# weidafeng/Efficient-SlowFast

Hardware: AMD Instinct MI355X
Metric: clips/sec (8x8 224^2 SlowFast-R50+CMDA, train step fwd+bwd+allreduce+SGD) (higher is better)
Workload: dtype f32

## Files before the change

### efficient-slowfast_amd/csrc/backward.hip

```cpp
#include "common.h"
#include <stdlib.h>

namespace {

constexpr int TPB = 256;


inline int pow2ceil_b(int v) {
  int p = 1;
  while (p < v) p <<= 1;
  return p;
}

template <int VEC>
__device__ __forceinline__ void bn_g(const float* __restrict__ dy, int dy_cs, int dy_coff,
                                     const float* __restrict__ y, int y_cs, int y_coff, long r, long THW, int HW,
                                     int rep, int relu, int c, float (&g)[VEC]) {
  long r0 = r;
  if (rep > 1) {
    const long n = r / THW, rem = r - n * THW;
    const long t = rem / HW, hw = rem - t * HW;
    r0 = (n * (THW / HW) * rep + t * rep) * HW + hw;
  }
#pragma unroll
// ... 387 lines not shown
  for (int a = 1; a < alpha; ++a) mx = fmaxf(mx, s[(long)a * HW * cs]);
  const float dm = dz[((long)b * rows + r) * dz_cs + dz_coff + c] * gate[(long)b * C + c] + dpool[(long)b * C + c];
  for (int a = 0; a < alpha; ++a)
    if (s[(long)a * HW * cs] == mx) {
      dx[(base + (long)a * HW) * dx_cs + dx_coff + c] += dm;
      break;
    }
}

__global__ void bcast_add_kernel(float* __restrict__ g, int cs, int coff, long rows_per_n, int C,
                                 const float* __restrict__ v, float scale, long total) {
  const long idx = (long)blockIdx.x * TPB + threadIdx.x;
  if (idx >= total) return;
  const int c = (int)(idx % C);
  const long r = idx / C;
  const long n = r / rows_per_n;
  g[r * cs + coff + c] += v[n * C + c] * scale;
}

__global__ void rowdot_kernel(const float* __restrict__ a, int a_cs, int a_coff, const float* __restrict__ b,
                              int b_cs, int b_coff, long rows, int C, float scale, float* __restrict__ out) {
  const long r = (long)blockIdx.x * TPB + threadIdx.x;
  if (r >= rows) return;
  const float* ap = a + r * a_cs + a_coff;
  const float* bp = b + r * b_cs + b_coff;
  float s = 0.f;
  for (int c = 0; c < C; ++c) s = fmaf(ap[c], bp[c], s);
  out[r] = s * scale;
}

__global__ __launch_bounds__(256) void rowdot_vec4_kernel(const float* __restrict__ a, int a_cs, int a_coff,
                                                          const float* __restrict__ b, int b_cs, int b_coff, long rows,
                                                          int cv_shift, float scale, float* __restrict__ out) {
  const long idx = (long)blockIdx.x * TPB + threadIdx.x;
  const long r = idx >> cv_shift;
  const int c = (int)(idx - (r << cv_shift)) * 4;
  float s = 0.f;
  if (r < rows) {
    const f32x4 x = *reinterpret_cast<const f32x4*>(a + r * a_cs + a_coff + c);
    const f32x4 y = *reinterpret_cast<const f32x4*>(b + r * b_cs + b_coff + c);
    s = x[0] * y[0] + x[1] * y[1] + x[2] * y[2] + x[3] * y[3];
  }
  for (int o = (1 << cv_shift) >> 1; o > 0; o >>= 1) s += __shfl_xor(s, o, 64);
  if (r < rows && c == 0) out[r] = s * scale;
}

__global__ void axpy_kernel(const float* __restrict__ a, int a_cs, int a_coff, float alpha, float* __restrict__ out,
                            int out_cs, int out_coff, int C, int accumulate, long total) {
  const long idx = (long)blockIdx.x * TPB + threadIdx.x;
  if (idx >= total) return;
  const int c = (int)(idx % C);
  const long r = idx / C;
  const float v = alpha * a[r * a_cs + a_coff + c];
  float* o = out + r * out_cs + out_coff + c;
  *o = accumulate ? *o + v : v;
}

__global__ void act_bwd_kernel(const float* __restrict__ dy, int dy_cs, int dy_coff, const float* __restrict__ y,
                               int y_cs, int y_coff, int act, float* __restrict__ dx, int dx_cs, int dx_coff, int C,
                               int accumulate, long total) {
  const long idx = (long)blockIdx.x * TPB + threadIdx.x;
  if (idx >= total) return;
  const int c = (int)(idx % C);
  const long r = idx / C;
  const float yv = y[r * y_cs + y_coff + c];
  const bool pass = (yv > 0.f) && (act != SF_ACT_RELU6 || yv < 6.f);
  const float v = pass ? dy[r * dy_cs + dy_coff + c] : 0.f;
  float* o = dx + r * dx_cs + dx_coff + c;
  *o = accumulate ? *o + v : v;
}

}

constexpr int MAX_P = 1024;
static inline void red_geometry(long rows, int C, int vec, int* CB, int* P) {
  const int cv = sf_cdiv(C, vec);
  *CB = pow2ceil_b(cv) < TPB ? pow2ceil_b(cv) : TPB;
  const int rpi = TPB / *CB;
  long p = rows / ((long)rpi * 8);
  if (p < 1) p = 1;
  if (p > MAX_P) p = MAX_P;
  *P = (int)p;
}
extern "C" long sf_bn_bwd_ws_floats(int C) { return (long)MAX_P * 2 * C; }

static int bn_bwd_reduce_launch(const float* dy, int dy_cs, int dy_coff, const float* y, int y_cs, int y_coff,
                                const float* z, int z_cs, int z_coff, int N, int T, int H, int W, int C, int S,
                                int rep, int relu, const float* mean, const float* invstd, float* dbeta,
                                float* dgamma, float* ws, void* stream, float* dbeta_acc = nullptr,
                                float* dgamma_acc = nullptr) {
  if ((dbeta_acc == nullptr) != (dgamma_acc == nullptr)) return SF_EINVAL;
  if (!dy || !z || !mean || !invstd || !dbeta || !dgamma || !ws || (relu && !y)) return SF_EINVAL;
  if (relu == 3 && (rep != 1 || (C % 4) != 0 || y_cs != C / 4 || y_coff != 0)) return SF_EINVAL;
  if (N <= 0 || T <= 0 || H <= 0 || W <= 0 || C <= 0 || rep <= 0 || S <= 0 || N % S != 0) return SF_EINVAL;
  if (S > 1 && N > MAX_P) return SF_EINVAL;
  const long rows = (long)N * T * H * W;
  const bool vec4 = (C % 4 == 0) && (dy_cs % 4 == 0) && (dy_coff % 4 == 0) && (z_cs % 4 == 0) && (z_coff % 4 == 0) &&
                    sf_aligned16(dy) && sf_aligned16(z) &&
                    (!relu || relu == 3 || ((y_cs % 4 == 0) && (y_coff % 4 == 0) && sf_aligned16(y)));
  if (relu == 3 && !vec4) return SF_EINVAL;
  const int groups = S > 1 ? N : 1;
  const long group_rows = rows / groups;
  int CB, P;
  const bool ring = sf_ticket_ring_ready((hipStream_t)stream);
  red_geometry(group_rows, C, vec4 ? 4 : 1, &CB, &P);
  const bool small = ring && S == 1 && P <= 16;
  const bool few = !small && ring && S == 1 && vec4 && C >= 256;
  const bool fused = few || small;
  const int max_p = few ? 64 : (small ? 512 : MAX_P);
  if (few && CB > 16) {
    CB = 16;
    long pp = group_rows / ((long)(TPB / CB) * 8);
    P = (int)(pp < 1 ? 1 : (pp > max_p ? max_p : pp));
  }
  if (P > max_p) P = max_p;
  if ((long)P * groups > max_p) P = max_p / groups;
  if (P < 1) return SF_EINVAL;
  const int chunks = P;
  P = chunks * groups;
  const int ncb = sf_cdiv(sf_cdiv(C, vec4 ? 4 : 1), CB);
  unsigned* tickets = fused ? sf_ticket_slots(ncb) : nullptr;
  if (fused && !tickets) return SF_ELAUNCH;
  if (vec4)
    hipLaunchKernelGGL(bn_bwd_partial_kernel<4>, dim3(P, ncb), dim3(TPB), 0, (hipStream_t)stream, dy, dy_cs, dy_coff,
                       y, y_cs, y_coff, z, z_cs, z_coff, group_rows, chunks, S, (long)T * H * W, H * W, C, rep, relu,
                       mean, invstd, CB, ws, tickets, dbeta, dgamma, dbeta_acc, dgamma_acc);
  else
    hipLaunchKernelGGL(bn_bwd_partial_kernel<1>, dim3(P, ncb), dim3(TPB), 0, (hipStream_t)stream, dy, dy_cs, dy_coff,
                       y, y_cs, y_coff, z, z_cs, z_coff, group_rows, chunks, S, (long)T * H * W, H * W, C, rep, relu,
                       mean, invstd, CB, ws, tickets, dbeta, dgamma, dbeta_acc, dgamma_acc);
  if (!fused)
    hipLaunchKernelGGL(pair_final_kernel, dim3(S * C), dim3(64), 0, (hipStream_t)stream, ws, C, P, chunks, S, dbeta,
                       dgamma, dbeta_acc, dgamma_acc);
  SF_CHECK_LAUNCH();
  return SF_OK;
}

extern "C" int sf_bn_bwd_reduce(const float* dy, int dy_cs, int dy_coff, const float* y, int y_cs, int y_coff,
                                const float* z, int z_cs, int z_coff, int N, int T, int H, int W, int C, int rep,
                                int relu, const float* mean, const float* invstd, float* dbeta, float* dgamma,
                                float* ws, void* stream) {
  return bn_bwd_reduce_launch(dy, dy_cs, dy_coff, y, y_cs, y_coff, z, z_cs, z_coff, N, T, H, W, C, 1, rep, relu, mean,
                              invstd, dbeta, dgamma, ws, stream);
}

extern "C" int sf_bn_bwd_reduce_acc(const float* dy, int dy_cs, int dy_coff, const float* y, int y_cs, int y_coff,
                                    const float* z, int z_cs, int z_coff, int N, int T, int H, int W, int C, int rep,
                                    int relu, const float* mean, const float* invstd, float* dbeta, float* dgamma,
                                    float* ws, float* dbeta_acc, float* dgamma_acc, void* stream) {
  return bn_bwd_reduce_launch(dy, dy_cs, dy_coff, y, y_cs, y_coff, z, z_cs, z_coff, N, T, H, W, C, 1, rep, relu, mean,
                              invstd, dbeta, dgamma, ws, stream, dbeta_acc, dgamma_acc);
}

extern "C" int sf_bn_bwd_reduce_split(const float* dy, int dy_cs, int dy_coff, const float* y, int y_cs, int y_coff,
                                      const float* z, int z_cs, int z_coff, int N, int T, int H, int W, int C,
                                      int nsplit, int rep, int relu, const float* mean, const float* invstd,
                                      float* dbeta, float* dgamma, float* ws, void* stream) {
  return bn_bwd_reduce_launch(dy, dy_cs, dy_coff, y, y_cs, y_coff, z, z_cs, z_coff, N, T, H, W, C, nsplit, rep, relu,
                              mean, invstd, dbeta, dgamma, ws, stream);
}

static int bn_bwd_apply_launch(const float* dy, int dy_cs, int dy_coff, const float* y, int y_cs, int y_coff,
                               const float* z, int z_cs, int z_coff, int N, int T, int H, int W, int C, int S, int rep,
                               int relu, const float* mean, const float* invstd, const float* gamma,
                               const float* dbeta, const float* dgamma, float* dz, int dz_cs, int dz_coff,
                               float* dres, int dres_cs, int dres_coff, int dres_acc, void* stream) {
  if (!dy || !z || !mean || !invstd || !gamma || !dbeta || !dgamma || !dz || (relu && !y)) return SF_EINVAL;
  if (relu == 3 && (rep != 1 || (C % 4) != 0 || y_cs != C / 4 || y_coff != 0)) return SF_EINVAL;
  if (N <= 0 || T <= 0 || H <= 0 || W <= 0 || C <= 0 || rep <= 0 || S <= 0 || N % S != 0) return SF_EINVAL;
  const long rows = (long)N * T * H * W;
  const bool vec4 = (C % 4 == 0) && (dy_cs % 4 == 0) && (dy_coff % 4 == 0) && (z_cs % 4 == 0) && (z_coff % 4 == 0) &&
                    (dz_cs % 4 == 0) && (dz_coff % 4 == 0) && sf_aligned16(dy) && sf_aligned16(z) && sf_aligned16(dz) &&
                    (!relu || relu == 3 || ((y_cs % 4 == 0) && (y_coff % 4 == 0) && sf_aligned16(y))) &&
                    (!dres || ((dres_cs % 4 == 0) && (dres_coff % 4 == 0) && sf_aligned16(dres)));
  if (relu == 3 && !vec4) return SF_EINVAL;
  const long total = rows * (vec4 ? C / 4 : C);
  const int unroll4 = (vec4 && rep == 1 && (relu == 0 || relu == 3) && total >= 262144L &&
                       total < 0x7fffffffL && rows < 0x7fffffffL && (rows % 4) == 0 &&
                       sf_aligned16(mean) && sf_aligned16(invstd) && sf_aligned16(gamma) && sf_aligned16(dbeta) &&
                       sf_aligned16(dgamma)) ? 1 : 0;
  if (vec4)
    hipLaunchKernelGGL(bn_bwd_apply_kernel<4>, dim3(sf_cdiv(unroll4 ? (total + 3) / 4 : total, TPB)), dim3(TPB), 0,
                       (hipStream_t)stream, dy, dy_cs, dy_coff, y, y_cs, y_coff, z, z_cs, z_coff, rows, (long)T * H * W,
                       H * W, C, S, rep, relu, mean, invstd, gamma, dbeta, dgamma, (float)S / (float)rows, dz, dz_cs,
                       dz_coff, dres, dres_cs, dres_coff, dres_acc, total, unroll4);
  else
    hipLaunchKernelGGL(bn_bwd_apply_kernel<1>, dim3(sf_cdiv(total, TPB)), dim3(TPB), 0, (hipStream_t)stream, dy, dy_cs,
                       dy_coff, y, y_cs, y_coff, z, z_cs, z_coff, rows, (long)T * H * W, H * W, C, S, rep, relu, mean,
                       invstd, gamma, dbeta, dgamma, (float)S / (float)rows, dz, dz_cs, dz_coff, dres, dres_cs,
                       dres_coff, dres_acc, total, 0);
  SF_CHECK_LAUNCH();
  return SF_OK;
}

extern "C" int sf_bn_bwd_apply(const float* dy, int dy_cs, int dy_coff, const float* y, int y_cs, int y_coff,
                               const float* z, int z_cs, int z_coff, int N, int T, int H, int W, int C, int rep,
                               int relu, const float* mean, const float* invstd, const float* gamma,
                               const float* dbeta, const float* dgamma, float* dz, int dz_cs, int dz_coff,
                               float* dres, int dres_cs, int dres_coff, void* stream) {
  return bn_bwd_apply_launch(dy, dy_cs, dy_coff, y, y_cs, y_coff, z, z_cs, z_coff, N, T, H, W, C, 1, rep, relu, mean,
                             invstd, gamma, dbeta, dgamma, dz, dz_cs, dz_coff, dres, dres_cs, dres_coff, 1, stream);
}

extern "C" int sf_bn_bwd_apply_first(const float* dy, int dy_cs, int dy_coff, const float* y, int y_cs, int y_coff,
                                     const float* z, int z_cs, int z_coff, int N, int T, int H, int W, int C, int rep,
                                     int relu, const float* mean, const float* invstd, const float* gamma,
                                     const float* dbeta, const float* dgamma, float* dz, int dz_cs, int dz_coff,
                                     float* dres, int dres_cs, int dres_coff, void* stream) {
  if (!dres) return SF_EINVAL;
  return bn_bwd_apply_launch(dy, dy_cs, dy_coff, y, y_cs, y_coff, z, z_cs, z_coff, N, T, H, W, C, 1, rep, relu, mean,
                             invstd, gamma, dbeta, dgamma, dz, dz_cs, dz_coff, dres, dres_cs, dres_coff, 0, stream);
}

extern "C" int sf_bn_bwd_apply_split(const float* dy, int dy_cs, int dy_coff, const float* y, int y_cs, int y_coff,
                                     const float* z, int z_cs, int z_coff, int N, int T, int H, int W, int C,
                                     int nsplit, int rep, int relu, const float* mean, const float* invstd,
                                     const float* gamma, const float* dbeta, const float* dgamma, float* dz,
                                     int dz_cs, int dz_coff, float* dres, int dres_cs, int dres_coff, void* stream) {
  return bn_bwd_apply_launch(dy, dy_cs, dy_coff, y, y_cs, y_coff, z, z_cs, z_coff, N, T, H, W, C, nsplit, rep, relu,
                             mean, invstd, gamma, dbeta, dgamma, dz, dz_cs, dz_coff, dres, dres_cs, dres_coff, 1,
                             stream);
}

__global__ __launch_bounds__(256) void maxpool_bwd_vec4_kernel(const sf_pool_desc d, const float* __restrict__ x,
                                                               const float* __restrict__ y,
                                                               const float* __restrict__ dy, int dy_cs, int dy_coff,
                                                               float* __restrict__ dx, int dx_cs, int dx_coff,
                                                               int acc, unsigned total) {
  const unsigned idx = blockIdx.x * TPB + threadIdx.x;
  if (idx >= total) return;
  const unsigned cv = d.C >> 2;
  const unsigned rin = idx / cv;
  const int c = (int)(idx - rin * cv) * 4;
  unsigned r = rin;
  const int wi = (int)(r % (unsigned)d.Wi);
  r /= (unsigned)d.Wi;
  const int hi = (int)(r % (unsigned)d.Hi);
  r /= (unsigned)d.Hi;
  const int ti = (int)(r % (unsigned)d.Ti);
  const int n = (int)(r / (unsigned)d.Ti);
  const f32x4 xv = *reinterpret_cast<const f32x4*>(x + (long)rin * d.in_cs + d.in_coff + c);
  auto lo = [](int i, int p, int k, int s) { const int a = i + p - k + 1; return a <= 0 ? 0 : (a + s - 1) / s; };
  const int t0 = lo(ti, d.pT, d.kT, d.sT), t1 = min((ti + d.pT) / d.sT, d.To - 1);
  const int h0 = lo(hi, d.pH, d.kH, d.sH), h1 = min((hi + d.pH) / d.sH, d.Ho - 1);
  const int w0 = lo(wi, d.pW, d.kW, d.sW), w1 = min((wi + d.pW) / d.sW, d.Wo - 1);
  f32x4 g = {0.f, 0.f, 0.f, 0.f};
  for (int to = t0; to <= t1; ++to)
    for (int ho = h0; ho <= h1; ++ho)
      for (int wo = w0; wo <= w1; ++wo) {
        const long ro = (((long)n * d.To + to) * d.Ho + ho) * d.Wo + wo;
        const f32x4 yv = *reinterpret_cast<const f32x4*>(y + ro * d.out_cs + d.out_coff + c);
        const f32x4 gv = *reinterpret_cast<const f32x4*>(dy + ro * dy_cs + dy_coff + c);
        unsigned m = (yv[0] == xv[0] ? 1u : 0u) | (yv[1] == xv[1] ? 2u : 0u) | (yv[2] == xv[2] ? 4u : 0u) |
                     (yv[3] == xv[3] ? 8u : 0u);
        if (m) {
          const int ts = to * d.sT - d.pT, hs = ho * d.sH - d.pH, ws = wo * d.sW - d.pW;
          for (int tt = max(ts, 0); tt <= ti && m; ++tt)
            for (int hh = max(hs, 0); hh < min(hs + d.kH, d.Hi) && m; ++hh) {
              if (tt == ti && hh > hi) break;
              for (int ww = max(ws, 0); ww < min(ws + d.kW, d.Wi) && m; ++ww) {
                if (tt == ti && hh == hi && ww >= wi) break;
                const f32x4 xe = *reinterpret_cast<const f32x4*>(
                    x + ((((long)n * d.Ti + tt) * d.Hi + hh) * d.Wi + ww) * d.in_cs + d.in_coff + c);
#pragma unroll
                for (int e = 0; e < 4; ++e)
                  if (xe[e] == yv[e]) m &= ~(1u << e);
              }
            }
#pragma unroll
          for (int e = 0; e < 4; ++e)
            if ((m >> e) & 1u) g[e] += gv[e];
        }
      }
  f32x4* o = reinterpret_cast<f32x4*>(dx + (long)rin * dx_cs + dx_coff + c);
  *o = acc ? *o + g : g;
}

static int maxpool_bwd_launch(const sf_pool_desc* d, const float* x, const float* y, const float* dy, int dy_cs,
                              int dy_coff, float* dx, int dx_cs, int dx_coff, int acc, void* stream) {
  if (!d || !x || !y || !dy || !dx || d->is_avg) return SF_EINVAL;
  const long total = (long)d->N * d->Ti * d->Hi * d->Wi * d->C;
  const bool vec4 = (d->C % 4 == 0) && (d->in_cs % 4 == 0) && (d->in_coff % 4 == 0) && (d->out_cs % 4 == 0) &&
                    (d->out_coff % 4 == 0) && (dy_cs % 4 == 0) && (dy_coff % 4 == 0) && (dx_cs % 4 == 0) &&
                    (dx_coff % 4 == 0) && sf_aligned16(x) && sf_aligned16(y) && sf_aligned16(dy) && sf_aligned16(dx) &&
                    total / 4 < 0x7fffffffL;
  if (vec4)
    hipLaunchKernelGGL(maxpool_bwd_vec4_kernel, dim3(sf_cdiv(total / 4, TPB)), dim3(TPB), 0, (hipStream_t)stream, *d, x,
                       y, dy, dy_cs, dy_coff, dx, dx_cs, dx_coff, acc, (unsigned)(total / 4));
  else
    hipLaunchKernelGGL(maxpool_bwd_kernel, dim3(sf_cdiv(total, TPB)), dim3(TPB), 0, (hipStream_t)stream, *d, x, y, dy,
                       dy_cs, dy_coff, dx, dx_cs, dx_coff, acc, total);
  SF_CHECK_LAUNCH();
  return SF_OK;
}

extern "C" int sf_maxpool_bwd(const sf_pool_desc* d, const float* x, const float* y, const float* dy, int dy_cs,
                              int dy_coff, float* dx, int dx_cs, int dx_coff, void* stream) {
  return maxpool_bwd_launch(d, x, y, dy, dy_cs, dy_coff, dx, dx_cs, dx_coff, 1, stream);
}

extern "C" int sf_maxpool_bwd_first(const sf_pool_desc* d, const float* x, const float* y, const float* dy, int dy_cs,
                                    int dy_coff, float* dx, int dx_cs, int dx_coff, void* stream) {
  return maxpool_bwd_launch(d, x, y, dy, dy_cs, dy_coff, dx, dx_cs, dx_coff, 0, stream);
}

extern "C" int sf_tmax_dot(const float* x, int cs, int coff, int N, int T, int H, int W, int C, int alpha,
// ... 449 lines not shown
```

### efficient-slowfast_amd/csrc/conv_bx.hip

```cpp
#include "bx.h"
#include <stdlib.h>

namespace {

constexpr int BXC_BM = 256;
constexpr int BXC_BK = 16;
constexpr int BXC_STAGES = 3;
constexpr int BXC_ROWB = BXC_BK * 2;
constexpr int BXC_A_STAGE = 3 * BXC_BM * BXC_ROWB;

struct BxArgs {
  sf_conv_desc d;
  const unsigned short* ap;
  const unsigned short* bp;
  float* ws;
  const float* scale;
  const float* bias;
  const float* res;
  float* out;
  int M, ntaps, cpk, nk, S, nk_per, nb_n, tiles;
  int tap_major;
  unsigned a_rows, a_bytes, b_bytes;
  unsigned a_plane, b_plane;
  unsigned wo_mul, wo_sh, ho_mul, ho_sh, to_mul, to_sh;
  const float* xf;
  unsigned xf_bytes;
  float* stats;
};

__device__ __forceinline__ unsigned mdiv(unsigned n, unsigned mul, unsigned sh) {
  return mul ? (__umulhi(n, mul) >> sh) : n;
}

typedef __attribute__((address_space(3))) void lds_void;

template <int BN, bool DIRECT, bool AF32>
__global__ __launch_bounds__(512, 2) void conv_bx_kernel(const BxArgs p) {
  constexpr int A_ST = AF32 ? BXC_BM * 64 : BXC_A_STAGE;
  constexpr int B_STAGE = 3 * BN * BXC_ROWB;
  constexpr int STAGE = A_ST + B_STAGE;
  constexpr int NT = BN / 64;
  extern __shared__ __attribute__((aligned(16))) char smem[];
  const sf_conv_desc& d = p.d;
  const int tid = threadIdx.x, lane = tid & 63;
  const int wave = __builtin_amdgcn_readfirstlane(tid >> 6);
  const int wm = wave & 3, wn = wave >> 2;
  const int bid = xcd_remap(blockIdx.x, p.tiles * p.S);
  const int split = bid / p.tiles, tile = bid - split * p.tiles;
  const int tile_m = tile / p.nb_n, tile_n = tile - tile_m * p.nb_n;
  const int m0 = tile_m * BXC_BM, n0 = tile_n * BN;
  const int ks0 = split * p.nk_per;
  const int ks1 = ks0 + p.nk_per < p.nk ? ks0 + p.nk_per : p.nk;
  const int nsteps = ks1 - ks0;

  const int lrow = lane >> 1;
  const unsigned lchunk = (unsigned)((lane & 1) ^ ((lrow >> 4) & 1)) * 16u;
  const int am = m0 + 32 * wave + lrow;
  const bool a_ok = am < p.M;
  int t0, h0, w0, nimg;
  {
    const unsigned mm = a_ok ? (unsigned)am : 0u;
    const unsigned q1 = mdiv(mm, p.wo_mul, p.wo_sh);
    const unsigned wo = mm - q1 * (unsigned)d.Wo;
    const unsigned q2 = mdiv(q1, p.ho_mul, p.ho_sh);
    const unsigned ho = q1 - q2 * (unsigned)d.Ho;
    const unsigned q3 = mdiv(q2, p.to_mul, p.to_sh);
    const unsigned to = q2 - q3 * (unsigned)d.To;
    nimg = (int)q3;
    t0 = d.transposed ? (int)to + d.pT : (int)to * d.sT - d.pT;
    h0 = d.transposed ? (int)ho + d.pH : (int)ho * d.sH - d.pH;
    w0 = d.transposed ? (int)wo + d.pW : (int)wo * d.sW - d.pW;
  }
  struct FRow { int t0, h0, w0, n; bool ok; unsigned chunk; };
  FRow fr0 = {0, 0, 0, 0, false, 0u}, fr1 = fr0;
  if constexpr (AF32) {
    auto frow = [&](int u) -> FRow {
      FRow f;
      const int r = 32 * wave + 16 * u + (lane >> 2);
      const int fm = m0 + r;
      f.ok = fm < p.M;
      f.chunk = (unsigned)((lane & 3) ^ ((r >> 2) & 3)) * 16u;
      const unsigned mm = f.ok ? (unsigned)fm : 0u;
      const unsigned q1 = mdiv(mm, p.wo_mul, p.wo_sh);
      const unsigned wo = mm - q1 * (unsigned)d.Wo;
      const unsigned q2 = mdiv(q1, p.ho_mul, p.ho_sh);
      const unsigned ho = q1 - q2 * (unsigned)d.Ho;
      const unsigned q3 = mdiv(q2, p.to_mul, p.to_sh);
      const unsigned to = q2 - q3 * (unsigned)d.To;
      f.n = (int)q3;
      f.t0 = d.transposed ? (int)to + d.pT : (int)to * d.sT - d.pT;
      f.h0 = d.transposed ? (int)ho + d.pH : (int)ho * d.sH - d.pH;
      f.w0 = d.transposed ? (int)wo + d.pW : (int)wo * d.sW - d.pW;
      return f;
    };
    fr0 = frow(0);
    fr1 = frow(1);
  }
  auto f_voff = [&](const FRow f, int kt, int kh, int kw) -> unsigned {
    const int ti = d.transposed ? f.t0 - kt * d.dT : f.t0 + kt * d.dT;
    const int hi = d.transposed ? f.h0 - kh * d.dH : f.h0 + kh * d.dH;
    const int wi = d.transposed ? f.w0 - kw * d.dW : f.w0 + kw * d.dW;
    const bool ok = f.ok && (unsigned)ti < (unsigned)d.Ti && (unsigned)hi < (unsigned)d.Hi && (unsigned)wi < (unsigned)d.Wi;
    if (!ok) return 0x80000000u;
    const unsigned r = (unsigned)(((f.n * d.Ti + ti) * d.Hi + hi) * d.Wi + wi);
    return (r * (unsigned)d.in_cs + (unsigned)d.in_coff) * 4u + f.chunk;
  };
  const unsigned row_bytes = (unsigned)d.Cin * 2u;
  auto a_voff = [&](int kt, int kh, int kw) -> unsigned {
    const int ti = d.transposed ? t0 - kt * d.dT : t0 + kt * d.dT;
    const int hi = d.transposed ? h0 - kh * d.dH : h0 + kh * d.dH;
    const int wi = d.transposed ? w0 - kw * d.dW : w0 + kw * d.dW;
    const bool ok = a_ok && (unsigned)ti < (unsigned)d.Ti && (unsigned)hi < (unsigned)d.Hi && (unsigned)wi < (unsigned)d.Wi;
    const unsigned r = ok ? (unsigned)(((nimg * d.Ti + ti) * d.Hi + hi) * d.Wi + wi) : p.a_rows;
    return r * row_bytes + lchunk;
  };
  const bool b_loader = BN == 256 || wave < BN / 32;
  const int bn = n0 + 32 * wave + lrow;
  const unsigned kbytes = (unsigned)p.nk * (unsigned)BXC_ROWB;
  const unsigned b_voff = (unsigned)((b_loader && bn < d.Cout) ? bn : d.Cout) * kbytes + lchunk;

  const __amdgpu_buffer_rsrc_t a_rs = __builtin_amdgcn_make_buffer_rsrc((void*)p.ap, 0, p.a_bytes, 0x00020000);
  const __amdgpu_buffer_rsrc_t b_rs = __builtin_amdgcn_make_buffer_rsrc((void*)p.bp, 0, p.b_bytes, 0x00020000);
  const __amdgpu_buffer_rsrc_t x_rs = __builtin_amdgcn_make_buffer_rsrc((void*)p.xf, 0, AF32 ? p.xf_bytes : 0u, 0x00020000);

  struct LS { int c, tap, kw, kh, kt; };
  LS ls;
  ls.c = __builtin_amdgcn_readfirstlane(p.tap_major ? ks0 % p.cpk : ks0 / p.ntaps);
  ls.tap = __builtin_amdgcn_readfirstlane(p.tap_major ? ks0 / p.cpk : ks0 - ls.c * p.ntaps);
  ls.kw = __builtin_amdgcn_readfirstlane(ls.tap % d.kW);
  ls.kh = __builtin_amdgcn_readfirstlane((ls.tap / d.kW) % d.kH);
  ls.kt = __builtin_amdgcn_readfirstlane(ls.tap / (d.kW * d.kH));
  const int tap_major = p.tap_major, cpk = p.cpk, kW = d.kW, kH = d.kH, kT = d.kT;
  auto next = [=](const LS o) -> LS {
    LS n;
    if (tap_major) {
      const int c1 = o.c + 1;
      const bool wc = c1 == cpk;
      n.c = wc ? 0 : c1;
      n.tap = o.tap + (wc ? 1 : 0);
      const int w1 = o.kw + (wc ? 1 : 0);
      const bool ww = w1 == kW;
      n.kw = ww ? 0 : w1;
      const int h1 = o.kh + (ww ? 1 : 0);
      const bool wh = h1 == kH;
      n.kh = wh ? 0 : h1;
      n.kt = o.kt + (wh ? 1 : 0);
      return n;
    }
    const int w1 = o.kw + 1;
    const bool ww = w1 == kW;
    n.kw = ww ? 0 : w1;
    const int h1 = o.kh + (ww ? 1 : 0);
    const bool wh = h1 == kH;
    n.kh = wh ? 0 : h1;
    const int t1 = o.kt + (wh ? 1 : 0);
    const bool wt = t1 == kT;
    n.kt = wt ? 0 : t1;
    n.tap = wt ? 0 : o.tap + 1;
    n.c = o.c + (wt ? 1 : 0);
    return n;
  };
  auto issue = [&](int stage) {
    const LS l = ls;
    unsigned cur_voff = 0, cur_aso, cur_f0 = 0, cur_f1 = 0;
    if constexpr (AF32) {
      cur_f0 = f_voff(fr0, l.kt, l.kh, l.kw);
      cur_f1 = f_voff(fr1, l.kt, l.kh, l.kw);
      cur_aso = (unsigned)l.c * 64u;
    } else {
      cur_voff = a_voff(l.kt, l.kh, l.kw);
      cur_aso = (unsigned)l.c * (unsigned)BXC_ROWB;
    }
    const unsigned cur_bso = (unsigned)(l.tap * p.cpk + l.c) * (unsigned)BXC_ROWB;
    if constexpr (AF32) {
      __builtin_amdgcn_raw_ptr_buffer_load_lds(x_rs, (lds_void*)(smem + stage * STAGE + wave * 2048), 16, cur_f0, cur_aso,
                                               0, 0);
      __builtin_amdgcn_raw_ptr_buffer_load_lds(x_rs, (lds_void*)(smem + stage * STAGE + wave * 2048 + 1024), 16, cur_f1,
                                               cur_aso, 0, 0);
    } else {
      char* const sa = smem + stage * STAGE + wave * 1024;
#pragma unroll
      for (int g = 0; g < 3; ++g)
        __builtin_amdgcn_raw_ptr_buffer_load_lds(a_rs, (lds_void*)(sa + g * (BXC_BM * BXC_ROWB)), 16, cur_voff,
                                                 cur_aso + (unsigned)g * p.a_plane, 0, 0);
    }
    if (b_loader) {
      char* const sb = smem + stage * STAGE + A_ST + wave * 1024;
#pragma unroll
      for (int g = 0; g < 3; ++g)
        __builtin_amdgcn_raw_ptr_buffer_load_lds(b_rs, (lds_void*)(sb + g * (BN * BXC_ROWB)), 16, b_voff,
                                                 cur_bso + (unsigned)g * p.b_plane, 0, 0);
    }
    ls = next(l);
  };

  const unsigned frag_lane = (unsigned)(lane & 31) * BXC_ROWB + (unsigned)(((lane >> 5) ^ ((lane >> 4) & 1)) * 16);
  const unsigned a_frag = (unsigned)(wm * 64) * BXC_ROWB + frag_lane;
  const unsigned b_frag = A_ST + (unsigned)(wn * (BN / 2)) * BXC_ROWB + frag_lane;
  unsigned f_frag[2][2] = {{0, 0}, {0, 0}};
  if constexpr (AF32) {
#pragma unroll
    for (int i = 0; i < 2; ++i) {
      const int r = wm * 64 + i * 32 + (lane & 31);
#pragma unroll
      for (int q = 0; q < 2; ++q) f_frag[i][q] = (unsigned)r * 64u + (unsigned)(((2 * (lane >> 5) + q) ^ ((r >> 2) & 3)) * 16);
    }
  }

  f32x16 acc[2][NT];
#pragma unroll
  for (int i = 0; i < 2; ++i)
#pragma unroll
    for (int j = 0; j < NT; ++j)
#pragma unroll
      for (int e = 0; e < 16; ++e) acc[i][j][e] = 0.f;

  if (nsteps > 0) issue(0);
  if (nsteps > 1) issue(1);
  for (int it = 0; it < nsteps; ++it) {
    if (it + 1 < nsteps) {
      if constexpr (AF32) {
        if (b_loader) asm volatile("s_waitcnt vmcnt(5)" ::: "memory");
        else asm volatile("s_waitcnt vmcnt(2)" ::: "memory");
      } else {
        if (b_loader) asm volatile("s_waitcnt vmcnt(6)" ::: "memory");
        else asm volatile("s_waitcnt vmcnt(3)" ::: "memory");
      }
    } else {
      asm volatile("s_waitcnt vmcnt(0)" ::: "memory");
    }
    __builtin_amdgcn_s_barrier();
    if (it + 2 < nsteps) issue((it + 2) % BXC_STAGES);
    const char* const st = smem + (it % BXC_STAGES) * STAGE;
    u32x4 af[2][3], bf[NT][3];
    if constexpr (AF32) {
#pragma unroll
      for (int i = 0; i < 2; ++i) {
        const f32x4 lo = *reinterpret_cast<const f32x4*>(st + f_frag[i][0]);
        const f32x4 hi = *reinterpret_cast<const f32x4*>(st + f_frag[i][1]);
        split_pair(lo[0], lo[1], af[i], 0);
        split_pair(lo[2], lo[3], af[i], 1);
        split_pair(hi[0], hi[1], af[i], 2);
        split_pair(hi[2], hi[3], af[i], 3);
      }
    }
#pragma unroll
    for (int pc = 0; pc < 3; ++pc) {
      if constexpr (!AF32) {
#pragma unroll
        for (int i = 0; i < 2; ++i)
          af[i][pc] = *reinterpret_cast<const u32x4*>(st + a_frag + pc * (BXC_BM * BXC_ROWB) + i * (32 * BXC_ROWB));
      }
#pragma unroll
      for (int j = 0; j < NT; ++j)
        bf[j][pc] = *reinterpret_cast<const u32x4*>(st + b_frag + pc * (BN * BXC_ROWB) + j * (32 * BXC_ROWB));
    }
#pragma unroll
    for (int i = 0; i < 2; ++i)
#pragma unroll
      for (int j = 0; j < NT; ++j) acc[i][j] = mfma_split(af[i], bf[j], acc[i][j]);
  }

  const int col = lane & 31, rsub = 4 * (lane >> 5);
  if (DIRECT) {
#pragma unroll
    for (int j = 0; j < NT; ++j) {
      const int n = n0 + wn * (BN / 2) + j * 32 + col;
      const bool n_ok = n < d.Cout;
      const float sc = (p.scale && n_ok) ? p.scale[n] : 1.f;
      const float bi = (p.bias && n_ok) ? p.bias[n] : 0.f;
#pragma unroll
      for (int i = 0; i < 2; ++i) {
        float r[16];
#pragma unroll
        for (int e = 0; e < 16; ++e) {
          const int m = m0 + wm * 64 + i * 32 + (e & 3) + 8 * (e >> 2) + rsub;
          r[e] = (p.res && m < p.M && n_ok) ? p.res[(long)m * d.res_cs + d.res_coff + n] : 0.f;
        }
#pragma unroll
        for (int e = 0; e < 16; ++e) {
          const int m = m0 + wm * 64 + i * 32 + (e & 3) + 8 * (e >> 2) + rsub;
          if (m < p.M && n_ok) p.out[(long)m * d.out_cs + d.out_coff + n] = sf_act(acc[i][j][e] * sc + bi + r[e], d.act);
        }
      }
    }
    return;
  }
  float* const wsp = p.ws + (long)split * p.M * d.Cout;
#pragma unroll
  for (int i = 0; i < 2; ++i)
#pragma unroll
    for (int j = 0; j < NT; ++j) {
      const int n = n0 + wn * (BN / 2) + j * 32 + col;
#pragma unroll
      for (int e = 0; e < 16; ++e) {
        const int m = m0 + wm * 64 + i * 32 + (e & 3) + 8 * (e >> 2) + rsub;
        if (m < p.M && n < d.Cout) wsp[(long)m * d.Cout + n] = acc[i][j][e];
      }
    }
}

template <int BN>
__global__ __launch_bounds__(512, 4) void conv_pw_bx_kernel(const BxArgs p) {
  constexpr int A_STAGE = BXC_BM * 64;
  constexpr int B_STAGE = 3 * BN * BXC_ROWB;
  constexpr int STAGE = A_STAGE + B_STAGE;
  constexpr int NT = BN / 64;
  extern __shared__ __attribute__((aligned(16))) char smem[];
  const sf_conv_desc& d = p.d;
  const int tid = threadIdx.x, lane = tid & 63;
  const int wave = __builtin_amdgcn_readfirstlane(tid >> 6);
  const int wm = wave & 3, wn = wave >> 2;
  const int bid = xcd_remap(blockIdx.x, p.tiles);
  const int tile_m = bid / p.nb_n, tile_n = bid - tile_m * p.nb_n;
  const int m0 = tile_m * BXC_BM, n0 = tile_n * BN;
  const int nsteps = p.nk;

  const int lrow = lane >> 1;
  const unsigned lchunk = (unsigned)((lane & 1) ^ ((lrow >> 4) & 1)) * 16u;
  const bool b_loader = BN == 256 || wave < BN / 32;
  const int bn = n0 + 32 * wave + lrow;
  const unsigned kbytes = (unsigned)p.nk * (unsigned)BXC_ROWB;
  const unsigned b_voff = (unsigned)((b_loader && bn < d.Cout) ? bn : d.Cout) * kbytes + lchunk;
  const __amdgpu_buffer_rsrc_t b_rs = __builtin_amdgcn_make_buffer_rsrc((void*)p.bp, 0, p.b_bytes, 0x00020000);
  const __amdgpu_buffer_rsrc_t x_rs = __builtin_amdgcn_make_buffer_rsrc((void*)p.xf, 0, p.xf_bytes, 0x00020000);
  unsigned a_lvoff[2];
#pragma unroll
  for (int u = 0; u < 2; ++u) {
    const int r = 32 * wave + 16 * u + (lane >> 2);
    const int m = m0 + r;
    const unsigned chunk = (unsigned)((lane & 3) ^ ((r >> 2) & 3));
    a_lvoff[u] = m < p.M ? ((unsigned)m * (unsigned)d.in_cs + (unsigned)d.in_coff) * 4u + chunk * 16u : 0x80000000u;
  }
  auto issue = [&](int step) {
    char* const st = smem + (step % 2) * STAGE;
#pragma unroll
    for (int u = 0; u < 2; ++u)
      __builtin_amdgcn_raw_ptr_buffer_load_lds(x_rs, (lds_void*)(st + wave * 2048 + u * 1024), 16, a_lvoff[u],
                                               (unsigned)step * 64u, 0, 0);
    if (b_loader) {
      char* const sb = st + A_STAGE + wave * 1024;
#pragma unroll
      for (int g = 0; g < 3; ++g)
        __builtin_amdgcn_raw_ptr_buffer_load_lds(b_rs, (lds_void*)(sb + g * (BN * BXC_ROWB)), 16, b_voff,
                                                 (unsigned)step * (unsigned)BXC_ROWB + (unsigned)g * p.b_plane, 0, 0);
    }
  };
  unsigned a_frag[2][2];
#pragma unroll
  for (int i = 0; i < 2; ++i) {
    const int r = wm * 64 + i * 32 + (lane & 31);
#pragma unroll
    for (int q = 0; q < 2; ++q)
      a_frag[i][q] = (unsigned)r * 64u + (unsigned)(((2 * (lane >> 5) + q) ^ ((r >> 2) & 3)) * 16);
  }
  const unsigned frag_lane = (unsigned)(lane & 31) * BXC_ROWB + (unsigned)(((lane >> 5) ^ ((lane >> 4) & 1)) * 16);
  const unsigned b_frag = A_STAGE + (unsigned)(wn * (BN / 2)) * BXC_ROWB + frag_lane;

  f32x16 acc[2][NT];
#pragma unroll
  for (int i = 0; i < 2; ++i)
#pragma unroll
    for (int j = 0; j < NT; ++j)
#pragma unroll
      for (int e = 0; e < 16; ++e) acc[i][j][e] = 0.f;

  if (nsteps > 0) issue(0);
  for (int it = 0; it < nsteps; ++it) {
    asm volatile("s_waitcnt vmcnt(0)" ::: "memory");
    __builtin_amdgcn_s_barrier();
    if (it + 1 < nsteps) issue(it + 1);
    const char* const st = smem + (it % 2) * STAGE;
    u32x4 af[2][3], bf[NT][3];
#pragma unroll
    for (int i = 0; i < 2; ++i) {
      const f32x4 lo = *reinterpret_cast<const f32x4*>(st + a_frag[i][0]);
      const f32x4 hi = *reinterpret_cast<const f32x4*>(st + a_frag[i][1]);
      split_pair(lo[0], lo[1], af[i], 0);
      split_pair(lo[2], lo[3], af[i], 1);
      split_pair(hi[0], hi[1], af[i], 2);
      split_pair(hi[2], hi[3], af[i], 3);
    }
#pragma unroll
    for (int pc = 0; pc < 3; ++pc)
#pragma unroll
      for (int j = 0; j < NT; ++j)
        bf[j][pc] = *reinterpret_cast<const u32x4*>(st + b_frag + pc * (BN * BXC_ROWB) + j * (32 * BXC_ROWB));
#pragma unroll
    for (int i = 0; i < 2; ++i)
#pragma unroll
      for (int j = 0; j < NT; ++j) acc[i][j] = mfma_split(af[i], bf[j], acc[i][j]);
  }

  const int col = lane & 31, rsub = 4 * (lane >> 5);
  const bool want_stats = p.stats != nullptr;
  float* const kred = reinterpret_cast<float*>(smem);
  if (want_stats) __syncthreads();
#pragma unroll
  for (int j = 0; j < NT; ++j) {
    const int cl = wn * (BN / 2) + j * 32 + col;
    const int n = n0 + cl;
    const bool n_ok = n < d.Cout;
    const float sc = (p.scale && n_ok) ? p.scale[n] : 1.f;
    const float bi = (p.bias && n_ok) ? p.bias[n] : 0.f;
#pragma unroll
    for (int i = 0; i < 2; ++i) {
      float r[16];
#pragma unroll
      for (int e = 0; e < 16; ++e) {
        const int m = m0 + wm * 64 + i * 32 + (e & 3) + 8 * (e >> 2) + rsub;
        r[e] = (p.res && m < p.M && n_ok) ? p.res[(long)m * d.res_cs + d.res_coff + n] : 0.f;
      }
#pragma unroll
      for (int e = 0; e < 16; ++e) {
        const int m = m0 + wm * 64 + i * 32 + (e & 3) + 8 * (e >> 2) + rsub;
        const float v = sf_act(acc[i][j][e] * sc + bi + r[e], d.act);
        acc[i][j][e] = v;
        if (m < p.M && n_ok) p.out[(long)m * d.out_cs + d.out_coff + n] = v;
      }
    }
    if (want_stats && wm == 0 && rsub == 0) kred[cl] = acc[0][j][0];
  }
  if (!want_stats) return;
  __syncthreads();
  float* const sred = kred + BN;
#pragma unroll
  for (int j = 0; j < NT; ++j) {
    const int cl = wn * (BN / 2) + j * 32 + col;
    const float k0 = kred[cl];
    float s1 = 0.f, s2 = 0.f;
#pragma unroll
    for (int i = 0; i < 2; ++i)
#pragma unroll
      for (int e = 0; e < 16; ++e) {
        const int m = m0 + wm * 64 + i * 32 + (e & 3) + 8 * (e >> 2) + rsub;
        if (m < p.M) {
          const float dv = acc[i][j][e] - k0;
          s1 += dv;
          s2 += dv * dv;
        }
      }
    s1 += __shfl_xor(s1, 32, 64);
    s2 += __shfl_xor(s2, 32, 64);
    if (rsub == 0) {
      sred[(wm * BN + cl) * 2] = s1;
      sred[(wm * BN + cl) * 2 + 1] = s2;
    }
  }
  __syncthreads();
  if (tid < BN) {
    const int n = n0 + tid;
    if (n < d.Cout) {
      float s1 = 0.f, s2 = 0.f;
#pragma unroll
      for (int w = 0; w < 4; ++w) {
        s1 += sred[(w * BN + tid) * 2];
        s2 += sred[(w * BN + tid) * 2 + 1];
      }
      const int left = p.M - m0;
      const float cnt = (float)(left < BXC_BM ? left : BXC_BM);
      float* const o = p.stats + ((long)tile_m * (d.Cout >> 2) + (n >> 2)) * 16 + (n & 3);
      o[0] = cnt;
      o[4] = kred[tid];
      o[8] = s1;
      o[12] = s2;
    }
  }
}

struct BxwArgs {
  sf_conv_desc d;
  const unsigned short* xp;
  const unsigned short* zp;
  float* part;
  int M, Kc, S, chunk, nb_col, tiles;
  unsigned x_rows, x_plane, x_bytes, z_plane, z_bytes;
  unsigned wo_mul, wo_sh, ho_mul, ho_sh, to_mul, to_sh, ci_mul, ci_sh;
};

__device__ __forceinline__ u32x2 lds_tr(const char* p) {
  return lds_read_tr(reinterpret_cast<const unsigned short*>(p));
}
__device__ __forceinline__ u32x2 lds_tr_raw(unsigned lds_byte_addr) {
  u32x2 r;
  asm volatile("ds_read_b64_tr_b16 %0, %1" : "=v"(r) : "v"(lds_byte_addr));
  return r;
}

template <int BCO>
__global__ __launch_bounds__(512, 2) void conv_bx_wgrad_kernel(const BxwArgs p) {
  constexpr int BCOL = 256;
  constexpr int NWC = BCO == 256 ? 2 : 4;
  constexpr int NT = BCOL / NWC / 32;
  constexpr int ROW_A = BCO * 2, ROW_B = BCOL * 2;
  constexpr int PL_A = 16 * ROW_A, PL_B = 16 * ROW_B;
  constexpr int A_STAGE = 3 * PL_A, STAGE = A_STAGE + 3 * PL_B;
  constexpr int NA = PL_A / 1024;
  constexpr int CPR_A = BCO / 8;
  extern __shared__ __attribute__((aligned(16))) char smem[];
  const sf_conv_desc& d = p.d;
  const int tid = threadIdx.x, lane = tid & 63;
  const int wave = __builtin_amdgcn_readfirstlane(tid >> 6);
  const int wr = wave / NWC, wc = wave - wr * NWC;
  const int bid = xcd_remap(blockIdx.x, p.tiles * p.S);
  const int split = bid / p.tiles, tile = bid - split * p.tiles;
  const int tile_co = tile / p.nb_col, tile_col = tile - tile_co * p.nb_col;
  const int co0 = tile_co * BCO, col0 = tile_col * BCOL;
  const int mb = split * p.chunk;
  const int me = mb + p.chunk < p.M ? mb + p.chunk : p.M;
  const int nsteps = me > mb ? (me - mb + 15) / 16 : 0;

  const int b_pos = 2 * wave + (lane >> 5);
  const int b_cs = (lane & 31) ^ ((b_pos & 3) << 2);
  const int b_col = col0 + b_cs * 8;
  const bool b_colok = b_col < p.Kc;
  const unsigned b_tap = b_colok ? mdiv((unsigned)b_col, p.ci_mul, p.ci_sh) : 0u;
  const unsigned b_ci = b_colok ? (unsigned)b_col - b_tap * (unsigned)d.Cin : 0u;
  const int b_kw = (int)(b_tap % (unsigned)d.kW), b_kh = (int)((b_tap / (unsigned)d.kW) % (unsigned)d.kH),
            b_kt = (int)(b_tap / (unsigned)(d.kW * d.kH));
  const int b_dt = b_kt * d.dT - d.pT, b_dh = b_kh * d.dH - d.pH, b_dw = b_kw * d.dW - d.pW;
  const unsigned x_rowb = (unsigned)d.Cin * 2u;
  auto b_voff = [&](int m) -> unsigned {
    unsigned r = p.x_rows;
    if (m < me && b_colok) {
      const unsigned q1 = mdiv((unsigned)m, p.wo_mul, p.wo_sh);
      const int wo = (int)((unsigned)m - q1 * (unsigned)d.Wo);
      const unsigned q2 = mdiv(q1, p.ho_mul, p.ho_sh);
      const int ho = (int)(q1 - q2 * (unsigned)d.Ho);
      const unsigned q3 = mdiv(q2, p.to_mul, p.to_sh);
      const int to = (int)(q2 - q3 * (unsigned)d.To);
      const int ti = to * d.sT + b_dt, hi = ho * d.sH + b_dh, wi = wo * d.sW + b_dw;
      if ((unsigned)ti < (unsigned)d.Ti && (unsigned)hi < (unsigned)d.Hi && (unsigned)wi < (unsigned)d.Wi)
        r = (unsigned)((((int)q3 * d.Ti + ti) * d.Hi + hi) * d.Wi + wi);
    }
    return r * x_rowb + b_ci * 2u;
  };
  const bool a_loader = wave < NA;
  const int a_pos = wave * (64 / CPR_A) + lane / CPR_A;
  const int a_cs = (lane % CPR_A) ^ ((a_pos & 3) << 2);
  const int a_co = co0 + a_cs * 8;
  const unsigned z_rowb = (unsigned)d.Cout * 2u;
  auto a_voff = [&](int m) -> unsigned {
    const unsigned r = (m < me && a_co < d.Cout) ? (unsigned)m : (unsigned)p.M;
    return r * z_rowb + (unsigned)(a_co < d.Cout ? a_co : 0) * 2u;
  };
  const __amdgpu_buffer_rsrc_t x_rs = __builtin_amdgcn_make_buffer_rsrc((void*)p.xp, 0, p.x_bytes, 0x00020000);
  const __amdgpu_buffer_rsrc_t z_rs = __builtin_amdgcn_make_buffer_rsrc((void*)p.zp, 0, p.z_bytes, 0x00020000);
// ... 18 lines not shown
  const int g = lane >> 4, q = (lane & 15) >> 2, pq = lane & 3, h = g >> 1;
  unsigned a_addr[2], b_addr[NT];
#pragma unroll
  for (int i = 0; i < 2; ++i) {
    const int ch = wr * 64 + i * 32 + 16 * (g & 1) + 4 * pq;
    a_addr[i] = (unsigned)((8 * h + q) * ROW_A + (((ch >> 3) ^ (q << 2)) << 4) + (ch & 7) * 2);
  }
#pragma unroll
  for (int j = 0; j < NT; ++j) {
    const int ch = wc * (BCOL / NWC) + j * 32 + 16 * (g & 1) + 4 * pq;
    b_addr[j] = (unsigned)(A_STAGE + (8 * h + q) * ROW_B + (((ch >> 3) ^ (q << 2)) << 4) + (ch & 7) * 2);
  }

  f32x16 acc[2][NT];
#pragma unroll
  for (int i = 0; i < 2; ++i)
#pragma unroll
    for (int j = 0; j < NT; ++j)
#pragma unroll
      for (int e = 0; e < 16; ++e) acc[i][j][e] = 0.f;
  const unsigned lds_base = (unsigned)(uintptr_t)(__attribute__((address_space(3))) char*)smem;

  if (nsteps > 0) issue(0);
  if (nsteps > 1) issue(1);
  for (int it = 0; it < nsteps; ++it) {
    if (it + 1 < nsteps) {
      if (a_loader) asm volatile("s_waitcnt vmcnt(6)" ::: "memory");
      else asm volatile("s_waitcnt vmcnt(3)" ::: "memory");
    } else {
      asm volatile("s_waitcnt vmcnt(0)" ::: "memory");
    }
    __builtin_amdgcn_s_barrier();
    const unsigned st = lds_base + (unsigned)((it % BXC_STAGES) * STAGE);
    u32x4 af[2][3], bf[NT][3];
#pragma unroll
    for (int pc = 0; pc < 3; ++pc) {
#pragma unroll
      for (int i = 0; i < 2; ++i) {
        const u32x2 lo = lds_tr_raw(st + a_addr[i] + pc * PL_A), hi = lds_tr_raw(st + a_addr[i] + pc * PL_A + 4 * ROW_A);
        af[i][pc] = (u32x4){lo[0], lo[1], hi[0], hi[1]};
      }
#pragma unroll
      for (int j = 0; j < NT; ++j) {
        const u32x2 lo = lds_tr_raw(st + b_addr[j] + pc * PL_B), hi = lds_tr_raw(st + b_addr[j] + pc * PL_B + 4 * ROW_B);
        bf[j][pc] = (u32x4){lo[0], lo[1], hi[0], hi[1]};
      }
    }
    __builtin_amdgcn_sched_barrier(0);
    if (it + 2 < nsteps) issue((it + 2) % BXC_STAGES);
    __builtin_amdgcn_sched_barrier(0);
#pragma unroll
    for (int pc = 0; pc < 3; ++pc) {
      if constexpr (NT == 4)
        asm volatile("s_waitcnt lgkmcnt(0)"
                     : "+v"(af[0][pc]), "+v"(af[1][pc]), "+v"(bf[0][pc]), "+v"(bf[1][pc]), "+v"(bf[2][pc]), "+v"(bf[3][pc]));
      else
        asm volatile("s_waitcnt lgkmcnt(0)" : "+v"(af[0][pc]), "+v"(af[1][pc]), "+v"(bf[0][pc]), "+v"(bf[1][pc]));
    }
#pragma unroll
    for (int i = 0; i < 2; ++i)
#pragma unroll
      for (int j = 0; j < NT; ++j) acc[i][j] = mfma_split(af[i], bf[j], acc[i][j]);
  }

  float* const out = p.part + (long)split * d.Cout * p.Kc;
  const int ccol = lane & 31, rsub = 4 * (lane >> 5);
#pragma unroll
  for (int i = 0; i < 2; ++i)
#pragma unroll
    for (int j = 0; j < NT; ++j) {
      const int col = col0 + wc * (BCOL / NWC) + j * 32 + ccol;
#pragma unroll
      for (int e = 0; e < 16; ++e) {
        const int co = co0 + wr * 64 + i * 32 + (e & 3) + 8 * (e >> 2) + rsub;
        if (co < d.Cout && col < p.Kc) out[(long)co * p.Kc + col] = acc[i][j][e];
      }
    }
}

__global__ __launch_bounds__(256) void bx_split_rows_kernel(const float* __restrict__ x, int cs, int coff, long rows,
                                                            int C, unsigned short* __restrict__ planes) {
  const int c8 = C >> 3;
  const long total = (rows + 1) * c8;
  const long plane = (rows + 1) * (long)C;
  for (long idx = (long)blockIdx.x * 256 + threadIdx.x; idx < total; idx += (long)gridDim.x * 256) {
    const long r = idx / c8;
    const int c = (int)(idx - r * c8) * 8;
    u32x4 w[3];
    if (r < rows) {
      const f32x4 v0 = *reinterpret_cast<const f32x4*>(x + r * cs + coff + c);
      const f32x4 v1 = *reinterpret_cast<const f32x4*>(x + r * cs + coff + c + 4);
      split_pair(v0[0], v0[1], w, 0);
      split_pair(v0[2], v0[3], w, 1);
      split_pair(v1[0], v1[1], w, 2);
      split_pair(v1[2], v1[3], w, 3);
    } else {
      w[0] = w[1] = w[2] = (u32x4){0u, 0u, 0u, 0u};
    }
#pragma unroll
    for (int pc = 0; pc < 3; ++pc) *reinterpret_cast<u32x4*>(planes + pc * plane + r * C + c) = w[pc];
  }
}

struct BxSplitItem {
  const float* x;
  unsigned short* planes;
  long rows;
  int C, pad_;
};
__global__ __launch_bounds__(256) void bx_split_batched_kernel(const BxSplitItem* __restrict__ items,
                                                               const int* __restrict__ blk0, int n) {
  int lo = 0, hi = n;
  while (hi - lo > 1) {
    const int mid = (lo + hi) >> 1;
    if (blk0[mid] <= (int)blockIdx.x) lo = mid; else hi = mid;
  }
  const BxSplitItem it = items[lo];
  const int c8 = it.C >> 3;
  const long idx = (long)((int)blockIdx.x - blk0[lo]) * 256 + threadIdx.x;
  if (idx >= (it.rows + 1) * c8) return;
  const long plane = (it.rows + 1) * (long)it.C;
  const long r = idx / c8;
  const int c = (int)(idx - r * c8) * 8;
  u32x4 w[3];
  if (r < it.rows) {
    const f32x4 v0 = *reinterpret_cast<const f32x4*>(it.x + r * it.C + c);
    const f32x4 v1 = *reinterpret_cast<const f32x4*>(it.x + r * it.C + c + 4);
    split_pair(v0[0], v0[1], w, 0);
    split_pair(v0[2], v0[3], w, 1);
    split_pair(v1[0], v1[1], w, 2);
    split_pair(v1[2], v1[3], w, 3);
  } else {
    w[0] = w[1] = w[2] = (u32x4){0u, 0u, 0u, 0u};
  }
#pragma unroll
  for (int pc = 0; pc < 3; ++pc) *reinterpret_cast<u32x4*>(it.planes + pc * plane + r * it.C + c) = w[pc];
}

void magic(unsigned dv, unsigned* mul, unsigned* sh) {
  if (dv <= 1) { *mul = 0; *sh = 0; return; }
  unsigned l = 0;
  while ((1u << l) < dv) ++l;
  const unsigned long long num = 1ull << (31 + l);
  *mul = (unsigned)((num + dv - 1) / dv);
  *sh = l - 1;
}

int g_bx_enable = 1;

struct BxPlan { int bn, S, nk, nk_per, nb_n, tiles, direct; long a_rows; };

bool bx_af32(const sf_conv_desc* d);

bool bx_plan(const sf_conv_desc* d, BxPlan* pl, bool gate = true) {
  if (!g_bx_enable) return false;
  const long M = (long)d->N * d->To * d->Ho * d->Wo;
  const int ntaps = d->kT * d->kH * d->kW;
  if ((d->Cin % 16) || d->cin_pad != d->Cin || (d->in_cs % 4) || (d->in_coff % 4)) return false;
  if (d->Cout < 128 || (d->Cout % 4) || d->out_cmul != 1) return false;
  const int nk = ntaps * (d->Cin / BXC_BK);
  if (nk < 32 || M < 2048 || M > 0x7fffffffL) return false;
  if (d->transposed && (d->sT != 1 || d->sH != 1 || d->sW != 1)) return false;
  const long a_rows = (long)d->N * d->Ti * d->Hi * d->Wi;
  if (3 * (a_rows + 1) * d->Cin * 2 > 0xfffffff0L) return false;
  if (3L * (d->Cout + 1) * nk * BXC_ROWB > 0xfffffff0L) return false;
  pl->bn = d->Cout >= 256 ? 256 : 128;
  pl->nb_n = sf_cdiv(d->Cout, pl->bn);
  pl->tiles = sf_cdiv(M, BXC_BM) * pl->nb_n;
  pl->nk = nk;
  pl->a_rows = a_rows;
  const bool scatter = d->os_T > 1 || d->os_H > 1 || d->os_W > 1;
  const double step_us = pl->bn == 256 ? 2.05 : 1.6;
  const double out_mb = (double)M * d->Cout * 4e-6;
  int best = 1;
  double best_t = 1e30;
  for (int S = 1; S <= 16 && nk / S >= 8; ++S) {
    const long wg = (long)pl->tiles * S;
    if (wg > 2048) break;
    const long rounds = sf_cdiv(wg, 256);
    double t = 6.0 + (double)rounds * sf_cdiv(nk, S) * step_us;
    if (S > 1 || scatter) t += 3.0 + out_mb * (2.0 * S + 1.0) / 4.0;
    else t += out_mb / 4.0;
    if (t < best_t - 1e-9) { best_t = t; best = S; }
  }
  pl->S = best;
  pl->nk_per = sf_cdiv(nk, best);
  pl->direct = (best == 1 && !scatter) ? 1 : 0;
  if (gate && g_bx_enable < 2) {
    const double flop = 2.0 * M * (double)nk * BXC_BK * d->Cout;
    const double wave_us = flop / (nk >= 64 ? 100e6 : 90e6);
    const double split_us = bx_af32(d) ? 0.0 : 4.0 + (double)a_rows * d->Cin * 10e-6 / 3.0;
    const double pad = (double)(pl->nb_n * pl->bn) / (double)d->Cout;
    if (best_t * pad + split_us > 0.93 * wave_us) return false;
  }
  return true;
}


int g_pw_enable = 1;

struct PwPlan { int bn, nb_n, tiles, nk; };

bool pw_plan(const sf_conv_desc* d, PwPlan* pl, bool gate = true) {
  if (!g_bx_enable || !g_pw_enable) return false;
  if (d->kT != 1 || d->kH != 1 || d->kW != 1 || d->sT != 1 || d->sH != 1 || d->sW != 1 || d->pT || d->pH || d->pW)
    return false;
  if (d->To != d->Ti || d->Ho != d->Hi || d->Wo != d->Wi) return false;
  if (d->os_T > 1 || d->os_H > 1 || d->os_W > 1 || d->out_cmul != 1) return false;
  if ((d->Cin % 16) || d->cin_pad != d->Cin || (d->in_cs % 4) || (d->in_coff % 4)) return false;
  if (d->Cin < 64 || d->Cout < 64 || (d->Cout % 4)) return false;
  const long M = (long)d->N * d->To * d->Ho * d->Wo;
  if (M < 2048 || M > 0x3fffffffL) return false;
  if (((M - 1) * d->in_cs + d->in_coff + d->Cin) * 4L >= 0x7fffffffL) return false;
  pl->nk = d->Cin / BXC_BK;
  if (3L * (d->Cout + 1) * pl->nk * BXC_ROWB > 0xfffffff0L) return false;
  pl->bn = d->Cout <= 64 ? 64 : 128;
  pl->nb_n = sf_cdiv(d->Cout, pl->bn);
  pl->tiles = sf_cdiv(M, BXC_BM) * pl->nb_n;
  if (gate && g_pw_enable < 2 && g_bx_enable < 2) {
    const double mb = (double)M * (d->Cin + d->Cout) * 4e-6;
    if (pl->bn == 64) {
      if (d->Cin < 128) return false;
      return true;
    }
    if (d->Cout < 128) return false;
    double t_pw = 6.0 + (double)sf_cdiv(pl->tiles, 256) * pl->nk * 1.5;
    if (t_pw < mb / 4.5) t_pw = mb / 4.5;
    const double t_f32 = 6.0 + 2.0 * M * (double)d->Cin * d->Cout / 95e6 + 0.5 * mb / 4.5;
    if (t_pw > 0.85 * t_f32) return false;
  }
  return true;
}

template <int BN>
int launch_pw(const BxArgs& a, int grid, hipStream_t stream) {
  constexpr int lds = 2 * (BXC_BM * 64 + 3 * BN * BXC_ROWB);
  static_assert(lds >= (BN + 4 * BN * 2) * 4, "the statistics scratch lives in the stages");
  static SfLdsAttr at;
  if (!sf_ensure_dyn_lds(at, reinterpret_cast<const void*>(conv_pw_bx_kernel<BN>), lds)) return SF_ELAUNCH;
  hipLaunchKernelGGL((conv_pw_bx_kernel<BN>), dim3(grid), dim3(512), lds, stream, a);
  SF_CHECK_LAUNCH();
  return SF_OK;
}

bool bx_af32(const sf_conv_desc* d) {
  const long rows = (long)d->N * d->Ti * d->Hi * d->Wi;
  return ((rows - 1) * d->in_cs + d->in_coff + d->Cin) * 4L < 0x7fffffffL;
}

long align4(long floats) { return (floats + 3) & ~3L; }
long a_plane_floats(const sf_conv_desc* d, long a_rows) { return align4((3 * (a_rows + 1) * d->Cin + 1) / 2); }
long b_plane_floats(const sf_conv_desc* d, int nk) { return align4((3L * (d->Cout + 1) * nk * BXC_BK + 1) / 2); }

template <int BN, bool DIRECT, bool AF32>
int launch_bx_v(const BxArgs& a, int grid, hipStream_t stream) {
  constexpr int lds = BXC_STAGES * ((AF32 ? BXC_BM * 64 : BXC_A_STAGE) + 3 * BN * BXC_ROWB);
  static SfLdsAttr at;
  if (!sf_ensure_dyn_lds(at, reinterpret_cast<const void*>(conv_bx_kernel<BN, DIRECT, AF32>), lds)) return SF_ELAUNCH;
  hipLaunchKernelGGL((conv_bx_kernel<BN, DIRECT, AF32>), dim3(grid), dim3(512), lds, stream, a);
  SF_CHECK_LAUNCH();
  return SF_OK;
}

template <int BN, bool DIRECT>
int launch_bx(const BxArgs& a, int grid, hipStream_t stream) {
  if (a.xf) return launch_bx_v<BN, DIRECT, true>(a, grid, stream);
  return launch_bx_v<BN, DIRECT, false>(a, grid, stream);
}

}

int sf_conv_bx_tune(int value) { g_bx_enable = value; return SF_OK; }

int sf_conv_bx_takes(const sf_conv_desc* d) {
  BxPlan pl;
  return bx_plan(d, &pl) ? 1 : 0;
}

extern "C" long sf_bx_planes_elems(long rows, int C) { return 3 * (rows + 1) * (long)C; }

int sf_bx_split_rows(const float* x, int cs, int coff, long rows, int C, unsigned short* planes, hipStream_t s) {
  if ((C & 7) || (cs & 3) || (coff & 3) || !sf_aligned16(x) || !sf_aligned16(planes)) return SF_EALIGN;
  const long total = (rows + 1) * (C >> 3);
  long blocks = (total + 255) / 256;
  if (blocks > 256 * 16) blocks = 256 * 16;
  hipLaunchKernelGGL(bx_split_rows_kernel, dim3((unsigned)blocks), dim3(256), 0, s, x, cs, coff, rows, C, planes);
  SF_CHECK_LAUNCH();
  return SF_OK;
}

extern "C" int sf_bx_split(const float* x, int cs, int coff, long rows, int C, unsigned short* planes, void* stream) {
  if (!x || !planes || rows <= 0 || C <= 0) return SF_EINVAL;
  return sf_bx_split_rows(x, cs, coff, rows, C, planes, (hipStream_t)stream);
}

extern "C" int sf_bx_split_batched(const void* items, const int* blk0, int n, int nblocks, void* stream) {
  if (!items || !blk0 || n <= 0 || nblocks <= 0) return SF_EINVAL;
  hipLaunchKernelGGL(bx_split_batched_kernel, dim3(nblocks), dim3(256), 0, (hipStream_t)stream,
                     reinterpret_cast<const BxSplitItem*>(items), blk0, n);
  SF_CHECK_LAUNCH();
  return SF_OK;
}

int sf_conv_pw_tune(int value) { g_pw_enable = value; return SF_OK; }

int sf_conv_pw_takes(const sf_conv_desc* d) {
  PwPlan pl;
  return pw_plan(d, &pl) ? 1 : 0;
}

extern "C" long sf_conv_pw_ws_floats(const sf_conv_desc* d, int have_w_planes) {
  PwPlan pl;
  if (!d || !pw_plan(d, &pl)) return 0;
  return 4 + (have_w_planes ? 0 : b_plane_floats(d, pl.nk));
}

extern "C" long sf_conv_pw_stats_floats(const sf_conv_desc* d) {
  PwPlan pl;
  if (!d || d->transposed || d->act != SF_ACT_NONE || !pw_plan(d, &pl)) return 0;
  const long M = (long)d->N * d->To * d->Ho * d->Wo;
  return (long)sf_cdiv(M, BXC_BM) * 4 * d->Cout;
}

int sf_conv_pw_try(const sf_conv_desc* d, const float* in, const float* w_packed, const unsigned short* w_planes,
                   const float* scale, const float* bias, const float* res, float* out, float* ws, float* stats,
                   int* parts, hipStream_t stream) {
  PwPlan pl;
  if (parts) *parts = 0;
  if (!ws || !pw_plan(d, &pl)) return 1;
  if (!sf_aligned16(in) || !sf_aligned16(w_packed) || !sf_aligned16(ws)) return 1;
  if (w_planes && !sf_aligned16(w_planes)) return SF_EALIGN;
  if (stats && (scale || res || d->act != SF_ACT_NONE || !parts || !sf_aligned16(stats))) return 1;
  const long M = (long)d->N * d->To * d->Ho * d->Wo;
  if (!w_planes) {
    unsigned short* const bp = reinterpret_cast<unsigned short*>(ws + 4);
    const int rc = sf_bx_split_rows(w_packed, pl.nk * BXC_BK, 0, d->Cout, pl.nk * BXC_BK, bp, stream);
    if (rc != SF_OK) return rc;
    w_planes = bp;
  }
  BxArgs a = {};
  a.d = *d;
  a.bp = w_planes;
  a.scale = scale; a.bias = bias; a.res = res; a.out = out;
  a.M = (int)M;
  a.ntaps = 1; a.cpk = pl.nk; a.nk = pl.nk; a.S = 1; a.nk_per = pl.nk; a.nb_n = pl.nb_n; a.tiles = pl.tiles;
  a.b_plane = (unsigned)((long)(d->Cout + 1) * pl.nk * BXC_ROWB);
  a.b_bytes = 3u * a.b_plane;
  a.xf = in;
  a.xf_bytes = (unsigned)(((M - 1) * d->in_cs + d->in_coff + d->Cin) * 4L);
  a.stats = stats;
  if (stats) *parts = (int)sf_cdiv(M, BXC_BM);
  if (pl.bn == 64) return launch_pw<64>(a, pl.tiles, stream);
  return launch_pw<128>(a, pl.tiles, stream);
}

extern "C" int sf_conv_fwd_pw(const sf_conv_desc* d, const float* in, const float* w_packed,
                              const unsigned short* w_planes, const float* scale, const float* bias, const float* res,
                              float* out, float* ws, float* stats, int* parts, void* stream) {
  if (!d || !in || !w_packed || !out || !ws) return SF_EINVAL;
  const int rc = sf_conv_pw_try(d, in, w_packed, w_planes, scale, bias, res, out, ws, stats, parts, (hipStream_t)stream);
  return rc == 1 ? SF_ENOTTAKEN : rc;
}

extern "C" long sf_conv_bx_ws_floats(const sf_conv_desc* d, int have_in_planes, int have_w_planes) {
  BxPlan pl;
  if (!d || !bx_plan(d, &pl)) return 0;
  const long M = (long)d->N * d->To * d->Ho * d->Wo;
  return 4 + ((have_in_planes || bx_af32(d)) ? 0 : a_plane_floats(d, pl.a_rows)) +
         (have_w_planes ? 0 : b_plane_floats(d, pl.nk)) + (pl.direct ? 0 : (long)pl.S * M * d->Cout);
}

int sf_conv_splitk_finish(const sf_conv_desc* d, const float* ws, int S, const float* scale, const float* bias,
                          const float* res, float* out, hipStream_t s);

int sf_conv_bx_try(const sf_conv_desc* d, const float* in, const unsigned short* in_planes, const float* w_packed,
                   const unsigned short* w_planes, const float* scale, const float* bias, const float* res, float* out,
                   float* ws, hipStream_t stream) {
  BxPlan pl;
  if (!ws || !bx_plan(d, &pl)) return 1;
  if (!sf_aligned16(in) || !sf_aligned16(w_packed) || !sf_aligned16(ws)) return 1;
  if ((in_planes && !sf_aligned16(in_planes)) || (w_planes && !sf_aligned16(w_planes))) return SF_EALIGN;
  const long M = (long)d->N * d->To * d->Ho * d->Wo;
  float* cur = ws;
  int rc = SF_OK;
  const bool af32 = bx_af32(d);
  if (!in_planes && !af32) {
    unsigned short* const ap = reinterpret_cast<unsigned short*>(cur);
    cur += a_plane_floats(d, pl.a_rows);
    rc = sf_bx_split_rows(in, d->in_cs, d->in_coff, pl.a_rows, d->Cin, ap, stream);
    if (rc != SF_OK) return rc;
    in_planes = ap;
  }
  if (!w_planes) {
    unsigned short* const bp = reinterpret_cast<unsigned short*>(cur);
    cur += b_plane_floats(d, pl.nk);
    rc = sf_bx_split_rows(w_packed, pl.nk * BXC_BK, 0, d->Cout, pl.nk * BXC_BK, bp, stream);
    if (rc != SF_OK) return rc;
    w_planes = bp;
  }
  BxArgs a = {};
  a.d = *d;
  a.ap = in_planes; a.bp = w_planes; a.ws = cur;
  if (af32) {
    a.xf = in;
    a.xf_bytes = (unsigned)(((pl.a_rows - 1) * d->in_cs + d->in_coff + d->Cin) * 4L);
  }
  a.scale = scale; a.bias = bias; a.res = res; a.out = out;
  a.M = (int)M;
  a.ntaps = d->kT * d->kH * d->kW;
  a.cpk = d->Cin / BXC_BK;
  a.nk = pl.nk; a.S = pl.S; a.nk_per = pl.nk_per; a.nb_n = pl.nb_n; a.tiles = pl.tiles;
  a.tap_major = (d->sT > 1 || d->sH > 1 || d->sW > 1) ? 1 : 0;
  a.a_rows = (unsigned)pl.a_rows;
  a.a_plane = (unsigned)((pl.a_rows + 1) * d->Cin * 2);
  a.a_bytes = 3u * a.a_plane;
  a.b_plane = (unsigned)((long)(d->Cout + 1) * pl.nk * BXC_ROWB);
  a.b_bytes = 3u * a.b_plane;
  magic((unsigned)d->Wo, &a.wo_mul, &a.wo_sh);
  magic((unsigned)d->Ho, &a.ho_mul, &a.ho_sh);
  magic((unsigned)d->To, &a.to_mul, &a.to_sh);
  const int grid = pl.tiles * pl.S;
  if (pl.bn == 256) rc = pl.direct ? launch_bx<256, true>(a, grid, stream) : launch_bx<256, false>(a, grid, stream);
  else rc = pl.direct ? launch_bx<128, true>(a, grid, stream) : launch_bx<128, false>(a, grid, stream);
  if (rc != SF_OK) return rc;
  if (pl.direct) return SF_OK;
  return sf_conv_splitk_finish(d, cur, pl.S, scale, bias, res, out, stream);
}

extern "C" int sf_conv_fwd_bx(const sf_conv_desc* d, const float* in, const unsigned short* in_planes,
                              const float* w_packed, const unsigned short* w_planes, const float* scale,
                              const float* bias, const float* res, float* out, float* ws, void* stream) {
  if (!d || !in || !w_packed || !out || !ws) return SF_EINVAL;
  const int rc = sf_conv_bx_try(d, in, in_planes, w_packed, w_planes, scale, bias, res, out, ws, (hipStream_t)stream);
  return rc == 1 ? SF_ENOTTAKEN : rc;
}

namespace {

struct BxwPlan { int bco, S, nb_col, tiles; long chunk, x_rows; };

int g_bxw_enable = 1;

bool bxw_plan(const sf_conv_desc* d, BxwPlan* pl) {
  if (!g_bxw_enable) return false;
  const long M = (long)d->N * d->To * d->Ho * d->Wo;
  const int ntaps = d->kT * d->kH * d->kW;
  if ((d->Cin % 8) || d->cin_pad != d->Cin || (d->in_cs % 4) || (d->in_coff % 4)) return false;
  if (d->Cout < 128 || (d->Cout % 8)) return false;
  const long Kc = (long)ntaps * d->Cin;
  if (Kc < 512 || M < 2048 || M > 0x7ffffff0L) return false;
  const long x_rows = (long)d->N * d->Ti * d->Hi * d->Wi;
  if (3 * (x_rows + 1) * d->Cin * 2 > 0xfffffff0L || 3 * (M + 1) * d->Cout * 2 > 0xfffffff0L) return false;
  pl->bco = d->Cout >= 256 ? 256 : 128;
  pl->nb_col = sf_cdiv(Kc, 256);
  pl->tiles = sf_cdiv(d->Cout, pl->bco) * pl->nb_col;
  pl->x_rows = x_rows;
  const double step_us = pl->bco == 256 ? 2.0 : 1.1;
  const double out_mb = (double)d->Cout * Kc * 4e-6;
  int best = 1;
  double best_t = 1e30;
  const int maxS = (int)(M / 256 > 512 ? 512 : M / 256);
  for (int S = 1; S <= maxS; ++S) {
    const long wg = (long)pl->tiles * S;
    if (wg > 1536) break;
    const long rounds = sf_cdiv(wg, 256);
    const long steps = sf_cdiv(sf_cdiv(M, S), 16);
    const double t = 6.0 + (double)rounds * steps * step_us + out_mb * (2.0 * S + 1.0) / 4.0;
    if (t < best_t - 1e-9) { best_t = t; best = S; }
  }
  pl->S = best;
  pl->chunk = (sf_cdiv(M, best) + 15) / 16 * 16;
  if (g_bxw_enable < 2) {
    const double flop = 2.0 * M * (double)Kc * d->Cout;
    const double wave_us = flop / 95e6;
    const double split_us = 8.0 + ((double)x_rows * d->Cin + (double)M * d->Cout) * 10e-6 / 3.0;
    if (best_t + split_us > 0.93 * wave_us) return false;
  }
  return true;
}

long x_plane_floats(const sf_conv_desc* d, long x_rows) { return align4((3 * (x_rows + 1) * d->Cin + 1) / 2); }
long z_plane_floats(const sf_conv_desc* d, long M) { return align4((3 * (M + 1) * d->Cout + 1) / 2); }

template <int BCO>
int launch_bxw(const BxwArgs& a, int grid, hipStream_t stream) {
  constexpr int lds = BXC_STAGES * (3 * 16 * BCO * 2 + 3 * 16 * 256 * 2);
  static SfLdsAttr at;
  if (!sf_ensure_dyn_lds(at, reinterpret_cast<const void*>(conv_bx_wgrad_kernel<BCO>), lds)) return SF_ELAUNCH;
  hipLaunchKernelGGL((conv_bx_wgrad_kernel<BCO>), dim3(grid), dim3(512), lds, stream, a);
  SF_CHECK_LAUNCH();
  return SF_OK;
}

}

int sf_conv_bxw_tune(int value) { g_bxw_enable = value; return SF_OK; }

extern "C" int sf_conv_wgrad_bx_splits(const sf_conv_desc* d) {
  BxwPlan pl;
  return (d && bxw_plan(d, &pl)) ? pl.S : 0;
}

extern "C" long sf_conv_wgrad_bx_ws_floats(const sf_conv_desc* d, int have_x_planes, int have_dz_planes) {
  BxwPlan pl;
  if (!d || !bxw_plan(d, &pl)) return 0;
  const long M = (long)d->N * d->To * d->Ho * d->Wo;
  return 4 + (have_x_planes ? 0 : x_plane_floats(d, pl.x_rows)) + (have_dz_planes ? 0 : z_plane_floats(d, M));
}

extern "C" int sf_conv_wgrad_bx(const sf_conv_desc* d, const float* x, const unsigned short* x_planes, const float* dz,
                                int dz_cs, int dz_coff, const unsigned short* dz_planes, float* partial, float* ws,
                                void* stream) {
  BxwPlan pl;
  if (!d || !x || !dz || !partial || !ws) return SF_EINVAL;
  if (!bxw_plan(d, &pl)) return SF_ENOTTAKEN;
  if (!sf_aligned16(x) || !sf_aligned16(dz) || !sf_aligned16(ws) || !sf_aligned16(partial) || (dz_cs % 4) || (dz_coff % 4))
    return SF_EALIGN;
  hipStream_t s = (hipStream_t)stream;
  const long M = (long)d->N * d->To * d->Ho * d->Wo;
  float* cur = ws;
  int rc = SF_OK;
  if (!x_planes) {
    unsigned short* const xp = reinterpret_cast<unsigned short*>(cur);
    cur += x_plane_floats(d, pl.x_rows);
    rc = sf_bx_split_rows(x, d->in_cs, d->in_coff, pl.x_rows, d->Cin, xp, s);
    if (rc != SF_OK) return rc;
    x_planes = xp;
  }
  if (!dz_planes) {
    unsigned short* const zp = reinterpret_cast<unsigned short*>(cur);
    cur += z_plane_floats(d, M);
    rc = sf_bx_split_rows(dz, dz_cs, dz_coff, M, d->Cout, zp, s);
    if (rc != SF_OK) return rc;
    dz_planes = zp;
  }
  BxwArgs a;
  a.d = *d;
  a.xp = x_planes; a.zp = dz_planes; a.part = partial;
  a.M = (int)M;
  a.Kc = d->kT * d->kH * d->kW * d->Cin;
  a.S = pl.S; a.chunk = (int)pl.chunk; a.nb_col = pl.nb_col; a.tiles = pl.tiles;
  a.x_rows = (unsigned)pl.x_rows;
  a.x_plane = (unsigned)((pl.x_rows + 1) * d->Cin * 2);
  a.x_bytes = 3u * a.x_plane;
  a.z_plane = (unsigned)((M + 1) * d->Cout * 2);
  a.z_bytes = 3u * a.z_plane;
  magic((unsigned)d->Wo, &a.wo_mul, &a.wo_sh);
  magic((unsigned)d->Ho, &a.ho_mul, &a.ho_sh);
  magic((unsigned)d->To, &a.to_mul, &a.to_sh);
  magic((unsigned)d->Cin, &a.ci_mul, &a.ci_sh);
  const int grid = pl.tiles * pl.S;
  return pl.bco == 256 ? launch_bxw<256>(a, grid, s) : launch_bxw<128>(a, grid, s);
}
```

### efficient-slowfast_amd/sfhip/__init__.py

```python
import ctypes
import os

import torch

_HERE = os.path.dirname(os.path.abspath(__file__))
_LIB_PATH = os.environ.get("SF_LIB") or os.path.join(_HERE, "libsfhip.so")
_lib = None

ACT_NONE, ACT_RELU, ACT_SIGMOID, ACT_SOFTMAX, ACT_HSIGMOID, ACT_RELU6 = 0, 1, 2, 3, 4, 5


def _act(relu):
    return ACT_RELU6 if relu == 6 else (ACT_RELU if relu else ACT_NONE)
SF_EINVAL, SF_EALIGN, SF_ELAUNCH, SF_ENOTTAKEN = -1, -2, -3, -4
_ERR = {-1: "SF_EINVAL (inconsistent descriptor)", -2: "SF_EALIGN", -3: "SF_ELAUNCH (hip launch failed)",
        -4: "SF_ENOTTAKEN (shape not served by this specialised entry point)"}
_REFUSED = (SF_EALIGN, SF_ENOTTAKEN)


class SfhipError(RuntimeError):
    pass


class ConvDesc(ctypes.Structure):
    _fields_ = [(n, ctypes.c_int) for n in (
        "N", "Ti", "Hi", "Wi", "Cin", "in_cs", "in_coff", "To", "Ho", "Wo", "Cout", "out_cs", "out_coff",
        "out_cmul", "kT", "kH", "kW", "sT", "sH", "sW", "pT", "pH", "pW", "dT", "dH", "dW", "cin_pad", "act",
        "res_cs", "res_coff", "transposed", "os_T", "os_H", "os_W", "oo_T", "oo_H", "oo_W", "ob_T", "ob_H", "ob_W")]


class PoolDesc(ctypes.Structure):
    _fields_ = [(n, ctypes.c_int) for n in (
        "N", "Ti", "Hi", "Wi", "C", "in_cs", "in_coff", "To", "Ho", "Wo", "out_cs", "out_coff",
        "kT", "kH", "kW", "sT", "sH", "sW", "pT", "pH", "pW", "is_avg")]


_vp, _ci, _cl, _cf = ctypes.c_void_p, ctypes.c_int, ctypes.c_long, ctypes.c_float
_CD, _PD, _pi, _pf = ctypes.POINTER(ConvDesc), ctypes.POINTER(PoolDesc), ctypes.POINTER(_ci), ctypes.POINTER(_cf)
_VIEW = [_vp, _ci, _ci]
_ATTN_FWD = [_vp, _ci, _vp, _ci, _vp, _ci, _vp, _ci, _vp, _vp, _vp, _ci, _vp, _ci, _ci] + [_ci] * 6 + [_vp, _vp]
_BN_BWD = _VIEW * 3 + [_ci] * 7 + [_vp] * 5
_BN_BWD_SPLIT = _VIEW * 3 + [_ci] * 8 + [_vp] * 5
_BN_APPLY_TAIL = _VIEW * 2 + [_vp]
_SIGNATURES = {
    "sf_abi_version": (_ci, []),
    "sf_build_arch": (ctypes.c_char_p, []),
    "sf_ncthw_to_ndhwc": (_ci, [_vp, _vp] + [_ci] * 9 + [_vp]),
    "sf_ndhwc_to_ncthw": (_ci, [_vp, _ci, _ci, _vp] + [_ci] * 5 + [_vp]),
    "sf_clip_prologue": (_ci, [_vp] + [_ci] * 10 + [_pf] * 2 + [_vp, _ci, _vp, _ci, _ci, _ci, _vp]),
    "sf_clip_prologue_gray": (_ci, [_vp] + [_ci] * 9 + [_cf, _cf, _vp, _ci, _vp, _ci, _ci, _ci, _vp]),
    "sf_clip_views": (_ci, [_vp, _ci, _ci, _ci, _vp, _vp] + [_ci] * 5 + [_vp] * 4 + [_ci, _ci, _ci, _vp]),
    "sf_clip_views_gray": (_ci, [_vp, _ci, _ci, _ci, _vp, _vp] + [_ci] * 4 + [_cf, _cf, _vp, _vp, _ci, _ci, _ci, _vp]),
    "sf_clip_batch": (_ci, [_vp, _vp] + [_ci] * 5 + [_vp] * 4 + [_ci, _ci, _ci, _vp]),
    "sf_clip_batch_gray": (_ci, [_vp, _vp] + [_ci] * 4 + [_cf, _cf, _vp, _vp, _ci, _ci, _ci, _vp]),
    "sf_ensemble_update": (_ci, [_vp] * 4 + [_pi] * 3 + [_ci] * 4 + [_vp]),
    "sf_ensemble_update_ml": (_ci, [_vp] * 3 + [_ci, _vp, _vp, _pi, _pi] + [_ci] * 4 + [_vp]),
    "sf_ncthw1_pack": (_ci, [_vp, _vp] + [_ci] * 7 + [_vp]),
    "sf_stem1_accepts": (_ci, [_ci] * 4),
    "sf_stem1_fwd": (_ci, [_vp, _ci, _ci, _ci, _ci, _vp, _ci, _ci, _ci, _vp, _vp, _ci, _vp, _ci, _ci, _vp]),
    "sf_stem1_wgrad_ws_floats": (_cl, [_ci] * 7),
    "sf_stem1_wgrad": (_ci, [_vp, _ci, _ci, _ci, _ci, _vp, _ci, _ci, _ci, _ci, _ci, _vp, _ci, _vp, _vp]),
    "sf_conv_fwd": (_ci, [_CD] + [_vp] * 7),
    "sf_conv_fwd_ws_floats": (_cl, [_CD]),
    "sf_conv_fwd_ws": (_ci, [_CD] + [_vp] * 8),
    "sf_conv_fwd_grouped": (_ci, [_CD, _ci, _ci] + [_vp] * 7),
    "sf_conv_stats_ws_floats": (_cl, [_CD]),
    "sf_conv_fwd_stats": (_ci, [_CD] + [_vp] * 7 + [_pi, _vp]),
    "sf_conv_tune": (_ci, [_ci, _ci]),
    "sf_bx_planes_elems": (_cl, [_cl, _ci]),
    "sf_bx_split": (_ci, [_vp, _ci, _ci, _cl, _ci, _vp, _vp]),
    "sf_bx_split_batched": (_ci, [_vp, _vp, _ci, _ci, _vp]),
    "sf_conv_rows_parts": (_ci, [_CD]),
    "sf_conv_pw_ws_floats": (_cl, [_CD, _ci]),
    "sf_conv_pw_stats_floats": (_cl, [_CD]),
    "sf_conv_fwd_pw": (_ci, [_CD] + [_vp] * 9 + [_pi, _vp]),
    "sf_conv_bx_ws_floats": (_cl, [_CD, _ci, _ci]),
    "sf_conv_fwd_bx": (_ci, [_CD] + [_vp] * 10),
    "sf_pack_conv_weight": (_ci, [_vp, _ci, _ci, _ci, _vp, _ci, _vp, _ci, _vp]),
    "sf_pack_conv_weights": (_ci, [_vp, _vp, _ci, _ci, _vp]),
    "sf_dwconv_fwd": (_ci, [_CD] + [_vp] * 7),
    "sf_conv_wgrad_splits": (_ci, [_CD]),
    "sf_conv_wgrad": (_ci, [_CD, _vp, _vp, _ci, _ci, _vp, _vp]),
    "sf_conv_wgrad_bx_splits": (_ci, [_CD]),
    "sf_conv_wgrad_bx_ws_floats": (_cl, [_CD, _ci, _ci]),
    "sf_conv_wgrad_bx": (_ci, [_CD, _vp, _vp, _vp, _ci, _ci, _vp, _vp, _vp, _vp]),
    "sf_conv_wgrad_grouped_splits": (_ci, [_CD, _ci]),
    "sf_conv_wgrad_grouped": (_ci, [_CD, _ci, _vp, _vp, _ci, _ci, _vp, _vp]),
    "sf_conv_wgrad_finish": (_ci, [_vp, _ci, _ci, _ci, _ci, _ci, _ci, _vp, _ci, _vp]),
    "sf_dwconv_dgrad": (_ci, [_CD, _vp, _ci, _ci, _vp, _vp, _ci, _ci, _ci, _vp]),
    "sf_dwconv_wgrad_ws_floats": (_cl, [_CD, _ci]),
    "sf_dwconv_wgrad": (_ci, [_CD, _vp, _vp, _ci, _ci, _ci, _vp, _vp, _vp]),
    "sf_dwconv_wgrad_param": (_ci, [_CD, _vp, _vp, _ci, _ci, _ci, _vp, _ci, _vp, _vp]),
    "sf_dwconv_dgrad_epi": (_ci, [_CD] + _VIEW * 2 + [_vp, _vp, _ci, _vp, _ci, _ci, _ci, _ci, _vp]),
    "sf_pool_fwd": (_ci, [_PD, _vp, _vp, _vp]),
    "sf_maxpool_fwd_arg": (_ci, [_PD, _vp, _vp, _vp, _vp]),
    "sf_maxpool_bwd_arg": (_ci, [_PD, _vp] + _VIEW * 2 + [_ci, _vp]),
    "sf_maxpool_bwd": (_ci, [_PD, _vp, _vp] + _VIEW * 2 + [_vp]),
    "sf_maxpool_bwd_first": (_ci, [_PD, _vp, _vp] + _VIEW * 2 + [_vp]),
    "sf_avgpool_win_fwd": (_ci, [_PD, _vp, _vp, _vp]),
    "sf_avgpool_win_bwd": (_ci, [_PD] + _VIEW * 2 + [_ci, _vp]),
    "sf_tmax_mean_ws_floats": (_cl, [_ci, _ci]),
    "sf_tmax_mean": (_ci, _VIEW + [_ci] * 6 + [_vp, _vp, _vp]),
    "sf_gate_apply": (_ci, _VIEW + [_ci] * 6 + [_vp, _vp, _vp, _vp, _ci] + _VIEW + [_vp]),
    "sf_tmax_dot": (_ci, _VIEW + [_ci] * 6 + _VIEW + [_vp, _vp, _vp]),
    "sf_eca_bwd_apply": (_ci, _VIEW + [_ci] * 6 + _VIEW + [_vp, _vp] + _VIEW + [_vp]),
    "sf_eca_gate_bwd": (_ci, [_vp, _vp, _vp, _ci, _ci, _cf, _vp, _vp, _vp, _vp]),
    "sf_attn_fwd": (_ci, _ATTN_FWD + [_vp]),
    "sf_attn_fwd_ws_floats": (_cl, [_ci] * 3),
    "sf_attn_products_per_fp32": (_ci, [_ci]),
    "sf_attn_fwd_ws": (_ci, _ATTN_FWD + [_vp, _vp]),
    "sf_attn_bwd": (_ci, [_vp, _ci] * 4 + [_vp, _vp, _vp] + [_vp, _ci] * 3 + [_ci] * 4 + [_vp]),
    "sf_attn_bwd_fused_ws_floats": (_cl, [_ci] * 3),
    "sf_attn_bwd_fused": (_ci, [_vp, _ci] * 4 + [_vp, _vp, _vp] + [_vp, _ci] * 3 + [_ci] * 3 + [_vp, _vp]),
    "sf_attn_bwd_variant": (_ci, [_ci] * 3),
    "sf_attn_tune": (_ci, [_ci, _ci]),
    "sf_xattn_accepts": (_ci, [_cl, _cl, _ci, _ci]),
    "sf_xattn_bwd_ws_floats": (_cl, [_ci, _cl, _cl, _ci, _ci]),
    "sf_xattn_fwd": (_ci, [_vp, _ci] * 4 + [_vp, _ci, _cl, _cl, _ci, _ci, _cf, _vp]),
    "sf_xattn_bwd": (_ci, [_vp, _ci] * 4 + [_vp, _vp] + [_vp, _ci] * 3 + [_ci, _ci, _cl, _cl, _ci, _ci, _cf, _vp, _vp]),
    "sf_assoc_accepts": (_ci, [_cl, _cl, _ci, _ci]),
    "sf_gram_splits": (_ci, [_ci, _cl, _ci, _ci]),
    "sf_gram_ws_floats": (_cl, [_ci, _cl, _ci, _ci]),
    "sf_gram": (_ci, [_vp, _ci, _vp, _ci, _vp, _vp, _ci, _cl, _ci, _ci, _cf, _vp, _vp]),
    "sf_rowmat": (_ci, [_vp, _ci, _vp, _vp, _ci, _ci, _cl, _ci, _ci, _cf, _ci, _vp]),
    "sf_channel_stats_ws_floats": (_cl, [_ci]),
    "sf_channel_stats": (_ci, _VIEW + [_cl, _ci, _vp, _vp, _vp, _vp]),
    "sf_bn_train_stats": (_ci, _VIEW + [_cl, _ci, _vp, _vp, _cf, _cf] + [_vp] * 9),
    "sf_bn_train_stats_split": (_ci, _VIEW + [_ci, _cl, _ci, _ci, _vp, _vp, _cf, _cf] + [_vp] * 9),
    "sf_bn_train_stats_merge": (_ci, [_vp, _ci, _ci, _vp, _vp, _cf, _cf] + [_vp] * 8),
    "sf_affine_fwd": (_ci, _VIEW + [_ci] * 5 + [_vp, _vp] + _VIEW + [_ci, _ci] + _VIEW + [_ci, _vp]),
    "sf_affine_fwd_split": (_ci, _VIEW + [_ci] * 6 + [_vp, _vp] + _VIEW + [_ci, _ci] + _VIEW + [_ci, _vp]),
    "sf_affine_fwd_mask": (_ci, _VIEW + [_ci] * 5 + [_vp, _vp] + _VIEW + [_ci] + _VIEW + [_vp, _vp]),
    "sf_bn_bwd_ws_floats": (_cl, [_ci]),
    "sf_bn_bwd_reduce": (_ci, _BN_BWD + [_vp]),
    "sf_bn_bwd_reduce_acc": (_ci, _BN_BWD + [_vp, _vp, _vp]),
    "sf_bn_bwd_reduce_split": (_ci, _BN_BWD_SPLIT + [_vp]),
    "sf_bn_bwd_apply": (_ci, _BN_BWD + _BN_APPLY_TAIL),
    "sf_bn_bwd_apply_first": (_ci, _BN_BWD + _BN_APPLY_TAIL),
    "sf_bn_bwd_apply_split": (_ci, _BN_BWD_SPLIT + _BN_APPLY_TAIL),
    "sf_bn_frozen_bwd": (_ci, _VIEW * 3 + [_ci] * 7 + [_vp] * 3 + _VIEW * 2 + [_ci] + [_vp] * 4),
    "sf_head_act_mean": (_ci, [_vp, _ci, _ci, _ci, _ci, _vp, _vp]),
    "sf_head_act_mean_bwd": (_ci, [_vp, _vp, _ci, _ci, _ci, _ci, _vp, _ci, _vp]),
    "sf_copy_channels": (_ci, _VIEW * 2 + [_ci, _cl, _ci, _vp]),
    "sf_channel_shuffle": (_ci, _VIEW * 2 + [_ci, _cl, _ci, _ci, _vp]),
    "sf_gather_add": (_ci, _VIEW + [_ci] + _VIEW + [_cl, _ci, _ci, _vp]),
    "sf_bcast_add": (_ci, _VIEW + [_ci, _cl, _ci, _vp, _cf, _vp]),
    "sf_rowdot": (_ci, _VIEW * 2 + [_cl, _ci, _cf, _vp, _vp]),
    "sf_axpy": (_ci, _VIEW + [_cf] + _VIEW + [_cl, _ci, _ci, _vp]),
    "sf_act_bwd": (_ci, _VIEW * 2 + [_ci] + _VIEW + [_cl, _ci, _ci, _vp]),
    "sf_sigmoid_bwd": (_ci, [_vp, _vp, _vp, _cl, _ci, _vp]),
    "sf_row_softmax_fwd": (_ci, _VIEW + [_cl, _ci, _cf, _vp]),
    "sf_row_softmax_bwd": (_ci, _VIEW * 2 + [_cl, _ci, _cf, _vp]),
    "sf_roi_tpool_fwd": (_ci, _VIEW + [_ci] * 5 + [_vp, _vp]),
    "sf_roi_align_max_fwd": (_ci, [_vp] + [_ci] * 4 + [_vp, _ci, _ci, _cf, _ci] + _VIEW + [_vp, _vp]),
    "sf_roi_align_max_bwd": (_ci, _VIEW + [_vp, _vp] + [_ci] * 7 + [_cf, _ci] + _VIEW + [_ci, _vp]),
    "sf_epilogue_bwd": (_ci, _VIEW * 2 + [_ci] * 6 + [_vp, _ci] + _VIEW + [_ci] + _VIEW + [_ci, _vp]),
    "sf_epilogue_bwd_act": (_ci, _VIEW * 2 + [_ci] * 6 + [_vp, _ci, _ci] + _VIEW + [_ci] + _VIEW + [_ci, _vp]),
    "sf_cam_weights": (_ci, _VIEW + [_ci] * 5 + [_vp, _vp]),
    "sf_cam_map_ws_floats": (_cl, [_ci] * 4),
    "sf_cam_map": (_ci, _VIEW + [_vp] + [_ci] * 5 + [_vp, _vp, _vp, _vp]),
    "sf_ctx_pool_parts": (_ci, [_cl]),
    "sf_ctx_pool_ws_floats": (_cl, [_ci, _cl, _ci]),
    "sf_ctx_pool_fwd": (_ci, _VIEW + [_ci, _cl, _ci] + [_vp] * 6),
    "sf_ctx_pool_bwd": (_ci, _VIEW + [_ci, _cl, _ci] + [_vp] * 5 + _VIEW + [_ci, _vp, _vp, _ci, _vp, _vp]),
    "sf_sample_affine_ws_floats": (_cl, [_ci, _cl, _ci]),
    "sf_sample_affine_fwd": (_ci, _VIEW + [_ci, _cl, _ci, _vp, _vp] + _VIEW + [_vp]),
    "sf_sample_affine_bwd": (_ci, _VIEW * 2 + [_ci, _cl, _ci, _vp] + _VIEW + [_ci, _vp, _vp, _vp, _vp]),
    "sf_stripe_pool_fwd": (_ci, _VIEW + [_ci] * 7 + _VIEW + [_vp, _vp]),
    "sf_stripe_add_fwd": (_ci, _VIEW * 2 + [_ci] * 6 + _VIEW + [_vp]),
    "sf_stripe_pool_bwd": (_ci, _VIEW * 3 + [_vp] + [_ci] * 6 + _VIEW + [_ci, _vp]),
    "sf_ce_topk": (_ci, [_vp, _ci, _vp, _ci, _ci, _ci, _vp, _vp, _pi, _ci, _vp, _vp]),
    "sf_sgd_chunk_elems": (_ci, []),
    "sf_sgd_step": (_ci, [_vp, _vp, _ci, _vp, _vp, _ci, _vp, _vp, _ci, _vp, _ci, _vp]),
    "sf_bce": (_ci, [_vp, _ci, _vp, _ci, _ci, _ci, _ci, _vp, _vp, _pi, _ci, _vp, _vp]),
    "sf_adam_step": (_ci, [_vp, _vp, _ci, _vp, _vp, _ci, _vp, _vp, _ci, _vp, _ci, _vp]),
    "sf_topk_errors": (_ci, [_vp, _ci, _vp, _ci, _ci, _ci, _vp, _pi, _ci, _vp]),
    "sf_rows_append": (_ci, [_vp, _ci, _vp, _ci, _ci, _ci, _vp, _vp, _pi, _ci, _vp]),
    "sf_map_ws_bytes": (_cl, [_ci, _ci]),
    "sf_map": (_ci, [_vp, _ci, _vp, _ci, _ci, _ci, _vp, _vp, _vp, _vp]),
    "sf_confusion_small_kmax": (_ci, []),
    "sf_confusion_update": (_ci, [_vp, _ci, _vp, _ci, _ci, _ci, _vp, _vp, _vp, _vp]),
    "sf_class_report": (_ci, [_vp, _vp, _ci, _vp, _vp, _vp]),
}
EXPORTS = list(_SIGNATURES)


def lib_path():
    return _LIB_PATH


def lib():
    global _lib
    if _lib is None:
        if not os.path.exists(_LIB_PATH):
            raise SfhipError(
                "libsfhip.so not found at %s — build it with `make -C efficient-slowfast_amd/csrc` "
                "(there is no CPU fallback for the SlowFast hot path)" % _LIB_PATH)
        L = ctypes.CDLL(_LIB_PATH)
        for name, (restype, argtypes) in _SIGNATURES.items():
            try:
                fn = getattr(L, name)
            except AttributeError:
                raise SfhipError("%s does not export %s — rebuild it with `make -C efficient-slowfast_amd/csrc`" % (
                    _LIB_PATH, name))
            fn.restype, fn.argtypes = restype, argtypes
        _lib = L
    return _lib


def _check(rc, what):
    if rc != 0:
        raise SfhipError("%s failed: %s" % (what, _ERR.get(rc, rc)))


CALLS = 0


def _stream():
    global CALLS
    CALLS += 1
    return ctypes.c_void_p(torch.cuda.current_stream().cuda_stream)


def _ptr(t):
    return ctypes.c_void_p(t.data_ptr()) if t is not None else None


def _slice_base(a):
    return ctypes.c_void_p(a.buf.data_ptr() + 4 * a.coff)


EVENT_TRACE = None


def _traced(tag, fn):
    if EVENT_TRACE is None:
        return fn()
    e0 = torch.cuda.Event(enable_timing=True)
    e1 = torch.cuda.Event(enable_timing=True)
    e0.record()
    rc = fn()
    e1.record()
    EVENT_TRACE.append((tag, e0, e1))
    return rc


def _call(name, *args, tag=None, what=None, allow=()):
    fn = getattr(lib(), name)
    if tag is None:
        rc = fn(*args, _stream())
    else:
        rc = _traced(tag, lambda: fn(*args, _stream()))
    if rc not in allow:
        _check(rc, what or name)
    return rc


def _require_gpu(t, what):
    if not t.is_cuda:
        raise SfhipError("%s: tensor is on %s — the SlowFast hot path only runs on an MI355X GPU "
                         "(no CPU fallback)" % (what, t.device))
    if t.dtype != torch.float32:
        raise SfhipError("%s: expected float32, got %s" % (what, t.dtype))
    if t.device.index != torch.cuda.current_device():
        raise SfhipError("%s: tensor is on %s but the current device is cuda:%d — call torch.cuda.set_device(%d) (one "
                         "process per GPU)" % (what, t.device, torch.cuda.current_device(), t.device.index))


class Act(object):
    __slots__ = ("buf", "coff", "C")

    def __init__(self, buf, coff=0, C=None):
        assert buf.dim() == 5 and buf.is_contiguous()
        self.buf = buf
        self.coff = coff
        self.C = buf.shape[4] - coff if C is None else C

    N = property(lambda s: s.buf.shape[0])
    T = property(lambda s: s.buf.shape[1])
    H = property(lambda s: s.buf.shape[2])
    W = property(lambda s: s.buf.shape[3])
    cs = property(lambda s: s.buf.shape[4])
    rows = property(lambda s: s.buf.shape[0] * s.buf.shape[1] * s.buf.shape[2] * s.buf.shape[3])

    def slice(self, off, C):
        assert 0 <= off and off + C <= self.C
        return Act(self.buf, self.coff + off, C)

    def ptr(self):
# ... 546 lines not shown
    if out is None:
        out = new_act(x, x.N, To, Ho, Wo, cout)
    else:
        assert (out.N, out.T, out.H, out.W) == (x.N, To, Ho, Wo)
    d = _conv_desc(x, (To, Ho, Wo), out.cs, out.coff, cout, kernel, stride, padding, cin_pad=wpitch, act=_act(relu),
                   res=res, out_cmul=out_cmul)
    nbytes = 4 * (x.rows * c + out.rows * cout * (2 if res is not None else 1))
    _call("sf_dwconv_fwd", ctypes.byref(d), x.ptr(), _ptr(wp), _ptr(scale), _ptr(bias),
          res.ptr() if res is not None else None, out.ptr(), tag=("dwconv", nbytes, taps, c))
    return out


def _pool_desc(x, out_thw, out_cs, out_coff, kernel, stride, padding, avg):
    return PoolDesc(x.N, x.T, x.H, x.W, x.C, x.cs, x.coff, out_thw[0], out_thw[1], out_thw[2], out_cs, out_coff,
                    kernel[0], kernel[1], kernel[2], stride[0], stride[1], stride[2],
                    padding[0], padding[1], padding[2], 1 if avg else 0)


def pool(x, kernel, stride, padding=(0, 0, 0), avg=False, out=None, out_reserve=(0, 0), want_arg=False):
    _require_gpu(x.buf, "pool")
    To, Ho, Wo = _out_thw(x, kernel, stride, padding)
    if out is None:
        out = new_act(x, x.N, To, Ho, Wo, x.C, out_reserve[0], out_reserve[1])
    else:
        assert (out.N, out.T, out.H, out.W, out.C) == (x.N, To, Ho, Wo, x.C)
    d = _pool_desc(x, (To, Ho, Wo), out.cs, out.coff, kernel, stride, padding, avg)
    if want_arg and not avg:
        ok = (x.C % 4 == 0 and x.cs % 4 == 0 and x.coff % 4 == 0 and out.cs % 4 == 0 and out.coff % 4 == 0 and
              kernel[0] * kernel[1] * kernel[2] <= 255 and x.buf.data_ptr() % 16 == 0 and out.buf.data_ptr() % 16 == 0)
        if ok:
            arg = torch.empty((out.rows, x.C), dtype=torch.uint8, device=x.buf.device)
            _call("sf_maxpool_fwd_arg", ctypes.byref(d), x.ptr(), out.ptr(), _ptr(arg))
            return out, arg
    _call("sf_pool_fwd", ctypes.byref(d), x.ptr(), out.ptr())
    return (out, None) if want_arg else out


def tmax_mean(x, alpha):
    _require_gpu(x.buf, "tmax_mean")
    pooled = torch.empty((x.N, x.C), dtype=torch.float32, device=x.buf.device)
    ws = torch.empty((lib().sf_tmax_mean_ws_floats(x.N, x.C),), dtype=torch.float32, device=x.buf.device)
    _call("sf_tmax_mean", x.ptr(), x.cs, x.coff, x.N, x.T, x.H, x.W, x.C, alpha, _ptr(pooled), _ptr(ws))
    return pooled


def gate_apply(x, alpha, pooled, w3=None, scale=None, bias=None, relu=False, out=None):
    _require_gpu(x.buf, "gate_apply")
    if out is None:
        out = new_act(x, x.N, x.T // alpha, x.H, x.W, x.C)
    else:
        assert (out.N, out.T, out.H, out.W, out.C) == (x.N, x.T // alpha, x.H, x.W, x.C), (out, x)
    _call("sf_gate_apply", x.ptr(), x.cs, x.coff, x.N, x.T, x.H, x.W, x.C, alpha, _ptr(pooled), _ptr(w3),
          _ptr(scale), _ptr(bias), ACT_RELU if relu else ACT_NONE, out.ptr(), out.cs, out.coff)
    return out


def attention(q, k, v, x, gamma, scale=None, bias=None, relu=False, alpha=1, out=None, save=None):
    _require_gpu(x.buf, "attention")
    if out is None:
        out = new_act(x, x.N, x.T * alpha, x.H, x.W, x.C)
    else:
        assert (out.N, out.T, out.H, out.W, out.C) == (x.N, x.T * alpha, x.H, x.W, x.C), (out, x)
    o_save = lse_save = None
    if save is not None:
        n = x.T * x.H * x.W
        o_save = save["o"] = torch.empty((x.N, n, x.C), dtype=torch.float32, device=x.buf.device)
        lse_save = save["lse"] = torch.empty((x.N, n), dtype=torch.float32, device=x.buf.device)
    ws = torch.empty((lib().sf_attn_fwd_ws_floats(x.N, x.T * x.H * x.W, x.C),), dtype=torch.float32,
                     device=x.buf.device)
    _call("sf_attn_fwd_ws", _slice_base(q), q.cs, _slice_base(k), k.cs, _slice_base(v), v.cs, _slice_base(x), x.cs,
          _ptr(gamma), _ptr(scale), _ptr(bias), ACT_RELU if relu else ACT_NONE, out.ptr(), out.cs, out.coff,
          x.N, x.T, x.H, x.W, x.C, alpha, _ptr(o_save), _ptr(lse_save), _ptr(ws),
          tag=("attn", x.N, x.T * x.H * x.W, x.C))
    return out


def head_act_mean(logits, act):
    assert logits.coff == 0 and logits.C == logits.cs
    out = torch.empty((logits.N, logits.C), dtype=torch.float32, device=logits.buf.device)
    _call("sf_head_act_mean", logits.ptr(), logits.N, logits.T * logits.H * logits.W, logits.C, act, _ptr(out))
    return out


def copy_channels(x, out, out_cmul=1):
    assert x.rows == out.rows
    _call("sf_copy_channels", x.ptr(), x.cs, x.coff, out.ptr(), out.cs, out.coff, out_cmul, x.rows, x.C)
    return out


def channel_shuffle(x, out, groups, accumulate=False):
    assert x.rows == out.rows and x.C == out.C and x.C % groups == 0
    _call("sf_channel_shuffle", x.ptr(), x.cs, x.coff, out.ptr(), out.cs, out.coff, groups, x.rows, x.C,
          1 if accumulate else 0)
    return out


def channel_stats(x):
    _require_gpu(x.buf, "channel_stats")
    dev = x.buf.device
    mean = torch.empty((x.C,), dtype=torch.float32, device=dev)
    var = torch.empty((x.C,), dtype=torch.float32, device=dev)
    ws = torch.empty((lib().sf_channel_stats_ws_floats(x.C),), dtype=torch.float32, device=dev)
    _call("sf_channel_stats", x.ptr(), x.cs, x.coff, x.rows, x.C, _ptr(mean), _ptr(var), _ptr(ws))
    return mean, var


def affine(x, scale=None, bias=None, res=None, relu=False, rep=1, out=None, out_reserve=(0, 0), out_cmul=1,
           nsplit=1, mask=None):
    _require_gpu(x.buf, "affine")
    if out is None:
        out = new_act(x, x.N, x.T * rep, x.H, x.W, x.C, out_reserve[0], out_reserve[1])
    else:
        assert (out.N, out.T, out.H, out.W) == (x.N, x.T * rep, x.H, x.W), (out, x, rep)
        assert out.coff + (x.C - 1) * out_cmul < out.cs and (out_cmul > 1 or out.C == x.C), (out, x)
    if res is not None:
        assert res.rows == x.rows and res.C == x.C
    head = (x.ptr(), x.cs, x.coff, x.N, x.T, x.H, x.W, x.C)
    mid = (_ptr(scale), _ptr(bias), res.ptr() if res is not None else None, res.cs if res is not None else 0,
           res.coff if res is not None else 0, _act(relu))
    if (mask is not None and relu and rep == 1 and nsplit == 1 and out_cmul == 1 and x.C % 4 == 0 and
            x.cs % 4 == 0 and x.coff % 4 == 0 and out.cs % 4 == 0 and out.coff % 4 == 0 and
            x.rows * (x.C // 4) < 2 ** 31 - 1 and scale is not None and
            (res is None or (res.cs % 4 == 0 and res.coff % 4 == 0))):
        mk = torch.empty((x.rows * (x.C // 4),), dtype=torch.uint8, device=x.buf.device)
        _call("sf_affine_fwd_mask", *head, *mid, out.ptr(), out.cs, out.coff, _ptr(mk))
        mask["bytes"] = mk
        return out
    tail = mid + (rep, out.ptr(), out.cs, out.coff, out_cmul)
    if nsplit == 1:
        _call("sf_affine_fwd", *head, *tail)
    else:
        _call("sf_affine_fwd_split", *head, nsplit, *tail)
    return out


def conv_dgrad(dz, wt_packed, x_like, kernel, stride=(1, 1, 1), padding=(0, 0, 0), dilation=(1, 1, 1),
               out=None, accumulate=False, dz_planes=None):
    _require_gpu(dz.buf, "conv_dgrad")
    cin, taps, cout_pad = wt_packed.shape
    if out is None:
        out = new_act(dz, x_like.N, x_like.T, x_like.H, x_like.W, cin)
        accumulate = False
    assert (out.N, out.T, out.H, out.W, out.C) == (x_like.N, x_like.T, x_like.H, x_like.W, cin), (out, x_like)
    if max(stride) > 1 and tuple(dilation) == (1, 1, 1) and (accumulate or (out.coff == 0 and out.cs == out.C)):
        return _conv_dgrad_strided(dz, wt_packed, out, kernel, stride, padding, accumulate, dz_planes)
    d = _conv_desc(dz, (out.T, out.H, out.W), out.cs, out.coff, cin, kernel, stride, padding, dilation,
                   cin_pad=cout_pad, res=out if accumulate else None, transposed=1)
    _conv_launch(d, dz.ptr(), _ptr(wt_packed), None, None, out.ptr() if accumulate else None, out.ptr(),
                 dz.buf.device, "sf_conv_fwd(transposed)", w_tensor=wt_packed, in_planes=dz_planes)
    return out



def _residue_taps(k, s, p, a):
    pairs = sorted(((a + p - kk) // s, kk) for kk in range(k) if (a + p - kk) % s == 0)
    return [o for o, _ in pairs], [kk for _, kk in pairs]


_TAP_INDEX = {}


def _class_weights(wt_packed, store, kernel, stride, padding):
    cin, taps, cout_pad = wt_packed.shape
    kT, kH, kW = kernel
    fam = (tuple(kernel), tuple(stride), tuple(padding))
    classes = []
    for at in range(stride[0]):
        tt = _residue_taps(kT, stride[0], padding[0], at)[1]
        for ah in range(stride[1]):
            th = _residue_taps(kH, stride[1], padding[1], ah)[1]
            for aw in range(stride[2]):
                tw = _residue_taps(kW, stride[2], padding[2], aw)[1]
                if tt and th and tw:
                    classes.append(((at, ah, aw) + fam, [(a * kH + b) * kW + c for a in tt for b in th for c in tw]))
    ikey = (cin, taps, fam, str(wt_packed.device))
    idx = _TAP_INDEX.get(ikey)
    if idx is None:
        rows = [ci * taps + t for _, sel in classes for ci in range(cin) for t in sel]
        idx = _TAP_INDEX[ikey] = torch.tensor(rows, dtype=torch.long, device=wt_packed.device)
    allrows = wt_packed.view(cin * taps, cout_pad).index_select(0, idx)
    off = 0
    for key, sel in classes:
        n = cin * len(sel)
        store[key] = allrows[off:off + n].view(cin, len(sel), cout_pad)
        off += n
    return store


def _conv_dgrad_strided(dz, wt_packed, out, kernel, stride, padding, accumulate, dz_planes=None):
    cin, _, cout_pad = wt_packed.shape
    kT, kH, kW = kernel
    every = all(_residue_taps(k, s, p, a)[1] and (full - a + s - 1) // s > 0
                for k, s, p, full in zip(kernel, stride, padding, (out.T, out.H, out.W)) for a in range(s))
    add = accumulate or not every
    if not accumulate and not every:
        out.buf.zero_()
    for at in range(stride[0]):
        ot, tt = _residue_taps(kT, stride[0], padding[0], at)
        for ah in range(stride[1]):
            oh, th = _residue_taps(kH, stride[1], padding[1], ah)
            for aw in range(stride[2]):
                ow, tw = _residue_taps(kW, stride[2], padding[2], aw)
                dims = [(full - a + s - 1) // s for full, a, s in zip((out.T, out.H, out.W), (at, ah, aw), stride)]
                if not (tt and th and tw) or min(dims) <= 0:
                    continue
                store = wt_packed.__dict__.setdefault("_sf_classes", {})
                key = (at, ah, aw, tuple(kernel), tuple(stride), tuple(padding))
                wsub = store.get(key)
                if wsub is None:
                    wsub = _class_weights(wt_packed, store, kernel, stride, padding)[key]
                d = _conv_desc(dz, dims, out.cs, out.coff, cin, (len(tt), len(th), len(tw)), (1, 1, 1),
                               (-ot[0], -oh[0], -ow[0]), cin_pad=cout_pad, res=out,
                               scatter=(stride[0], stride[1], stride[2], at, ah, aw, out.T, out.H, out.W))
                _conv_launch(d, dz.ptr(), _ptr(wsub), None, None, out.ptr() if add else None, out.ptr(),
                             dz.buf.device, "sf_conv_fwd(strided dgrad class)", w_tensor=wsub, in_planes=dz_planes)
    return out




def conv_wgrad(x, dz, cout, kernel, stride=(1, 1, 1), padding=(0, 0, 0), dilation=(1, 1, 1), cin=None,
               cin_pad=None, finish_into=None, x_planes=None, dz_planes=None):
    _require_gpu(x.buf, "conv_wgrad")
    cin = x.C if cin is None else cin
    cin_pad = _pad16(cin) if cin_pad is None else cin_pad
    kT, kH, kW = kernel
    d = _conv_desc(x, (dz.T, dz.H, dz.W), 0, 0, cout, kernel, stride, padding, dilation, cin=cin, cin_pad=cin_pad)
    tag = ("conv", dz.rows, kT * kH * kW * cin, cout)
    nws = lib().sf_conv_wgrad_bx_ws_floats(ctypes.byref(d), 1 if x_planes is not None else 0,
                                           1 if dz_planes is not None else 0) if cin_pad == cin else 0
    if nws > 0:
        S = lib().sf_conv_wgrad_bx_splits(ctypes.byref(d))
        part = torch.empty((S, cout, kT * kH * kW, cin_pad), dtype=torch.float32, device=x.buf.device)
        ws = torch.empty((nws,), dtype=torch.float32, device=x.buf.device)
        if _call("sf_conv_wgrad_bx", ctypes.byref(d), x.ptr(), _ptr(x_planes), dz.ptr(), dz.cs, dz.coff,
                 _ptr(dz_planes), _ptr(part), _ptr(ws), tag=tag, allow=_REFUSED) != 0:
            nws = 0
    if nws <= 0:
        S = lib().sf_conv_wgrad_splits(ctypes.byref(d))
        part = torch.empty((S, cout, kT * kH * kW, cin_pad), dtype=torch.float32, device=x.buf.device)
        _call("sf_conv_wgrad", ctypes.byref(d), x.ptr(), dz.ptr(), dz.cs, dz.coff, _ptr(part), tag=tag)
    if finish_into is not None:
        dst, real_cin, fold_kw = finish_into
        assert dst.is_contiguous() and dst.dtype == torch.float32
        if S > 128 and cout * kT * kH * kW * cin_pad > 65536:
            part, S = part.sum(0, keepdim=True), 1
        assert dst.numel() == cout * real_cin * kT * kH * kW * max(fold_kw, 1), (dst.shape, cout, real_cin, kernel)
        _call("sf_conv_wgrad_finish", _ptr(part), S, cout, kT * kH * kW, cin_pad, real_cin, fold_kw, _ptr(dst), 1)
        return None
    return part.sum(0) if S > 1 else part[0]


def conv_grouped(x, wp, groups, kernel, stride=(1, 1, 1), padding=(0, 0, 0), dilation=(1, 1, 1), scale=None,
                 bias=None, relu=False, res=None, out=None, shuffle=False, out_reserve=(0, 0)):
    _require_gpu(x.buf, "conv_grouped")
    cout, taps, cin_pad = wp.shape
    To, Ho, Wo = _out_thw(x, kernel, stride, padding, dilation)
    if out is None:
        out = new_act(x, x.N, To, Ho, Wo, cout, out_reserve[0], out_reserve[1])
    assert (out.N, out.T, out.H, out.W, out.C) == (x.N, To, Ho, Wo, cout), (out, (x.N, To, Ho, Wo, cout))
    assert x.C % groups == 0 and cout % groups == 0 and cin_pad >= x.C // groups, (x, wp.shape, groups)
    d = _conv_desc(x, (To, Ho, Wo), out.cs, out.coff, cout, kernel, stride, padding, dilation, cin_pad=cin_pad,
                   act=_act(relu), res=res)
    if res is not None:
        assert res.rows == out.rows and res.C == cout
    _call("sf_conv_fwd_grouped", ctypes.byref(d), groups, 1 if shuffle else 0, x.ptr(), _ptr(wp), _ptr(scale),
          _ptr(bias), res.ptr() if res is not None else None, out.ptr(),
          tag=("conv", d.N * d.To * d.Ho * d.Wo, taps * (x.C // groups), cout))
    return out


def conv_dgrad_grouped(dz, wtp, groups, x_like, kernel, stride=(1, 1, 1), padding=(0, 0, 0), dilation=(1, 1, 1),
                       out=None, accumulate=False):
    _require_gpu(dz.buf, "conv_dgrad_grouped")
    cin, taps, cout_pad = wtp.shape
    if out is None:
        out = new_act(dz, x_like.N, x_like.T, x_like.H, x_like.W, cin)
        accumulate = False
    assert (out.N, out.T, out.H, out.W, out.C) == (x_like.N, x_like.T, x_like.H, x_like.W, cin), (out, x_like)
    assert dz.C % groups == 0 and cin % groups == 0 and cout_pad >= dz.C // groups
    d = _conv_desc(dz, (out.T, out.H, out.W), out.cs, out.coff, cin, kernel, stride, padding, dilation,
                   cin_pad=cout_pad, res=out if accumulate else None, transposed=1)
    _call("sf_conv_fwd_grouped", ctypes.byref(d), groups, 0, dz.ptr(), _ptr(wtp), None, None,
          out.ptr() if accumulate else None, out.ptr(), tag=("conv", dz.rows, taps * (dz.C // groups), cin),
          what="sf_conv_fwd_grouped(transposed)")
    return out


def conv_wgrad_grouped(x, dz, groups, kernel, stride=(1, 1, 1), padding=(0, 0, 0), dilation=(1, 1, 1),
                       cin_pad=None, finish_into=None):
    _require_gpu(x.buf, "conv_wgrad_grouped")
    cin_g, cout = x.C // groups, dz.C
    assert x.C % groups == 0 and cout % groups == 0
    cin_pad = _pad16(cin_g) if cin_pad is None else cin_pad
    kT, kH, kW = kernel
    d = _conv_desc(x, (dz.T, dz.H, dz.W), 0, 0, cout, kernel, stride, padding, dilation, cin_pad=cin_pad)
    S = lib().sf_conv_wgrad_grouped_splits(ctypes.byref(d), groups)
    if S <= 0:
        raise SfhipError("sf_conv_wgrad_grouped_splits: %d -> %d channels in %d groups" % (x.C, cout, groups))
    part = torch.empty((S, cout, kT * kH * kW, cin_pad), dtype=torch.float32, device=x.buf.device)
    _call("sf_conv_wgrad_grouped", ctypes.byref(d), groups, x.ptr(), dz.ptr(), dz.cs, dz.coff, _ptr(part),
          tag=("conv", dz.rows, kT * kH * kW * cin_g, cout))
    if finish_into is not None:
        dst = finish_into
        assert dst.is_contiguous() and dst.dtype == torch.float32 and dst.numel() == cout * cin_g * kT * kH * kW
        _call("sf_conv_wgrad_finish", _ptr(part), S, cout, kT * kH * kW, cin_pad, cin_g, 0, _ptr(dst), 1)
        return None
    return part.sum(0) if S > 1 else part[0]


def unpack_conv_weight_grad(dwp, shape):
    cout, cin, kT, kH, kW = shape
    return dwp[:, :, :cin].permute(0, 2, 1).reshape(cout, cin, kT, kH, kW).contiguous()


def _bn_bwd_y(who, y, z, relu, mask, plain):
    if mask is not None and relu:
        if not plain or mask.numel() != z.rows * (z.C // 4) or not mask.is_cuda:
            raise SfhipError("%s: the byte mask holds rows * C/4 bytes of an un-repeated, un-split layer" % who)
        return _ptr(mask), z.C // 4, 0, 3
    code = 2 if relu == 6 else (1 if relu else 0)
    return (y.ptr(), y.cs, y.coff, code) if y is not None else (None, 0, 0, code)


def bn_bwd(dy, y, z, mean, invstd, gamma, relu, rep=1, dres=None, dz_out=None, dgamma_out=None, nsplit=1,
           sync=None, grad_sink=None, mask=None, dres_overwrite=False):
    C = z.C
    dev = z.buf.device
    mean, invstd, gamma = mean.contiguous(), invstd.contiguous(), gamma.detach().contiguous()
    dbeta = torch.empty((nsplit * C,), dtype=torch.float32, device=dev)
    dgamma = torch.empty((nsplit * C,), dtype=torch.float32, device=dev)
    ws = torch.empty((lib().sf_bn_bwd_ws_floats(C),), dtype=torch.float32, device=dev)
    yp, ycs, yco, code = _bn_bwd_y("bn_bwd", y, z, relu, mask, rep == 1 and nsplit == 1)
    head = (dy.ptr(), dy.cs, dy.coff, yp, ycs, yco, z.ptr(), z.cs, z.coff, z.N, z.T, z.H, z.W, C)
    tail = (rep, code, _ptr(mean), _ptr(invstd))
    split = (nsplit,) if nsplit > 1 else ()
    reduce_fn = "sf_bn_bwd_reduce_split" if nsplit > 1 else "sf_bn_bwd_reduce"
    apply_fn = "sf_bn_bwd_apply_split" if nsplit > 1 else "sf_bn_bwd_apply"
    if dres_overwrite:
        assert dres is not None and nsplit == 1
        apply_fn = "sf_bn_bwd_apply_first"
    if grad_sink is not None:
        assert nsplit == 1 and dgamma_out is None
        _call("sf_bn_bwd_reduce_acc", *head, *tail, _ptr(dbeta), _ptr(dgamma), _ptr(ws), _ptr(grad_sink[1]),
              _ptr(grad_sink[0]))
    else:
        _call(reduce_fn, *head, *split, *tail, _ptr(dbeta), _ptr(dgamma), _ptr(ws))
    db_apply, dg_apply = (dbeta, dgamma) if sync is None else sync(dbeta, dgamma)
    out = z if dz_out is None else dz_out
    _call(apply_fn, *head, *split, *tail, _ptr(gamma), _ptr(db_apply), _ptr(dg_apply), out.ptr(), out.cs, out.coff,
          dres.ptr() if dres is not None else None, dres.cs if dres is not None else 0,
          dres.coff if dres is not None else 0)
    if dgamma_out is not None:
        if nsplit > 1:
            dgamma_out[0][:C] = dgamma.view(nsplit, C).sum(0)
            dgamma_out[1][:C] = dbeta.view(nsplit, C).sum(0)
        else:
            dgamma_out[0][:C] = dgamma
            dgamma_out[1][:C] = dbeta
    return out, dgamma, dbeta


def bn_frozen_bwd(dy, y, z, mean, invstd, gamma, relu, rep=1, dres=None, dres_overwrite=False, dz_out=None,
                  grads=None, mask=None):
    if dy is None or z is None or (relu and mask is None and y is None):
        raise SfhipError("bn_frozen_bwd: dy, z and (with an activation) y or its mask are required")
    for name, a in (("dy", dy), ("z", z), ("dz", dz_out), ("dres", dres), ("y", y if (relu and mask is None) else None)):
        if a is not None:
            _require_gpu(a.buf, "bn_frozen_bwd(%s)" % name)
    C, dev = z.C, z.buf.device
    if dres is not None and rep != 1:
        raise SfhipError("bn_frozen_bwd: the residual's gradient is only defined without a T repeat (rep = %d)" % rep)
    if (dy.N, dy.T, dy.H, dy.W, dy.C) != (z.N, z.T * rep, z.H, z.W, C):
        raise SfhipError("bn_frozen_bwd: dy %r does not match z %r repeated %d times" % (dy, z, rep))
    vecs = [("mean", mean), ("invstd", invstd)] + ([("gamma", gamma)] if gamma is not None else [])
    for name, v in vecs:
        _require_gpu(v, "bn_frozen_bwd(%s)" % name)
        if v.numel() < C or not v.is_contiguous():
            raise SfhipError("bn_frozen_bwd: %s must be a contiguous tensor of at least %d floats" % (name, C))
    dgp = dbp = ws = None
    if grads is not None:
        for name, v in (("dgamma", grads[0]), ("dbeta", grads[1])):
            _require_gpu(v, "bn_frozen_bwd(%s)" % name)
            if v.numel() < C or not v.is_contiguous():
                raise SfhipError("bn_frozen_bwd: %s must be a contiguous tensor of at least %d floats" % (name, C))
        dgp, dbp = _ptr(grads[0]), _ptr(grads[1])
        ws = torch.empty((lib().sf_bn_bwd_ws_floats(C),), dtype=torch.float32, device=dev)
    yp, ycs, yco, code = _bn_bwd_y("bn_frozen_bwd", y if relu else None, z, relu, mask, rep == 1)
    out = z if dz_out is None else dz_out
    _call("sf_bn_frozen_bwd", dy.ptr(), dy.cs, dy.coff, yp, ycs, yco, z.ptr(), z.cs, z.coff, z.N, z.T, z.H, z.W, C,
          rep, code, _ptr(mean.detach()), _ptr(invstd.detach()), _ptr(gamma.detach()) if gamma is not None else None,
          out.ptr(), out.cs, out.coff, dres.ptr() if dres is not None else None,
          dres.cs if dres is not None else 0, dres.coff if dres is not None else 0, 0 if dres_overwrite else 1,
          dbp, dgp, _ptr(ws))
    return out


def maxpool_bwd(x, y, dy, dx, kernel, stride, padding=(0, 0, 0), overwrite=False):
    d = _pool_desc(x, (y.T, y.H, y.W), y.cs, y.coff, kernel, stride, padding, False)
    _call("sf_maxpool_bwd_first" if overwrite else "sf_maxpool_bwd", ctypes.byref(d), x.ptr(), y.ptr(), dy.ptr(),
          dy.cs, dy.coff, dx.ptr(), dx.cs, dx.coff)
    return dx


def maxpool_bwd_arg(x_like, arg, dy, dx, kernel, stride, padding=(0, 0, 0), overwrite=False):
    if not (dy.cs % 4 == 0 and dy.coff % 4 == 0 and dx.cs % 4 == 0 and dx.coff % 4 == 0 and
            dy.buf.data_ptr() % 16 == 0 and dx.buf.data_ptr() % 16 == 0):
        return False
    d = _pool_desc(x_like, (dy.T, dy.H, dy.W), dy.cs, dy.coff, kernel, stride, padding, False)
    _call("sf_maxpool_bwd_arg", ctypes.byref(d), _ptr(arg), dy.ptr(), dy.cs, dy.coff, dx.ptr(), dx.cs, dx.coff,
          1 if overwrite else 0)
    return True


def tmax_dot(x, alpha, dz):
    out = torch.empty((x.N, x.C), dtype=torch.float32, device=x.buf.device)
    ws = torch.empty((lib().sf_tmax_mean_ws_floats(x.N, x.C),), dtype=torch.float32, device=x.buf.device)
    _call("sf_tmax_dot", x.ptr(), x.cs, x.coff, x.N, x.T, x.H, x.W, x.C, alpha, dz.ptr(), dz.cs, dz.coff,
          _ptr(out), _ptr(ws))
    return out


def eca_bwd_apply(x, alpha, dz, gate, dpool, dx):
    _call("sf_eca_bwd_apply", x.ptr(), x.cs, x.coff, x.N, x.T, x.H, x.W, x.C, alpha, dz.ptr(), dz.cs, dz.coff,
          _ptr(gate), _ptr(dpool), dx.ptr(), dx.cs, dx.coff)
    return dx


def eca_gate_bwd(dg, pooled, w3, dpool_scale, dw3):
    n, c = pooled.shape
    gate = torch.empty_like(pooled)
    dpool = torch.empty_like(pooled)
    _call("sf_eca_gate_bwd", _ptr(dg), _ptr(pooled), _ptr(w3), n, c, float(dpool_scale), _ptr(gate), _ptr(dpool),
          _ptr(dw3))
    return gate, dpool


def bcast_add(g, v, scale):
    _call("sf_bcast_add", g.ptr(), g.cs, g.coff, g.N, g.T * g.H * g.W, g.C, _ptr(v), float(scale))
    return g


def rowdot(a, b, scale=1.0):
    out = torch.empty((a.rows,), dtype=torch.float32, device=a.buf.device)
    _call("sf_rowdot", a.ptr(), a.cs, a.coff, b.ptr(), b.cs, b.coff, a.rows, a.C, float(scale), _ptr(out))
    return out


def axpy(a, out, alpha=1.0, accumulate=True):
    assert a.rows == out.rows and a.C == out.C
    _call("sf_axpy", a.ptr(), a.cs, a.coff, float(alpha), out.ptr(), out.cs, out.coff, a.rows, a.C,
          1 if accumulate else 0)
    return out


def row_softmax(x, scale=1.0):
    _require_gpu(x.buf, "row_softmax")
    _call("sf_row_softmax_fwd", x.ptr(), x.cs, x.coff, x.rows, x.C, float(scale))
    return x


def row_softmax_bwd(p, dp, scale=1.0):
    assert p.rows == dp.rows and p.C == dp.C
    _call("sf_row_softmax_bwd", p.ptr(), p.cs, p.coff, dp.ptr(), dp.cs, dp.coff, p.rows, p.C, float(scale))
    return dp


def act_bwd(dy, y, relu, dx, accumulate=True):
    assert dy.rows == y.rows == dx.rows and dy.C == y.C == dx.C
    _call("sf_act_bwd", dy.ptr(), dy.cs, dy.coff, y.ptr(), y.cs, y.coff, _act(relu), dx.ptr(), dx.cs, dx.coff,
          dy.rows, dy.C, 1 if accumulate else 0)
    return dx


def attention_bwd(q, k, v, dz, o, lse, gamma, dq, dk, dv, workspace=True):
    B, n, C = o.shape
    o_act = Act(o.view(B, 1, 1, n, C))
    dvec = rowdot(Act(dz.buf.view(B, 1, 1, n, dz.cs), dz.coff, C), o_act)
    args = (_slice_base(q), q.cs, _slice_base(k), k.cs, _slice_base(v), v.cs, _slice_base(dz), dz.cs, _ptr(lse),
            _ptr(dvec), _ptr(gamma), _slice_base(dq), dq.cs, _slice_base(dk), dk.cs, _slice_base(dv), dv.cs, B, n, C)
    nws = lib().sf_attn_bwd_fused_ws_floats(B, n, C) if workspace else 0
    if nws > 0:
        ws = torch.empty((nws,), dtype=torch.float32, device=o.device)
        _call("sf_attn_bwd_fused", *args, _ptr(ws), tag=("attn_bwd_fused", B, n, C))
        return dvec
    for which, tag in ((1, "attn_bwd_dq"), (2, "attn_bwd_dkv")):
        _call("sf_attn_bwd", *args, which, tag=(tag, B, n, C))
    return dvec


def xattn_accepts(q, k, v):
    nq, nk = q.T * q.H * q.W, k.T * k.H * k.W
    if not lib().sf_xattn_accepts(nq, nk, q.C, v.C):
        return False
    return all(a.cs % 4 == 0 and a.coff % 4 == 0 and a.buf.data_ptr() % 16 == 0 for a in (q, k, v))
# ... 441 lines not shown
```

### efficient-slowfast_amd/slowfast/models/engine.py

```python
import os
import threading
import weakref

import torch
import torch.nn as nn

import sfhip
from sfhip import Act

_tls = threading.local()


class internal(object):

    def __enter__(self):
        self.prev = getattr(_tls, "depth", 0)
        _tls.depth = self.prev + 1

    def __exit__(self, *a):
        _tls.depth = self.prev


def is_internal():
    return getattr(_tls, "depth", 0) > 0


def enter(xs):
    return [x if isinstance(x, Act) else sfhip.from_ncthw(x) for x in xs]


def leave(acts):
    if is_internal():
        return acts
    return [sfhip.to_ncthw(a) for a in acts]


class Tape(object):

    def __init__(self):
        self.ops = []
        self.gbuf = {}
        self.pgrads = {}
        self.out_act = None
        self.sink = None
        self.side = None
        self.serial = getattr(_tls, "serial", False)
        self.input_ids = {}
        self.input_grads = {}
        self.joins = set()
        self.model = None
        self.capturing = False
        self.arena = None
        self.arena_off = 0
        self.zero_floats = -1
        self.armed = True
        self.param_grads = True

    def pgrad_target(self, param):
        if self.sink is None:
            return None
        g = self.sink.get(param)
        return g if g is not None and g.is_contiguous() else None

    def grad_of(self, act):
        key = act.buf.data_ptr()
        g = self.gbuf.get(key)
        if g is None:
            n = act.buf.numel()
            nal = (n + 63) // 64 * 64
            if self.zero_floats >= 0:
                self.zero_floats += nal
            if self.arena is not None and self.arena_off + nal <= self.arena.numel() and \
                    self.arena.device == act.buf.device:
                g = self.arena[self.arena_off:self.arena_off + n]
                self.arena_off += nal
            else:
                g = torch.zeros(n, dtype=torch.float32, device=act.buf.device)
            self.gbuf[key] = g
        return Act(g.view(act.buf.shape), act.coff, act.C)

    def has_grad(self, act):
        return act.buf.data_ptr() in self.gbuf

    def grad_dst(self, act, whole=True):
        key = act.buf.data_ptr()
        if not whole or key in self.gbuf or act.coff != 0 or act.cs != act.C:
            return self.grad_of(act), True
        g = torch.empty(act.buf.numel(), dtype=torch.float32, device=act.buf.device)
        self.gbuf[key] = g
        return Act(g.view(act.buf.shape), 0, act.C), False

    def record(self, fn):
        self.ops.append((fn, self.side))

    def add_pgrad(self, param, g):
        g = g.reshape(param.shape)
        tgt = self.sink.get(param) if self.sink is not None else None
        if tgt is not None:
            tgt.add_(g)
            return
        cur = self.pgrads.get(param)
        self.pgrads[param] = g if cur is None else cur + g

    def add_pgrads(self, params, grads):
        tgts = [self.sink.get(p) if self.sink is not None else None for p in params]
        if all(t is not None for t in tgts) and len(tgts) > 1:
            torch._foreach_add_(tgts, [g.reshape(p.shape) for p, g in zip(params, grads)])
            return
        for p, g in zip(params, grads):
            self.add_pgrad(p, g)

    def _replay(self):
        for fn, side in reversed(self.ops):
            if side is None:
                fn()
            else:
                with torch.cuda.stream(side):
                    fn()

    def backward(self):
        self._open_arena()
        self.capturing = bool(torch.cuda.is_available() and torch.cuda.is_current_stream_capturing())
        asked = -1
        try:
            self._replay()
            for wg in self.joins:
                _sync_streams(wg, torch.cuda.current_stream(wg.device))
            asked = self.zero_floats
        finally:
            self.joins = set()
            self.ops = []
            self.zero_floats = -1
            self.gbuf = {}
            self.arena = None
            self.arena_off = 0
            self.capturing = False
        if self.model is not None and asked >= 0:
            self.model.__dict__["_sf_arena_floats"] = asked

    def _open_arena(self):
        self.zero_floats = 0
        if self.model is None or self.out_act is None:
            return
        want = self.model.__dict__.get("_sf_arena_floats", 0)
        if 0 < want <= ARENA_MAX_FLOATS:
            self.arena = torch.zeros(want, dtype=torch.float32, device=self.out_act.buf.device)
            self.arena_off = 0


def tape():
    t = getattr(_tls, "tape", None)
    return t if t is None or t.armed else None


class EvalTape(Tape):

    def __init__(self, target):
        super(EvalTape, self).__init__()
        self.armed = False
        self.param_grads = False
        self.target = target
        self.target_acts = None
        self.out = None
        self.dout = None

    def pgrad_target(self, param):
        return None

    def add_pgrad(self, param, g):
        pass

    def add_pgrads(self, params, grads):
        pass

    def backward(self, dout):
        if self.target_acts is None or self.out is None:
            raise RuntimeError("the eval tape saw no boundary named %r, or no head output" % (self.target,))
        self.dout = dout.contiguous()
        try:
            self._replay()
            return [self.grad_of(a) for a in self.target_acts]
        finally:
            self.ops = []
            self.gbuf = {}
            self.dout = None


class eval_taping(object):

    def __init__(self, target):
        self.t = EvalTape(target)

    def __enter__(self):
        self.prev = getattr(_tls, "tape", None)
        _tls.tape = self.t
        return self.t

    def __exit__(self, *a):
        _tls.tape = self.prev


def boundary(name, x):
    t = getattr(_tls, "tape", None)
    if isinstance(t, EvalTape) and not t.armed and name == t.target:
        join_pending(x[0].buf.device)
        t.target_acts = list(x)
        t.armed = True
    return x


_MILESTONE_HOOKS = weakref.WeakKeyDictionary()


def set_milestone_hook(fn, model):
    if fn is None:
        _MILESTONE_HOOKS.pop(model, None)
    else:
        _MILESTONE_HOOKS[model] = fn


def milestone(name):
    t = tape()
    if t is None or t.model is None:
        return
    hook = _MILESTONE_HOOKS.get(t.model)
    if hook is not None:
        t.record(lambda: hook(name, t))


OVERLAP_PATHS = os.environ.get("SF_OVERLAP_PATHS", "1") != "0"
_SIDE = {}


def _side_stream(device):
    s = _SIDE.get(device)
    if s is None:
        s = _SIDE[device] = torch.cuda.Stream(device=device)
    return s


_COMPANION = {}


def _companion_stream(parent):
    key = (parent.device, parent.cuda_stream)
    s = _COMPANION.get(key)
    if s is None:
        s = _COMPANION[key] = torch.cuda.Stream(device=parent.device)
    return s


def _sync_streams(first, then):
    ev = torch.cuda.Event()
    ev.record(first)
    then.wait_event(ev)


def run_paths(fns, device, defer_join=False):
    if not OVERLAP_PATHS or getattr(_tls, "serial", False) or len(fns) != 2 or device.type != "cuda":
        return [f() for f in fns]
    t = tape()
    if t is not None and t.side is not None:
        return [f() for f in fns]
    main, side = torch.cuda.current_stream(device), _side_stream(device)

    def bwd_join():
        _sync_streams(side, torch.cuda.current_stream(device))

    def bwd_fork():
        _sync_streams(torch.cuda.current_stream(device), side)

    if t is not None:
        t.record(bwd_join)
    _sync_streams(main, side)
    out0 = fns[0]()
    with torch.cuda.stream(side):
        if t is not None:
            t.side = side
        try:
            out1 = fns[1]()
        finally:
            if t is not None:
                t.side = None
    if not defer_join:
        _sync_streams(side, main)
        _tls.pending_side = None
    else:
        _tls.pending_side = side
    if t is not None:
        t.record(bwd_fork)
    return [out0, out1]


def join_pending(device):
    pend = getattr(_tls, "pending_side", None)
    if pend is not None:
        _sync_streams(pend, torch.cuda.current_stream(device))
        _tls.pending_side = None


class taping(object):
    def __init__(self, t):
        self.t = t

    def __enter__(self):
        self.prev = getattr(_tls, "tape", None)
        _tls.tape = self.t

    def __exit__(self, *a):
        _tls.tape = self.prev


def _colsum(act):
    mean, _ = sfhip.channel_stats(act)
    return mean * float(act.rows)


def _record_conv(x, conv_weight, conv_bias, wp_shape, gsrc, kernel, stride, padding, dilation, x_needs_grad=True,
                 cin=None, unpack=None, fold_kw=0):
    t = tape()
    if t is None:
        return
    cout = conv_weight.shape[0]

    def wgrad(g):
        tgt = t.pgrad_target(conv_weight)
        if tgt is not None:
            real_cin = conv_weight.shape[1]
            sfhip.conv_wgrad(x, g, cout, kernel, stride, padding, dilation, cin=cin, cin_pad=wp_shape[2],
                             finish_into=(tgt, real_cin, fold_kw))
        else:
            dwp = sfhip.conv_wgrad(x, g, cout, kernel, stride, padding, dilation, cin=cin, cin_pad=wp_shape[2])
            t.add_pgrad(conv_weight, unpack(dwp) if unpack else sfhip.unpack_conv_weight_grad(dwp, conv_weight.shape))
        if conv_bias is not None:
            t.add_pgrad(conv_bias, _colsum(g))

    def bwd():
        g = gsrc() if callable(gsrc) else gsrc
        dev = x.buf.device
        if not t.param_grads:
            pass
        elif OVERLAP_PATHS and not t.capturing and not t.serial and x_needs_grad and dev.type == "cuda":
            cur = torch.cuda.current_stream(dev)
            wg = _companion_stream(cur)
            _sync_streams(cur, wg)
            with torch.cuda.stream(wg):
                wgrad(g)
            g.buf.record_stream(wg)
            x.buf.record_stream(wg)
            t.joins.add(wg)
        else:
            wgrad(g)
        if x_needs_grad:
            if conv_weight.dim() == 5 and tuple(conv_weight.shape[2:]) == tuple(kernel):
                wtp = _packed_pair(conv_weight)[1]
            else:
                wtp = _cached_t(conv_weight, "_sf_wtp", _key(conv_weight),
                                lambda: sfhip.pack_conv_weight(conv_weight.detach().reshape(
                                    conv_weight.shape[0], conv_weight.shape[1], *kernel).transpose(0, 1).contiguous()))
            dx, acc = t.grad_dst(x)
            sfhip.conv_dgrad(g, wtp, x, kernel, stride, padding, dilation, out=dx, accumulate=acc)

    t.record(bwd)


_PCACHE = {}


_CAPTURE_KEEP = {}


def _keep_if_capturing(obj):
    if getattr(_tls, "capturing", False):
        _CAPTURE_KEEP[id(obj)] = obj
    return obj


def _cached_t(tensor, slot, key, make):
    store = tensor.__dict__.setdefault("_sf_cache", {})
    c = store.get(slot)
    if c is None or c[0] != key:
        with torch.no_grad():
            c = (key, make())
        store[slot] = c
    return _keep_if_capturing(c[1])


_PARAM_EPOCH = 0


def parameters_changed(*_unused):
    global _PARAM_EPOCH
    _PARAM_EPOCH += 1


def replay(graph):
    graph.replay()
    parameters_changed()


try:
    from torch.optim.optimizer import register_optimizer_step_post_hook as _register_step_hook
    _STEP_HOOK = _register_step_hook(lambda optimizer, args, kwargs: parameters_changed())
except ImportError:
    _STEP_HOOK = None


def _key(*tensors):
    return (_PARAM_EPOCH,) + tuple((t.data_ptr(), t._version) for t in tensors if t is not None)


def _cached(mod, slot, key, make):
    c = mod.__dict__.get(slot)
    if c is None or c[0] != key:
        with torch.no_grad():
            c = (key, make())
        mod.__dict__[slot] = c
    return _keep_if_capturing(c[1])


def check_bn(bn):
    from .batchnorm_helper import SubBatchNorm3d
    if not isinstance(bn, (nn.BatchNorm3d, SubBatchNorm3d)):
        raise NotImplementedError("unsupported normalisation layer on the HIP path: %s" % type(bn))


def _sub_bn(bn):
    from .batchnorm_helper import SubBatchNorm3d
    return isinstance(bn, SubBatchNorm3d)


def _sync_bn(bn):
    from .batchnorm_helper import NaiveSyncBatchNorm3d
    from slowfast.utils import distributed as du
    return isinstance(bn, NaiveSyncBatchNorm3d) and du.get_local_size() > 1


_NBT = None


def _bump(counter):
    if _NBT is not None:
        _NBT.append(counter)
    else:
        counter.add_(1)


def _plain_bn(bn):
    return not _sub_bn(bn) and not _sync_bn(bn)


def _bn_train_stats(bn, z, conv_stats=None):
    if _sub_bn(bn):
        S, sb = bn.num_splits, bn.split_bn
        if z.N % S != 0:
            raise ValueError("SubBatchNorm3d: batch %d is not divisible by num_splits %d" % (z.N, S))
        dev = z.buf.device
        w = bn.weight.detach().repeat(S) if bn.affine else torch.ones(S * z.C, device=dev)
        b = bn.bias.detach().repeat(S) if bn.affine else torch.zeros(S * z.C, device=dev)
        track = sb.track_running_stats and sb.running_mean is not None
        m = sb.momentum if sb.momentum is not None else 1.0 / float(int(sb.num_batches_tracked) + 1)
        mean, invstd, scale, shift = sfhip.bn_train_stats(
            z, w, b, sb.eps, m, sb.running_mean if track else None, sb.running_var if track else None, nsplit=S)
        if track:
            _bump(sb.num_batches_tracked)
        return mean, invstd, scale, shift, S, w, None
    track = bn.track_running_stats and bn.running_mean is not None
    m = bn.momentum if bn.momentum is not None else 1.0 / float(int(bn.num_batches_tracked) + 1)
    if _sync_bn(bn):
        from .batchnorm_helper import group_gather_sum
        nd, ng = bn.num_sync_devices, bn.num_groups
        lmean, lvar = sfhip.channel_stats(z)
        lm = lmean.double()
        vec = group_gather_sum(torch.cat([lm, lvar.double() + lm * lm]), nd, ng) / nd
        mean64, meansqr = vec[:z.C], vec[z.C:]
        var64 = (meansqr - mean64 * mean64).clamp_min(0.0)
        mean, var = mean64.float(), var64.float()
        invstd = torch.rsqrt(var64 + bn.eps).float()
        scale = (bn.weight.detach() * invstd).contiguous()
        shift = (bn.bias.detach() - mean * scale).contiguous()
        if track:
            bn.running_mean += m * (mean - bn.running_mean)
            bn.running_var += m * (var - bn.running_var)
            bn.__dict__.pop("_sf_affine", None)

        def sync(dbeta, dgamma):
            tot = group_gather_sum(torch.cat([dbeta, dgamma]).double(), nd, ng) / nd
            return tot[:dbeta.numel()].float().contiguous(), tot[dbeta.numel():].float().contiguous()

        return mean, invstd, scale, shift, 1, bn.weight, sync
    if conv_stats is not None:
        mean, invstd, scale, shift = sfhip.bn_train_stats_merge(
            conv_stats, z.C, bn.weight, bn.bias, bn.eps, m, bn.running_mean if track else None,
            bn.running_var if track else None)
    else:
        mean, invstd, scale, shift = sfhip.bn_train_stats(
            z, bn.weight, bn.bias, bn.eps, m, bn.running_mean if track else None, bn.running_var if track else None)
    if track:
        bn.__dict__.pop("_sf_affine", None)
        _bump(bn.num_batches_tracked)
    return mean, invstd, scale, shift, 1, bn.weight, None


def _bn_epilogue(bn, z, scale, shift, make_backward, res, relu, rep, out, out_reserve, keep, out_cmul, nsplit=1,
                 eager_sums=False, always_sums=False):
    zz = z if keep is None else z.slice(0, keep)
    if keep is not None:
        assert nsplit == 1, "channel-sliced BN (GhostModule) is only defined for plain BatchNorm3d"
        scale, shift = scale[:keep], shift[:keep]
    t = tape()
    shuffled = t is not None and out_cmul != 1
    mk = {} if (t is not None and relu) else None
    dst = {} if shuffled else dict(out=out, out_reserve=out_reserve, out_cmul=out_cmul)
    y = sfhip.affine(zz, scale.contiguous(), shift.contiguous(), res=res, relu=relu, rep=rep, nsplit=nsplit, mask=mk,
                     **dst)
    if t is not None:
        mask = mk.get("bytes") if mk else None
        weight, bias = getattr(bn, "weight", None), getattr(bn, "bias", None)
        affine = weight is not None and bias is not None
        backward = make_backward()

        def zeros():
            return torch.zeros(z.C, dtype=torch.float32, device=z.buf.device)

        made = (zeros(), zeros()) if eager_sums else None

        def bwd():
            dres, acc = None, True
            if res is not None:
                dres, acc = t.grad_dst(res, whole=nsplit == 1 and res.C == zz.C and rep == 1)
            sink = sums = None
            if always_sums or (affine and t.param_grads):
                wt, bt = (t.pgrad_target(weight), t.pgrad_target(bias)) if (affine and nsplit == 1) else (None, None)
                if wt is not None and bt is not None:
                    sink = (wt, bt)
                else:
                    sums = made or (zeros(), zeros())
            backward(t.grad_of(y), y, zz, dres, acc, sink, sums, mask)
            if keep is not None and keep < z.C:
                rest = z.slice(keep, z.C - keep)
                sfhip.axpy(rest, rest, alpha=0.0, accumulate=False)
            if sums is not None and affine:
                t.add_pgrad(weight, sums[0])
                t.add_pgrad(bias, sums[1])

        t.record(bwd)
    if shuffled:
        return copy_channels(y, out, out_cmul=out_cmul)
    return y


def bn_train_apply(bn, z, res=None, relu=False, rep=1, out=None, out_reserve=(0, 0), keep=None, out_cmul=1,
                   conv_stats=None):
    check_bn(bn)
    with torch.no_grad():
        mean, invstd, scale, shift, nsplit, gamma_b, sync = _bn_train_stats(bn, z, conv_stats)
    sel = slice(None) if nsplit > 1 else slice(0, z.C if keep is None else keep)

    def backward(dy, y, zz, dres, dres_accumulate, sink, sums, mask):
        sfhip.bn_bwd(dy, y, zz, mean[sel], invstd[sel], gamma_b[sel], relu, rep=rep, dres=dres, dz_out=zz,
                     dgamma_out=sums, nsplit=nsplit, sync=sync, grad_sink=sink, mask=mask,
                     dres_overwrite=not dres_accumulate)

    return _bn_epilogue(bn, z, scale, shift, lambda: backward, res, relu, rep, out, out_reserve, keep, out_cmul,
                        nsplit=nsplit, eager_sums=not _GRAD_SINK, always_sums=True)


def bn_affine(bn, conv_bias=None):
    check_bn(bn)
    stat = bn.bn if _sub_bn(bn) else bn
    w = getattr(bn, "weight", None)
    b = getattr(bn, "bias", None)

    def make():
        inv = 1.0 / torch.sqrt(stat.running_var + stat.eps)
        scale = w * inv if w is not None else inv
        bias = -stat.running_mean * scale
        if b is not None:
            bias = bias + b
        if conv_bias is not None:
            bias = bias + scale * conv_bias
        return scale.detach().contiguous(), bias.detach().contiguous()

    return _cached(bn, "_sf_affine", _key(w, b, stat.running_mean, stat.running_var, conv_bias), make)


def _taped_training():
    t = tape()
    return t is not None and not isinstance(t, EvalTape)


def bn_unfused(bn):
    return bn.training or _taped_training()


def bn_apply(bn, z, conv_stats=None, **kw):
    if bn.training:
        return bn_train_apply(bn, z, conv_stats=conv_stats, **kw)
    return bn_frozen_apply(bn, z, **kw)


def _bn_frozen_stats(bn):
    stat = bn.bn if _sub_bn(bn) else bn
    return _cached(bn, "_sf_frozen", _key(stat.running_mean, stat.running_var),
                   lambda: (stat.running_mean.detach().float().contiguous(),
                            (1.0 / torch.sqrt(stat.running_var + stat.eps)).detach().contiguous()))


def bn_frozen_apply(bn, z, res=None, relu=False, rep=1, out=None, out_reserve=(0, 0), keep=None, out_cmul=1):
    check_bn(bn)
    scale, shift = bn_affine(bn)

    def make_backward():
        mean, invstd = _bn_frozen_stats(bn)
        weight = getattr(bn, "weight", None)

        def backward(dy, y, zz, dres, dres_accumulate, sink, sums, mask):
            sfhip.bn_frozen_bwd(dy, y, zz, mean, invstd, weight, relu, rep=rep, dres=dres,
                                dres_overwrite=not dres_accumulate, dz_out=zz,
                                grads=sink if sink is not None else sums, mask=mask)

        return backward

    return _bn_epilogue(bn, z, scale, shift, make_backward, res, relu, rep, out, out_reserve, keep, out_cmul)


def norm_forward(bn, x):
    (a,) = enter([x])
    if bn.training:
        y = bn_train_apply(bn, a)
    elif _taped_training():
        y = bn_frozen_apply(bn, a)
    else:
        y = sfhip.affine(a, *bn_affine(bn))
    return leave([y])[0]


ARENA_MAX_FLOATS = 64 << 18
_GROUPS_OF = {}
_PAIR_WEIGHTS = {}


def _packed_pair(weight):
    if not weight.is_cuda:
        return sfhip.pack_conv_weight(weight), None
    if id(weight) not in _PAIR_WEIGHTS:
        wid = id(weight)
        _PAIR_WEIGHTS[wid] = weakref.ref(weight, lambda _r, wid=wid: _PAIR_WEIGHTS.pop(wid, None))
    return _cached_t(weight, "_sf_wpair", _key(weight), lambda: sfhip.pack_conv_weight_pair(weight))


def repack_all(model):
    cand = model.__dict__.get("_sf_pair_params")
    if cand is None or cand[0] != len(_PAIR_WEIGHTS):
        cand = (len(_PAIR_WEIGHTS), [p for p in model.parameters()
                                     if id(p) in _PAIR_WEIGHTS and _PAIR_WEIGHTS[id(p)]() is p])
        model.__dict__["_sf_pair_params"] = cand
    stale, old, slots = [], [], []
    for w in cand[1]:
        store = w.__dict__.get("_sf_cache", {})
        c = store.get("_sf_wpair")
        if c is not None and c[0] != _key(w) and w.is_cuda and w.is_contiguous():
            stale.append(w.detach())
            old.append(c[1])
            slots.append((w, "_sf_wpair", None))
        c = store.get("_sf_wgroups")
        G = _GROUPS_OF.get(id(w))
        if c is not None and G and c[0] != _key(w) and w.is_cuda and w.is_contiguous():
            wd, (wp, wtp) = w.detach(), c[1]
            cout_g, cin_g = wd.shape[0] // G, wd.shape[1]
            for g in range(G):
                stale.append(wd[g * cout_g:(g + 1) * cout_g])
                old.append((wp[g * cout_g:(g + 1) * cout_g], wtp[g * cin_g:(g + 1) * cin_g]))
                slots.append((w, "_sf_wgroups", (wp, wtp)) if g == 0 else None)
    if len(stale) < 2:
        return
    with torch.no_grad():
        new = sfhip.pack_conv_weight_pairs(stale, old)
    for sl, o, prev in zip(slots, new, old):
        if sl is None:
            continue
        w, name, whole = sl
        if whole is not None and (o[0].data_ptr() != prev[0].data_ptr() or o[1].data_ptr() != prev[1].data_ptr()):
            continue
        w.__dict__["_sf_cache"][name] = (_key(w), _keep_if_capturing(o if whole is None else whole))


def packed_weight(conv):
    if conv.groups == 1:
        return _packed_pair(conv.weight)[0]
    if conv.groups == conv.in_channels and conv.out_channels == conv.in_channels:
        if conv.weight.is_cuda:
            return _packed_pair(conv.weight)[1][0]
        return _cached(conv, "_sf_wp", _key(conv.weight), lambda: sfhip.pack_dw_weight(conv.weight))
    return _group_pairs(conv)


def _group_pairs(conv):
    w, G = conv.weight, conv.groups
    if conv.in_channels % G or conv.out_channels % G:
        raise ValueError("grouped conv: %d -> %d channels are not divisible by %d groups" % (
            conv.in_channels, conv.out_channels, G))
    if w.is_cuda and id(w) not in _PAIR_WEIGHTS:
        wid = id(w)
        _PAIR_WEIGHTS[wid] = weakref.ref(w, lambda _r, wid=wid: (_PAIR_WEIGHTS.pop(wid, None), _GROUPS_OF.pop(wid, None)))
        _GROUPS_OF[wid] = G
    return _cached_t(w, "_sf_wgroups", _key(w), lambda: sfhip.pack_grouped_weight_pair(w, G))


def grouped_conv(x, conv, scale=None, bias=None, relu=False, res=None, out=None, out_reserve=(0, 0), shuffle=False):
    k, s, p, d = conv.kernel_size, conv.stride, conv.padding, conv.dilation
    assert x.C == conv.in_channels, (x, conv)
    return sfhip.conv_grouped(x, _group_pairs(conv)[0], conv.groups, k, s, p, d,
                              scale=None if scale is None else scale.contiguous(),
                              bias=None if bias is None else bias.contiguous(), relu=relu, res=res, out=out,
                              shuffle=shuffle, out_reserve=out_reserve)


# ... 484 lines not shown
```

### include/sfhip.h

```cpp
#ifndef SFHIP_H
#define SFHIP_H
#ifdef __cplusplus
extern "C" {
#endif

#define SF_OK 0
#define SF_EINVAL (-1)
#define SF_EALIGN (-2)
#define SF_ELAUNCH (-3)
#define SF_ENOTTAKEN (-4)

#define SF_ACT_NONE 0
#define SF_ACT_RELU 1
#define SF_ACT_SIGMOID 2
#define SF_ACT_SOFTMAX 3
#define SF_ACT_HSIGMOID 4
#define SF_ACT_RELU6 5

int sf_abi_version(void);
const char* sf_build_arch(void);

int sf_ncthw_to_ndhwc(const float* src, float* dst, int N, int C, int T, int H, int W,
                      int cpad, int ph, int pw, int Wp, void* stream);
int sf_ndhwc_to_ncthw(const float* src, int cs, int coff, float* dst, int N, int C, int T, int H,
                      int W, void* stream);

typedef struct sf_conv_desc {
  int N, Ti, Hi, Wi, Cin;
  int in_cs, in_coff;
  int To, Ho, Wo, Cout;
  int out_cs, out_coff;
  int out_cmul;
  int kT, kH, kW, sT, sH, sW, pT, pH, pW, dT, dH, dW;
  int cin_pad;
  int act;
  int res_cs, res_coff;
  int transposed;
  int os_T, os_H, os_W;
  int oo_T, oo_H, oo_W;
  int ob_T, ob_H, ob_W;
} sf_conv_desc;
int sf_conv_fwd(const sf_conv_desc* d, const float* in, const float* w_packed, const float* scale,
                const float* bias, const float* res, float* out, void* stream);
long sf_conv_fwd_ws_floats(const sf_conv_desc* d);
int sf_conv_fwd_ws(const sf_conv_desc* d, const float* in, const float* w_packed, const float* scale,
                   const float* bias, const float* res, float* out, float* ws, void* stream);
int sf_conv_fwd_grouped(const sf_conv_desc* d, int groups, int shuffle, const float* in, const float* w_packed,
                        const float* scale, const float* bias, const float* res, float* out, void* stream);
long sf_conv_stats_ws_floats(const sf_conv_desc* d);
int sf_conv_fwd_stats(const sf_conv_desc* d, const float* in, const float* w_packed, const float* scale,
                      const float* bias, const float* res, float* out, float* stats_ws, int* parts, void* stream);
int sf_conv_tune(int knob, int value);
long sf_bx_planes_elems(long rows, int C);
int sf_bx_split(const float* x, int cs, int coff, long rows, int C, unsigned short* planes, void* stream);
int sf_bx_split_batched(const void* items, const int* blk0, int n, int nblocks, void* stream);
int sf_conv_rows_parts(const sf_conv_desc* d);
long sf_conv_pw_ws_floats(const sf_conv_desc* d, int have_w_planes);
long sf_conv_pw_stats_floats(const sf_conv_desc* d);
int sf_conv_fwd_pw(const sf_conv_desc* d, const float* in, const float* w_packed, const unsigned short* w_planes,
                   const float* scale, const float* bias, const float* res, float* out, float* ws, float* stats,
                   int* parts, void* stream);
long sf_conv_bx_ws_floats(const sf_conv_desc* d, int have_in_planes, int have_w_planes);
int sf_conv_fwd_bx(const sf_conv_desc* d, const float* in, const unsigned short* in_planes, const float* w_packed,
                   const unsigned short* w_planes, const float* scale, const float* bias, const float* res, float* out,
                   float* ws, void* stream);
int sf_pack_conv_weight(const float* w, int Cout, int Cin, int taps, float* wp, int cin_pad, float* wtp,
                        int cout_pad, void* stream);
int sf_pack_conv_weights(const void* items, const int* blk0, int n, int nblocks, void* stream);

int sf_dwconv_fwd(const sf_conv_desc* d, const float* in, const float* w_packed, const float* scale,
                  const float* bias, const float* res, float* out, void* stream);

typedef struct sf_pool_desc {
  int N, Ti, Hi, Wi, C, in_cs, in_coff;
  int To, Ho, Wo, out_cs, out_coff;
  int kT, kH, kW, sT, sH, sW, pT, pH, pW;
  int is_avg;
} sf_pool_desc;
int sf_pool_fwd(const sf_pool_desc* d, const float* in, float* out, void* stream);
int sf_maxpool_fwd_arg(const sf_pool_desc* d, const float* in, float* out, unsigned char* arg, void* stream);
int sf_maxpool_bwd_arg(const sf_pool_desc* d, const unsigned char* arg, const float* dy, int dy_cs, int dy_coff,
                       float* dx, int dx_cs, int dx_coff, int overwrite, void* stream);

long sf_tmax_mean_ws_floats(int N, int C);
int sf_tmax_mean(const float* x, int cs, int coff, int N, int T, int H, int W, int C, int alpha,
                 float* pooled, float* ws, void* stream);
int sf_gate_apply(const float* x, int cs, int coff, int N, int T, int H, int W, int C, int alpha,
                  const float* pooled, const float* w3, const float* scale, const float* bias, int act,
                  float* out, int out_cs, int out_coff, void* stream);

int sf_attn_fwd(const float* q, int q_cs, const float* k, int k_cs, const float* v, int v_cs,
                const float* x, int x_cs, const float* gamma, const float* scale, const float* bias,
                int act, float* out, int out_cs, int out_coff, int B, int T, int H, int W, int C,
                int alpha, float* o_save, float* lse_save, void* stream);

long sf_attn_fwd_ws_floats(int B, int N, int C);
int sf_attn_products_per_fp32(int C);
int sf_attn_fwd_ws(const float* q, int q_cs, const float* k, int k_cs, const float* v, int v_cs,
                   const float* x, int x_cs, const float* gamma, const float* scale, const float* bias,
                   int act, float* out, int out_cs, int out_coff, int B, int T, int H, int W, int C,
                   int alpha, float* o_save, float* lse_save, float* ws, void* stream);

int sf_attn_bwd(const float* q, int q_cs, const float* k, int k_cs, const float* v, int v_cs,
                const float* dz, int dz_cs, const float* lse, const float* dvec, const float* gamma,
                float* dq, int dq_cs, float* dk, int dk_cs, float* dv, int dv_cs, int B, int N, int C,
                int which , void* stream);

long sf_attn_bwd_fused_ws_floats(int B, int N, int C);
int sf_attn_bwd_fused(const float* q, int q_cs, const float* k, int k_cs, const float* v, int v_cs, const float* dz,
                      int dz_cs, const float* lse, const float* dvec, const float* gamma, float* dq, int dq_cs,
                      float* dk, int dk_cs, float* dv, int dv_cs, int B, int N, int C, float* ws, void* stream);

int sf_attn_bwd_variant(int B, int N, int C);
int sf_attn_tune(int knob, int value);

int sf_xattn_accepts(long Nq, long Nk, int d, int dv);
long sf_xattn_bwd_ws_floats(int B, long Nq, long Nk, int d, int dv);
int sf_xattn_fwd(const float* q, int q_cs, const float* k, int k_cs, const float* v, int v_cs, float* y, int y_cs,
                 float* lse, int B, long Nq, long Nk, int d, int dv, float sm_scale, void* stream);
int sf_xattn_bwd(const float* q, int q_cs, const float* k, int k_cs, const float* v, int v_cs, const float* dy,
                 int dy_cs, const float* lse, const float* dvec, float* dq, int dq_cs, float* dk, int dk_cs,
                 float* dv_, int dv_cs, int accumulate_mask, int B, long Nq, long Nk, int d, int dv, float sm_scale,
                 float* ws, void* stream);

int sf_assoc_accepts(long Nq, long Nk, int d, int dv);
int sf_gram_splits(int B, long R, int da, int db);
long sf_gram_ws_floats(int B, long R, int da, int db);
int sf_gram(const float* a, int a_cs, const float* b, int b_cs, float* g, float* gt, int B, long R, int da, int db,
            float alpha, float* ws, void* stream);
int sf_rowmat(const float* x, int x_cs, const float* w, float* y, int y_cs, int B, long R, int k, int n, float alpha,
              int accumulate, void* stream);

long sf_channel_stats_ws_floats(int C);
int sf_channel_stats(const float* x, int cs, int coff, long rows, int C, float* mean, float* var, float* ws,
                     void* stream);
int sf_bn_train_stats(const float* x, int cs, int coff, long rows, int C, const float* gamma, const float* beta,
                      float eps, float momentum, float* run_mean, float* run_var, float* mean, float* var,
                      float* invstd, float* scale, float* shift, float* ws, void* stream);
int sf_bn_train_stats_merge(const float* parts_ws, int parts, int C, const float* gamma, const float* beta, float eps,
                            float momentum, float* run_mean, float* run_var, float* mean, float* var, float* invstd,
                            float* scale, float* shift, void* stream);
int sf_affine_fwd(const float* x, int cs, int coff, int N, int T, int H, int W, int C, const float* scale,
                  const float* bias, const float* res, int res_cs, int res_coff, int act, int rep, float* out,
                  int out_cs, int out_coff, int out_cmul, void* stream);

int sf_head_act_mean(const float* logits, int B, int P, int K, int act, float* out, void* stream);

int sf_copy_channels(const float* in, int in_cs, int in_coff, float* out, int out_cs, int out_coff,
                     int out_cmul, long rows, int C, void* stream);
int sf_channel_shuffle(const float* in, int in_cs, int in_coff, float* out, int out_cs, int out_coff, int groups,
                       long rows, int C, int accumulate, void* stream);

int sf_conv_wgrad_splits(const sf_conv_desc* d);
int sf_conv_wgrad_bx_splits(const sf_conv_desc* d);
long sf_conv_wgrad_bx_ws_floats(const sf_conv_desc* d, int have_x_planes, int have_dz_planes);
int sf_conv_wgrad_bx(const sf_conv_desc* d, const float* x, const unsigned short* x_planes, const float* dz, int dz_cs,
                     int dz_coff, const unsigned short* dz_planes, float* partial, float* ws, void* stream);
int sf_conv_wgrad(const sf_conv_desc* d, const float* x, const float* dz, int dz_cs, int dz_coff,
                  float* partial, void* stream);
int sf_conv_wgrad_grouped_splits(const sf_conv_desc* d, int groups);
int sf_conv_wgrad_grouped(const sf_conv_desc* d, int groups, const float* x, const float* dz, int dz_cs, int dz_coff,
                          float* partial, void* stream);
int sf_conv_wgrad_finish(const float* partial, int S, int Cout, int packed_taps, int cin_pad, int Cin, int fold_kw,
                         float* dst, int accumulate, void* stream);

#define SF_BN_MASK_BYTES 3
long sf_bn_bwd_ws_floats(int C);
int sf_affine_fwd_mask(const float* x, int cs, int coff, int N, int T, int H, int W, int C, const float* scale,
                       const float* bias, const float* res, int res_cs, int res_coff, int act, float* out,
                       int out_cs, int out_coff, unsigned char* mask, void* stream);
int sf_bn_bwd_reduce(const float* dy, int dy_cs, int dy_coff, const float* y, int y_cs, int y_coff,
                     const float* z, int z_cs, int z_coff, int N, int T, int H, int W, int C, int rep, int relu,
                     const float* mean, const float* invstd, float* dbeta, float* dgamma, float* ws, void* stream);
int sf_bn_bwd_reduce_acc(const float* dy, int dy_cs, int dy_coff, const float* y, int y_cs, int y_coff,
                         const float* z, int z_cs, int z_coff, int N, int T, int H, int W, int C, int rep, int relu,
                         const float* mean, const float* invstd, float* dbeta, float* dgamma, float* ws,
                         float* dbeta_acc, float* dgamma_acc, void* stream);
int sf_bn_bwd_apply(const float* dy, int dy_cs, int dy_coff, const float* y, int y_cs, int y_coff,
                    const float* z, int z_cs, int z_coff, int N, int T, int H, int W, int C, int rep, int relu,
                    const float* mean, const float* invstd, const float* gamma, const float* dbeta,
                    const float* dgamma, float* dz, int dz_cs, int dz_coff, float* dres, int dres_cs,
                    int dres_coff, void* stream);
int sf_bn_bwd_apply_first(const float* dy, int dy_cs, int dy_coff, const float* y, int y_cs, int y_coff,
                          const float* z, int z_cs, int z_coff, int N, int T, int H, int W, int C, int rep, int relu,
                          const float* mean, const float* invstd, const float* gamma, const float* dbeta,
                          const float* dgamma, float* dz, int dz_cs, int dz_coff, float* dres, int dres_cs,
                          int dres_coff, void* stream);
int sf_bn_frozen_bwd(const float* dy, int dy_cs, int dy_coff, const float* y, int y_cs, int y_coff,
                     const float* z, int z_cs, int z_coff, int N, int T, int H, int W, int C, int rep, int relu,
                     const float* mean, const float* invstd, const float* gamma, float* dz, int dz_cs, int dz_coff,
                     float* dres, int dres_cs, int dres_coff, int dres_accumulate, float* dbeta, float* dgamma,
                     float* ws, void* stream);

int sf_maxpool_bwd(const sf_pool_desc* d, const float* x, const float* y, const float* dy, int dy_cs,
                   int dy_coff, float* dx, int dx_cs, int dx_coff, void* stream);
int sf_maxpool_bwd_first(const sf_pool_desc* d, const float* x, const float* y, const float* dy, int dy_cs,
                         int dy_coff, float* dx, int dx_cs, int dx_coff, void* stream);

int sf_tmax_dot(const float* x, int cs, int coff, int N, int T, int H, int W, int C, int alpha, const float* dz,
                int dz_cs, int dz_coff, float* out, float* ws, void* stream);
int sf_eca_bwd_apply(const float* x, int cs, int coff, int N, int T, int H, int W, int C, int alpha,
                     const float* dz, int dz_cs, int dz_coff, const float* gate, const float* dpool, float* dx,
                     int dx_cs, int dx_coff, void* stream);

int sf_eca_gate_bwd(const float* dg, const float* pooled, const float* w3, int N, int C, float dpool_scale,
                    float* gate, float* dpool, float* dw3, void* stream);

int sf_dwconv_dgrad(const sf_conv_desc* d, const float* dz, int dz_cs, int dz_coff, const float* w_packed,
                    float* dx, int dx_cs, int dx_coff, int C, void* stream);
long sf_dwconv_wgrad_ws_floats(const sf_conv_desc* d, int C);
int sf_dwconv_wgrad(const sf_conv_desc* d, const float* x, const float* dz, int dz_cs, int dz_coff, int C,
                    float* dw, float* ws, void* stream);
int sf_dwconv_wgrad_param(const sf_conv_desc* d, const float* x, const float* dz, int dz_cs, int dz_coff, int C,
                          float* dw_param, int accumulate, float* ws, void* stream);
int sf_gather_add(const float* in, int in_cs, int in_coff, int in_cmul, float* out, int out_cs, int out_coff,
                  long rows, int C, int accumulate, void* stream);

int sf_bcast_add(float* g, int cs, int coff, int N, long rows_per_n, int C, const float* v, float scale,
                 void* stream);
int sf_rowdot(const float* a, int a_cs, int a_coff, const float* b, int b_cs, int b_coff, long rows, int C,
              float scale, float* out, void* stream);
int sf_axpy(const float* a, int a_cs, int a_coff, float alpha, float* out, int out_cs, int out_coff, long rows,
            int C, int accumulate, void* stream);
int sf_bn_train_stats_split(const float* x, int cs, int coff, int N, long rows_per_sample, int C, int nsplit,
                            const float* gamma, const float* beta, float eps, float momentum, float* run_mean,
                            float* run_var, float* mean, float* var, float* invstd, float* scale, float* shift,
                            float* ws, void* stream);
int sf_affine_fwd_split(const float* x, int cs, int coff, int N, int T, int H, int W, int C, int nsplit,
                        const float* scale, const float* bias, const float* res, int res_cs, int res_coff, int act,
                        int rep, float* out, int out_cs, int out_coff, int out_cmul, void* stream);
int sf_bn_bwd_reduce_split(const float* dy, int dy_cs, int dy_coff, const float* y, int y_cs, int y_coff,
                           const float* z, int z_cs, int z_coff, int N, int T, int H, int W, int C, int nsplit,
                           int rep, int relu, const float* mean, const float* invstd, float* dbeta, float* dgamma,
                           float* ws, void* stream);
int sf_bn_bwd_apply_split(const float* dy, int dy_cs, int dy_coff, const float* y, int y_cs, int y_coff,
                          const float* z, int z_cs, int z_coff, int N, int T, int H, int W, int C, int nsplit,
                          int rep, int relu, const float* mean, const float* invstd, const float* gamma,
                          const float* dbeta, const float* dgamma, float* dz, int dz_cs, int dz_coff, float* dres,
                          int dres_cs, int dres_coff, void* stream);
int sf_act_bwd(const float* dy, int dy_cs, int dy_coff, const float* y, int y_cs, int y_coff, int act, float* dx,
               int dx_cs, int dx_coff, long rows, int C, int accumulate, void* stream);

int sf_row_softmax_fwd(float* x, int cs, int coff, long rows, int C, float scale, void* stream);
int sf_row_softmax_bwd(const float* p, int p_cs, int p_coff, float* dp, int dp_cs, int dp_coff, long rows, int C,
                       float scale, void* stream);

int sf_roi_tpool_fwd(const float* x, int cs, int coff, int N, int T, int H, int W, int C, float* out, void* stream);
int sf_roi_align_max_fwd(const float* x, int N, int H, int W, int C, const float* boxes, int K, int R,
                         float spatial_scale, int aligned, float* out, int out_cs, int out_coff, unsigned char* arg,
                         void* stream);
int sf_roi_align_max_bwd(const float* dy, int dy_cs, int dy_coff, const unsigned char* arg, const float* boxes, int K,
                         int N, int T, int H, int W, int C, int R, float spatial_scale, int aligned, float* dx,
                         int dx_cs, int dx_coff, int accumulate, void* stream);
int sf_sigmoid_bwd(const float* y, const float* dy, float* dx, long n, int accumulate, void* stream);

int sf_avgpool_win_fwd(const sf_pool_desc* d, const float* x, float* out, void* stream);
int sf_avgpool_win_bwd(const sf_pool_desc* d, const float* dy, int dy_cs, int dy_coff, float* dx, int dx_cs,
                       int dx_coff, int overwrite, void* stream);

int sf_clip_prologue(const unsigned char* clip, int T, int H, int W, int new_h, int new_w, int y0, int x0, int crop,
                     int flip, int reverse, const float* mean3, const float* std3, const int* frame_idx,
                     int n_frames, float* dst, int ph, int pw, int Wp, void* stream);

int sf_clip_prologue_gray(const unsigned char* clip, int T, int H, int W, int new_h, int new_w, int y0, int x0,
                          int crop, int flip, float mean, float stdv, const int* frame_idx, int n_frames, float* dst,
                          int ph, int pw, int Wp, void* stream);

int sf_clip_views(const unsigned char* video, int T, int H, int W, const int* table_host, const int* table, int V,
                  int n_fast, int n_slow, int crop, int reverse, const float* mean3, const float* std3, float* fast,
                  float* slow, int ph, int pw, int Wp, void* stream);
int sf_clip_views_gray(const unsigned char* video, int T, int H, int W, const int* table_host, const int* table, int V,
                       int n_fast, int n_slow, int crop, float mean, float stdv, float* fast, float* slow, int ph,
                       int pw, int Wp, void* stream);

int sf_clip_batch(const long* table_host, const long* table, int B, int n_fast, int n_slow, int crop, int reverse,
                  const float* mean3, const float* std3, float* fast, float* slow, int ph, int pw, int Wp,
                  void* stream);
int sf_clip_batch_gray(const long* table_host, const long* table, int B, int n_fast, int n_slow, int crop, float mean,
                       float stdv, float* fast, float* slow, int ph, int pw, int Wp, void* stream);

int sf_ensemble_update(const float* preds, const int* video_idx, const int* labels, float* video_preds,
                       int* video_labels, int* clip_count, int* bad_count, int B, int K, int Nv, int mode,
                       void* stream);
int sf_ensemble_update_ml(const float* preds, const int* video_idx, const float* labels, int ldl, float* video_preds,
                          float* video_labels, int* clip_count, int* bad_count, int B, int K, int Nv, int mode,
                          void* stream);

int sf_stem1_accepts(int Hp, int Wp, int Cout, int kT);
int sf_stem1_fwd(const float* x, int N, int T, int Hp, int Wp, const float* w, int Cout, int kT, int pT,
                 const float* scale, const float* bias, int act, float* out, int out_cs, int out_coff, void* stream);
long sf_stem1_wgrad_ws_floats(int N, int T, int Hp, int Wp, int Cout, int kT, int pT);
int sf_stem1_wgrad(const float* x, int N, int T, int Hp, int Wp, const float* dz, int dz_cs, int dz_coff, int Cout,
                   int kT, int pT, float* dw, int accumulate, float* ws, void* stream);
int sf_ncthw1_pack(const float* src, float* dst, int N, int T, int H, int W, int ph, int pw, int Wp, void* stream);

int sf_epilogue_bwd(const float* dy, int dy_cs, int dy_coff, const float* y, int y_cs, int y_coff, int N, int T, int H,
                    int W, int C, int rep, const float* scale, int relu, float* dz, int dz_cs, int dz_coff,
                    int dz_accumulate, float* dres, int dres_cs, int dres_coff, int dres_accumulate, void* stream);
int sf_epilogue_bwd_act(const float* dy, int dy_cs, int dy_coff, const float* y, int y_cs, int y_coff, int N, int T,
                        int H, int W, int C, int rep, const float* scale, int act, int groups, float* dz, int dz_cs,
                        int dz_coff, int dz_accumulate, float* dres, int dres_cs, int dres_coff, int dres_accumulate,
                        void* stream);
int sf_dwconv_dgrad_epi(const sf_conv_desc* d, const float* dy, int dy_cs, int dy_coff, const float* y, int y_cs,
                        int y_coff, const float* w_packed, const float* scale, int act, float* dx, int dx_cs,
                        int dx_coff, int C, int accumulate, void* stream);
int sf_head_act_mean_bwd(const float* logits, const float* dout, int B, int P, int K, int act, float* dl,
                         int accumulate, void* stream);
int sf_cam_weights(const float* g, int g_cs, int g_coff, int N, int T, int H, int W, int C, float* w, void* stream);
long sf_cam_map_ws_floats(int N, int H, int W, int C);
int sf_cam_map(const float* a, int a_cs, int a_coff, const float* w, int N, int T, int H, int W, int C, float* ws,
               float* raw, float* cam, void* stream);

int sf_ctx_pool_parts(long rows_per_sample);
long sf_ctx_pool_ws_floats(int N, long rows_per_sample, int C);
int sf_ctx_pool_fwd(const float* x, int cs, int coff, int N, long rows_per_sample, int C, const float* w,
                    const float* b, float* ctx, float* lse, float* ws, void* stream);
int sf_ctx_pool_bwd(const float* x, int cs, int coff, int N, long rows_per_sample, int C, const float* w,
                    const float* b, const float* lse, const float* ctx, const float* dctx, float* dx, int dx_cs,
                    int dx_coff, int accumulate, float* dw, float* db, int dw_accumulate, float* ws, void* stream);
long sf_sample_affine_ws_floats(int N, long rows_per_sample, int C);
int sf_sample_affine_fwd(const float* x, int cs, int coff, int N, long rows_per_sample, int C, const float* mul,
                         const float* add, float* out, int out_cs, int out_coff, void* stream);
int sf_sample_affine_bwd(const float* dy, int dy_cs, int dy_coff, const float* x, int x_cs, int x_coff, int N,
                         long rows_per_sample, int C, const float* mul, float* dx, int dx_cs, int dx_coff,
                         int accumulate, float* dmul, float* dadd, float* ws, void* stream);

#define SF_STRIPE_MEAN 0
#define SF_STRIPE_MAX 1
#define SF_STRIPE_MEANMAX 2
#define SF_STRIPE_SUM 3
// ... 38 lines not shown
```

Measured before the change: 152.8.

## Fuse BN-backward channel reductions into the conv dgrad epilogue

When a conv's data-gradient output feeds straight into a BatchNorm backward, the dgrad GEMM epilogue now also computes per-tile partial sums of masked dy and dy*xhat from the accumulator registers. It writes those partials to a small buffer. The BN backward then runs a light final reduction instead of a full reduce pass over dy and z, saving one read of large activations. The cost is extra z and mask loads plus an LDS reduction in the GEMM epilogue, and bookkeeping in the tape to check that the gradient is touched only once.

```diff
diff --git a/efficient-slowfast_amd/csrc/backward.hip b/efficient-slowfast_amd/csrc/backward.hip
--- a/efficient-slowfast_amd/csrc/backward.hip
+++ b/efficient-slowfast_amd/csrc/backward.hip
@@ -563,6 +563,16 @@
                               invstd, dbeta, dgamma, ws, stream, dbeta_acc, dgamma_acc);
 }
 
+extern "C" int sf_bn_bwd_sums_final(const float* sums, int parts, int C, float* dbeta, float* dgamma, float* dbeta_acc,
+                                    float* dgamma_acc, void* stream) {
+  if (!sums || parts <= 0 || C <= 0 || !dbeta || !dgamma) return SF_EINVAL;
+  if ((dbeta_acc == nullptr) != (dgamma_acc == nullptr)) return SF_EINVAL;
+  hipLaunchKernelGGL(pair_final_kernel, dim3(C), dim3(64), 0, (hipStream_t)stream, sums, C, parts, parts, 1, dbeta,
+                     dgamma, dbeta_acc, dgamma_acc);
+  SF_CHECK_LAUNCH();
+  return SF_OK;
+}
+
 extern "C" int sf_bn_bwd_reduce_split(const float* dy, int dy_cs, int dy_coff, const float* y, int y_cs, int y_coff,
                                       const float* z, int z_cs, int z_coff, int N, int T, int H, int W, int C,
                                       int nsplit, int rep, int relu, const float* mean, const float* invstd,
diff --git a/efficient-slowfast_amd/csrc/conv_bx.hip b/efficient-slowfast_amd/csrc/conv_bx.hip
--- a/efficient-slowfast_amd/csrc/conv_bx.hip
+++ b/efficient-slowfast_amd/csrc/conv_bx.hip
@@ -26,6 +26,13 @@
   const float* xf;
   unsigned xf_bytes;
   float* stats;
+  const float* bn_z;
+  const unsigned char* bn_mask;
+  const float* bn_mean;
+  const float* bn_invstd;
+  float* sums;
+  int bn_z_cs, bn_z_coff;
+  unsigned bn_z_bytes, bn_mask_bytes;
 };
 
 __device__ __forceinline__ unsigned mdiv(unsigned n, unsigned mul, unsigned sh) {
@@ -34,8 +41,71 @@
 
 typedef __attribute__((address_space(3))) void lds_void;
 
-template <int BN, bool DIRECT, bool AF32>
+template <int BN, int NT, int EB, class Args>
+__device__ __forceinline__ void bn_sums_tile(const Args& p, const f32x16 (&acc)[2][NT], float* sred, int m0, int n0,
+                                             int tile_m, int wm, int wn, int lane, int tid) {
+  const int col = lane & 31, rsub = 4 * (lane >> 5);
+  const int C = p.d.Cout;
+  const __amdgpu_buffer_rsrc_t z_rs = __builtin_amdgcn_make_buffer_rsrc((void*)p.bn_z, 0, p.bn_z_bytes, 0x00020000);
+  const __amdgpu_buffer_rsrc_t k_rs = __builtin_amdgcn_make_buffer_rsrc((void*)p.bn_mask, 0, p.bn_mask_bytes, 0x00020000);
+#pragma unroll
+  for (int j = 0; j < NT; ++j) {
+    const int cl = wn * (BN / 2) + j * 32 + col;
+    const int n = n0 + cl;
+    const bool n_ok = n < C;
+    const float mu = n_ok ? p.bn_mean[n] : 0.f;
+    const float is = n_ok ? p.bn_invstd[n] : 0.f;
+    const unsigned bit = 1u << (n & 3);
+    float s1 = 0.f, s2 = 0.f;
+#pragma unroll
+    for (int ih = 0; ih < 2 * (16 / EB); ++ih) {
+      const int i = ih / (16 / EB), e0 = (ih % (16 / EB)) * EB;
+      float zv[EB];
+      unsigned mk[EB];
+#pragma unroll
+      for (int u = 0; u < EB; ++u) {
+        const int e = e0 + u;
+        const int m = m0 + wm * 64 + i * 32 + (e & 3) + 8 * (e >> 2) + rsub;
+        const bool ok = n_ok && m < p.M;
+        const unsigned zo = ((unsigned)m * (unsigned)p.bn_z_cs + (unsigned)(p.bn_z_coff + n)) * 4u;
+        const unsigned ko = (unsigned)m * (unsigned)(C >> 2) + (unsigned)(n >> 2);
+        zv[u] = __builtin_bit_cast(float, __builtin_amdgcn_raw_buffer_load_b32(z_rs, ok ? zo : 0x80000000u, 0, 0));
+        mk[u] = (unsigned)__builtin_amdgcn_raw_buffer_load_b8(k_rs, ok ? ko : 0x80000000u, 0, 0);
+      }
+#pragma unroll
+      for (int u = 0; u < EB; ++u) {
+        const float g = (mk[u] & bit) ? acc[i][j][e0 + u] : 0.f;
+        s1 += g;
+        s2 = fmaf(g, (zv[u] - mu) * is, s2);
+      }
+      __builtin_amdgcn_sched_barrier(0);
+    }
+    s1 += __shfl_xor(s1, 32, 64);
+    s2 += __shfl_xor(s2, 32, 64);
+    if (rsub == 0) {
+      sred[(wm * BN + cl) * 2] = s1;
+      sred[(wm * BN + cl) * 2 + 1] = s2;
+    }
+  }
+  __syncthreads();
+  if (tid < BN) {
+    const int n = n0 + tid;
+    if (n < C) {
+      float s1 = 0.f, s2 = 0.f;
+#pragma unroll
+      for (int w = 0; w < 4; ++w) {
+        s1 += sred[(w * BN + tid) * 2];
+        s2 += sred[(w * BN + tid) * 2 + 1];
+      }
+      p.sums[((long)tile_m * 2 + 0) * C + n] = s1;
+      p.sums[((long)tile_m * 2 + 1) * C + n] = s2;
+    }
+  }
+}
+
+template <int BN, bool DIRECT, bool AF32, bool SUMS = false>
 __global__ __launch_bounds__(512, 2) void conv_bx_kernel(const BxArgs p) {
+  static_assert(!SUMS || DIRECT, "only a workgroup that holds the finished tile takes the BN-backward sums");
   constexpr int A_ST = AF32 ? BXC_BM * 64 : BXC_A_STAGE;
   constexpr int B_STAGE = 3 * BN * BXC_ROWB;
   constexpr int STAGE = A_ST + B_STAGE;
@@ -284,6 +354,10 @@
         }
       }
     }
+    if constexpr (SUMS) {
+      __syncthreads();
+      bn_sums_tile<BN, NT, 16>(p, acc, reinterpret_cast<float*>(smem), m0, n0, tile_m, wm, wn, lane, tid);
+    }
     return;
   }
   float* const wsp = p.ws + (long)split * p.M * d.Cout;
@@ -300,7 +374,7 @@
     }
 }
 
-template <int BN>
+template <int BN, bool SUMS = false>
 __global__ __launch_bounds__(512, 4) void conv_pw_bx_kernel(const BxArgs p) {
   constexpr int A_STAGE = BXC_BM * 64;
   constexpr int B_STAGE = 3 * BN * BXC_ROWB;
@@ -393,6 +467,23 @@
   }
 
   const int col = lane & 31, rsub = 4 * (lane >> 5);
+  if constexpr (SUMS) {
+#pragma unroll
+    for (int j = 0; j < NT; ++j) {
+      const int n = n0 + wn * (BN / 2) + j * 32 + col;
+#pragma unroll
+      for (int i = 0; i < 2; ++i)
+#pragma unroll
+        for (int e = 0; e < 16; ++e) {
+          const int m = m0 + wm * 64 + i * 32 + (e & 3) + 8 * (e >> 2) + rsub;
+          if (m < p.M && n < d.Cout) p.out[(long)m * d.out_cs + d.out_coff + n] = acc[i][j][e];
+        }
+    }
+    __syncthreads();
+    constexpr int EB = BN > 64 ? 4 : 16;
+    bn_sums_tile<BN, NT, EB>(p, acc, reinterpret_cast<float*>(smem), m0, n0, tile_m, wm, wn, lane, tid);
+    return;
+  }
   const bool want_stats = p.stats != nullptr;
   float* const kred = reinterpret_cast<float*>(smem);
   if (want_stats) __syncthreads();
@@ -717,14 +808,14 @@
 
 bool bx_af32(const sf_conv_desc* d);
 
-bool bx_plan(const sf_conv_desc* d, BxPlan* pl, bool gate = true) {
+bool bx_plan(const sf_conv_desc* d, BxPlan* pl, bool gate = true, bool any = false) {
   if (!g_bx_enable) return false;
   const long M = (long)d->N * d->To * d->Ho * d->Wo;
   const int ntaps = d->kT * d->kH * d->kW;
   if ((d->Cin % 16) || d->cin_pad != d->Cin || (d->in_cs % 4) || (d->in_coff % 4)) return false;
-  if (d->Cout < 128 || (d->Cout % 4) || d->out_cmul != 1) return false;
+  if ((!any && d->Cout < 128) || (d->Cout % 4) || d->out_cmul != 1) return false;
   const int nk = ntaps * (d->Cin / BXC_BK);
-  if (nk < 32 || M < 2048 || M > 0x7fffffffL) return false;
+  if ((!any && (nk < 32 || M < 2048)) || M < 1 || M > 0x7fffffffL) return false;
   if (d->transposed && (d->sT != 1 || d->sH != 1 || d->sW != 1)) return false;
   const long a_rows = (long)d->N * d->Ti * d->Hi * d->Wi;
   if (3 * (a_rows + 1) * d->Cin * 2 > 0xfffffff0L) return false;
@@ -739,7 +830,7 @@
   const double out_mb = (double)M * d->Cout * 4e-6;
   int best = 1;
   double best_t = 1e30;
-  for (int S = 1; S <= 16 && nk / S >= 8; ++S) {
+  for (int S = 1; S <= (any ? 1 : 16) && nk / S >= 8; ++S) {
     const long wg = (long)pl->tiles * S;
     if (wg > 2048) break;
     const long rounds = sf_cdiv(wg, 256);
@@ -751,7 +842,7 @@
   pl->S = best;
   pl->nk_per = sf_cdiv(nk, best);
   pl->direct = (best == 1 && !scatter) ? 1 : 0;
-  if (gate && g_bx_enable < 2) {
+  if (gate && !any && g_bx_enable < 2) {
     const double flop = 2.0 * M * (double)nk * BXC_BK * d->Cout;
     const double wave_us = flop / (nk >= 64 ? 100e6 : 90e6);
     const double split_us = bx_af32(d) ? 0.0 : 4.0 + (double)a_rows * d->Cin * 10e-6 / 3.0;
@@ -766,7 +857,7 @@
 
 struct PwPlan { int bn, nb_n, tiles, nk; };
 
-bool pw_plan(const sf_conv_desc* d, PwPlan* pl, bool gate = true) {
+bool pw_plan(const sf_conv_desc* d, PwPlan* pl, bool gate = true, bool any = false) {
   if (!g_bx_enable || !g_pw_enable) return false;
   if (d->kT != 1 || d->kH != 1 || d->kW != 1 || d->sT != 1 || d->sH != 1 || d->sW != 1 || d->pT || d->pH || d->pW)
     return false;
@@ -775,14 +866,14 @@
   if ((d->Cin % 16) || d->cin_pad != d->Cin || (d->in_cs % 4) || (d->in_coff % 4)) return false;
   if (d->Cin < 64 || d->Cout < 64 || (d->Cout % 4)) return false;
   const long M = (long)d->N * d->To * d->Ho * d->Wo;
-  if (M < 2048 || M > 0x3fffffffL) return false;
+  if ((!any && M < 2048) || M < 1 || M > 0x3fffffffL) return false;
   if (((M - 1) * d->in_cs + d->in_coff + d->Cin) * 4L >= 0x7fffffffL) return false;
   pl->nk = d->Cin / BXC_BK;
   if (3L * (d->Cout + 1) * pl->nk * BXC_ROWB > 0xfffffff0L) return false;
   pl->bn = d->Cout <= 64 ? 64 : 128;
   pl->nb_n = sf_cdiv(d->Cout, pl->bn);
   pl->tiles = sf_cdiv(M, BXC_BM) * pl->nb_n;
-  if (gate && g_pw_enable < 2 && g_bx_enable < 2) {
+  if (gate && !any && g_pw_enable < 2 && g_bx_enable < 2) {
     const double mb = (double)M * (d->Cin + d->Cout) * 4e-6;
     if (pl->bn == 64) {
       if (d->Cin < 128) return false;
@@ -797,13 +888,13 @@
   return true;
 }
 
-template <int BN>
+template <int BN, bool SUMS = false>
 int launch_pw(const BxArgs& a, int grid, hipStream_t stream) {
   constexpr int lds = 2 * (BXC_BM * 64 + 3 * BN * BXC_ROWB);
   static_assert(lds >= (BN + 4 * BN * 2) * 4, "the statistics scratch lives in the stages");
   static SfLdsAttr at;
-  if (!sf_ensure_dyn_lds(at, reinterpret_cast<const void*>(conv_pw_bx_kernel<BN>), lds)) return SF_ELAUNCH;
-  hipLaunchKernelGGL((conv_pw_bx_kernel<BN>), dim3(grid), dim3(512), lds, stream, a);
+  if (!sf_ensure_dyn_lds(at, reinterpret_cast<const void*>(conv_pw_bx_kernel<BN, SUMS>), lds)) return SF_ELAUNCH;
+  hipLaunchKernelGGL((conv_pw_bx_kernel<BN, SUMS>), dim3(grid), dim3(512), lds, stream, a);
   SF_CHECK_LAUNCH();
   return SF_OK;
 }
@@ -817,12 +908,14 @@
 long a_plane_floats(const sf_conv_desc* d, long a_rows) { return align4((3 * (a_rows + 1) * d->Cin + 1) / 2); }
 long b_plane_floats(const sf_conv_desc* d, int nk) { return align4((3L * (d->Cout + 1) * nk * BXC_BK + 1) / 2); }
 
-template <int BN, bool DIRECT, bool AF32>
+template <int BN, bool DIRECT, bool AF32, bool SUMS = false>
 int launch_bx_v(const BxArgs& a, int grid, hipStream_t stream) {
   constexpr int lds = BXC_STAGES * ((AF32 ? BXC_BM * 64 : BXC_A_STAGE) + 3 * BN * BXC_ROWB);
+  static_assert(lds >= 4 * BN * 2 * 4, "bn_sums_tile's scratch lives in the stages");
   static SfLdsAttr at;
-  if (!sf_ensure_dyn_lds(at, reinterpret_cast<const void*>(conv_bx_kernel<BN, DIRECT, AF32>), lds)) return SF_ELAUNCH;
-  hipLaunchKernelGGL((conv_bx_kernel<BN, DIRECT, AF32>), dim3(grid), dim3(512), lds, stream, a);
+  if (!sf_ensure_dyn_lds(at, reinterpret_cast<const void*>(conv_bx_kernel<BN, DIRECT, AF32, SUMS>), lds))
+    return SF_ELAUNCH;
+  hipLaunchKernelGGL((conv_bx_kernel<BN, DIRECT, AF32, SUMS>), dim3(grid), dim3(512), lds, stream, a);
   SF_CHECK_LAUNCH();
   return SF_OK;
 }
@@ -998,6 +1091,71 @@
   if (!d || !in || !w_packed || !out || !ws) return SF_EINVAL;
   const int rc = sf_conv_bx_try(d, in, in_planes, w_packed, w_planes, scale, bias, res, out, ws, (hipStream_t)stream);
   return rc == 1 ? SF_ENOTTAKEN : rc;
+}
+
+namespace {
+
+int dgrad_sums_plan(const sf_conv_desc* d, int any_shape, PwPlan* pw, BxPlan* bx) {
+  if (!d->transposed || d->act != SF_ACT_NONE || (d->Cout % 4)) return 0;
+  if (pw_plan(d, pw, true, any_shape != 0)) return 1;
+  if (bx_plan(d, bx, true, any_shape != 0) && bx->direct && bx_af32(d)) return 2;
+  return 0;
+}
+
+}
+
+extern "C" long sf_conv_dgrad_bn_sums_floats(const sf_conv_desc* d, int any_shape) {
+  PwPlan pw;
+  BxPlan bx;
+  if (!d || !dgrad_sums_plan(d, any_shape, &pw, &bx)) return 0;
+  const long M = (long)d->N * d->To * d->Ho * d->Wo;
+  return (long)sf_cdiv(M, BXC_BM) * 2 * d->Cout;
+}
+
+extern "C" int sf_conv_dgrad_bn_sums(const sf_conv_desc* d, const float* dz, const unsigned short* w_planes, float* out,
+                                     const float* z, int z_cs, int z_coff, const unsigned char* mask,
+                                     const float* mean, const float* invstd, float* sums, int any_shape, int* parts,
+                                     void* stream) {
+  if (!d || !dz || !w_planes || !out || !z || !mask || !mean || !invstd || !sums || !parts) return SF_EINVAL;
+  if (z_cs < z_coff + d->Cout || z_coff < 0) return SF_EINVAL;
+  PwPlan pw;
+  BxPlan bx;
+  const int kind = dgrad_sums_plan(d, any_shape, &pw, &bx);
+  if (!kind) return SF_ENOTTAKEN;
+  if (!sf_aligned16(dz) || !sf_aligned16(w_planes)) return SF_EALIGN;
+  const long M = (long)d->N * d->To * d->Ho * d->Wo;
+  const long z_bytes = ((M - 1) * z_cs + z_coff + d->Cout) * 4L, mask_bytes = M * (d->Cout / 4);
+  if (z_bytes >= 0x7fffffffL || mask_bytes >= 0x7fffffffL) return SF_ENOTTAKEN;
+  const int nk = kind == 1 ? pw.nk : bx.nk;
+  BxArgs a = {};
+  a.d = *d;
+  a.bp = w_planes;
+  a.out = out;
+  a.M = (int)M;
+  a.b_plane = (unsigned)((long)(d->Cout + 1) * nk * BXC_ROWB);
+  a.b_bytes = 3u * a.b_plane;
+  a.xf = dz;
+  a.bn_z = z; a.bn_z_cs = z_cs; a.bn_z_coff = z_coff;
+  a.bn_z_bytes = (unsigned)z_bytes; a.bn_mask_bytes = (unsigned)mask_bytes;
+  a.bn_mask = mask; a.bn_mean = mean; a.bn_invstd = invstd; a.sums = sums;
+  *parts = (int)sf_cdiv(M, BXC_BM);
+  hipStream_t s = (hipStream_t)stream;
+  if (kind == 1) {
+    a.ntaps = 1; a.cpk = nk; a.nk = nk; a.S = 1; a.nk_per = nk; a.nb_n = pw.nb_n; a.tiles = pw.tiles;
+    a.xf_bytes = (unsigned)(((M - 1) * d->in_cs + d->in_coff + d->Cin) * 4L);
+    return pw.bn == 64 ? launch_pw<64, true>(a, pw.tiles, s) : launch_pw<128, true>(a, pw.tiles, s);
+  }
+  a.xf_bytes = (unsigned)(((bx.a_rows - 1) * d->in_cs + d->in_coff + d->Cin) * 4L);
+  a.ntaps = d->kT * d->kH * d->kW;
+  a.cpk = d->Cin / BXC_BK;
+  a.nk = nk; a.S = 1; a.nk_per = nk; a.nb_n = bx.nb_n; a.tiles = bx.tiles;
+  a.tap_major = 0;
+  a.a_rows = (unsigned)bx.a_rows;
+  magic((unsigned)d->Wo, &a.wo_mul, &a.wo_sh);
+  magic((unsigned)d->Ho, &a.ho_mul, &a.ho_sh);
+  magic((unsigned)d->To, &a.to_mul, &a.to_sh);
+  return bx.bn == 256 ? launch_bx_v<256, true, true, true>(a, bx.tiles, s)
+                      : launch_bx_v<128, true, true, true>(a, bx.tiles, s);
 }
 
 namespace {
diff --git a/efficient-slowfast_amd/sfhip/__init__.py b/efficient-slowfast_amd/sfhip/__init__.py
--- a/efficient-slowfast_amd/sfhip/__init__.py
+++ b/efficient-slowfast_amd/sfhip/__init__.py
@@ -76,6 +76,8 @@
     "sf_conv_fwd_pw": (_ci, [_CD] + [_vp] * 9 + [_pi, _vp]),
     "sf_conv_bx_ws_floats": (_cl, [_CD, _ci, _ci]),
     "sf_conv_fwd_bx": (_ci, [_CD] + [_vp] * 10),
+    "sf_conv_dgrad_bn_sums_floats": (_cl, [_CD, _ci]),
+    "sf_conv_dgrad_bn_sums": (_ci, [_CD] + [_vp] * 4 + [_ci, _ci] + [_vp] * 4 + [_ci, _pi, _vp]),
     "sf_pack_conv_weight": (_ci, [_vp, _ci, _ci, _ci, _vp, _ci, _vp, _ci, _vp]),
     "sf_pack_conv_weights": (_ci, [_vp, _vp, _ci, _ci, _vp]),
     "sf_dwconv_fwd": (_ci, [_CD] + [_vp] * 7),
@@ -135,6 +137,7 @@
     "sf_bn_bwd_reduce": (_ci, _BN_BWD + [_vp]),
     "sf_bn_bwd_reduce_acc": (_ci, _BN_BWD + [_vp, _vp, _vp]),
     "sf_bn_bwd_reduce_split": (_ci, _BN_BWD_SPLIT + [_vp]),
+    "sf_bn_bwd_sums_final": (_ci, [_vp, _ci, _ci] + [_vp] * 5),
     "sf_bn_bwd_apply": (_ci, _BN_BWD + _BN_APPLY_TAIL),
     "sf_bn_bwd_apply_first": (_ci, _BN_BWD + _BN_APPLY_TAIL),
     "sf_bn_bwd_apply_split": (_ci, _BN_BWD_SPLIT + _BN_APPLY_TAIL),
@@ -987,6 +990,25 @@
 
 
 
+def conv_dgrad_bn_sums(dz, wt_packed, out, kernel, padding, dilation, z, mask, mean, invstd, any_shape=False):
+    _require_gpu(dz.buf, "conv_dgrad_bn_sums")
+    cin, taps, cout_pad = wt_packed.shape
+    if not SPLIT_K or cout_pad != dz.C or z.C != cin or (z.N, z.T, z.H, z.W) != (out.N, out.T, out.H, out.W):
+        return None
+    d = _conv_desc(dz, (out.T, out.H, out.W), out.cs, out.coff, cin, kernel, (1, 1, 1), padding, dilation,
+                   cin_pad=cout_pad, transposed=1)
+    n = lib().sf_conv_dgrad_bn_sums_floats(ctypes.byref(d), 1 if any_shape else 0)
+    if n <= 0:
+        return None
+    sums = torch.empty((n,), dtype=torch.float32, device=dz.buf.device)
+    parts = ctypes.c_int(0)
+    tag = ("conv", d.N * d.To * d.Ho * d.Wo, d.kT * d.kH * d.kW * d.Cin, d.Cout)
+    rc = _call("sf_conv_dgrad_bn_sums", ctypes.byref(d), dz.ptr(), _ptr(_weight_planes(wt_packed)), out.ptr(), z.ptr(),
+               z.cs, z.coff, _ptr(mask), _ptr(mean.contiguous()), _ptr(invstd.contiguous()), _ptr(sums),
+               1 if any_shape else 0, ctypes.byref(parts), tag=tag, allow=_REFUSED)
+    return (sums, parts.value) if rc == 0 else None
+
+
 def _residue_taps(k, s, p, a):
     pairs = sorted(((a + p - kk) // s, kk) for kk in range(k) if (a + p - kk) % s == 0)
     return [o for o, _ in pairs], [kk for _, kk in pairs]
@@ -1159,7 +1181,7 @@
 
 
 def bn_bwd(dy, y, z, mean, invstd, gamma, relu, rep=1, dres=None, dz_out=None, dgamma_out=None, nsplit=1,
-           sync=None, grad_sink=None, mask=None, dres_overwrite=False):
+           sync=None, grad_sink=None, mask=None, dres_overwrite=False, conv_sums=None):
     C = z.C
     dev = z.buf.device
     mean, invstd, gamma = mean.contiguous(), invstd.contiguous(), gamma.detach().contiguous()
@@ -1175,7 +1197,13 @@
     if dres_overwrite:
         assert dres is not None and nsplit == 1
         apply_fn = "sf_bn_bwd_apply_first"
-    if grad_sink is not None:
+    if conv_sums is not None:
+        assert nsplit == 1 and rep == 1 and code == 3 and conv_sums[0].numel() >= conv_sums[1] * 2 * C
+        assert grad_sink is None or dgamma_out is None
+        _call("sf_bn_bwd_sums_final", _ptr(conv_sums[0]), conv_sums[1], C, _ptr(dbeta), _ptr(dgamma),
+              _ptr(grad_sink[1]) if grad_sink is not None else None,
+              _ptr(grad_sink[0]) if grad_sink is not None else None)
+    elif grad_sink is not None:
         assert nsplit == 1 and dgamma_out is None
         _call("sf_bn_bwd_reduce_acc", *head, *tail, _ptr(dbeta), _ptr(dgamma), _ptr(ws), _ptr(grad_sink[1]),
               _ptr(grad_sink[0]))
diff --git a/efficient-slowfast_amd/slowfast/models/engine.py b/efficient-slowfast_amd/slowfast/models/engine.py
--- a/efficient-slowfast_amd/slowfast/models/engine.py
+++ b/efficient-slowfast_amd/slowfast/models/engine.py
@@ -55,6 +55,9 @@
         self.zero_floats = -1
         self.armed = True
         self.param_grads = True
+        self.bn_src = {}
+        self.bn_sums = {}
+        self.gtouch = {}
 
     def pgrad_target(self, param):
         if self.sink is None:
@@ -64,6 +67,8 @@
 
     def grad_of(self, act):
         key = act.buf.data_ptr()
+        if key in self.bn_src:
+            self.gtouch[key] = self.gtouch.get(key, 0) + 1
         g = self.gbuf.get(key)
         if g is None:
             n = act.buf.numel()
@@ -86,6 +91,8 @@
         key = act.buf.data_ptr()
         if not whole or key in self.gbuf or act.coff != 0 or act.cs != act.C:
             return self.grad_of(act), True
+        if key in self.bn_src:
+            self.gtouch[key] = self.gtouch.get(key, 0) + 1
         g = torch.empty(act.buf.numel(), dtype=torch.float32, device=act.buf.device)
         self.gbuf[key] = g
         return Act(g.view(act.buf.shape), 0, act.C), False
@@ -132,6 +139,7 @@
             self.ops = []
             self.zero_floats = -1
             self.gbuf = {}
+            self.bn_src, self.bn_sums, self.gtouch = {}, {}, {}
             self.arena = None
             self.arena_off = 0
             self.capturing = False
@@ -359,6 +367,12 @@
                                 lambda: sfhip.pack_conv_weight(conv_weight.detach().reshape(
                                     conv_weight.shape[0], conv_weight.shape[1], *kernel).transpose(0, 1).contiguous()))
             dx, acc = t.grad_dst(x)
+            src = None if acc else t.bn_src.get(x.buf.data_ptr())
+            if src is not None and max(stride) == 1:
+                got = sfhip.conv_dgrad_bn_sums(g, wtp, dx, kernel, padding, dilation, *src)
+                if got is not None:
+                    t.bn_sums[x.buf.data_ptr()] = got
+                    return
             sfhip.conv_dgrad(g, wtp, x, kernel, stride, padding, dilation, out=dx, accumulate=acc)
 
     t.record(bwd)
@@ -502,8 +516,16 @@
     return mean, invstd, scale, shift, 1, bn.weight, None
 
 
+def bn_sums_source(t, y, zz, mask, stats, rep, nsplit, keep, shuffled):
+    if stats is None or mask is None or type(t) is not Tape or rep != 1 or nsplit != 1 or keep is not None or shuffled:
+        return None
+    if zz.C % 4 or y.coff != 0 or y.cs != y.C or y.C != zz.C:
+        return None
+    return zz, mask, stats[0], stats[1]
+
+
 def _bn_epilogue(bn, z, scale, shift, make_backward, res, relu, rep, out, out_reserve, keep, out_cmul, nsplit=1,
-                 eager_sums=False, always_sums=False):
+                 eager_sums=False, always_sums=False, dgrad_stats=None):
     zz = z if keep is None else z.slice(0, keep)
     if keep is not None:
         assert nsplit == 1, "channel-sliced BN (GhostModule) is only defined for plain BatchNorm3d"
@@ -519,6 +541,10 @@
         weight, bias = getattr(bn, "weight", None), getattr(bn, "bias", None)
         affine = weight is not None and bias is not None
         backward = make_backward()
+        ykey = y.buf.data_ptr()
+        src = bn_sums_source(t, y, zz, mask, dgrad_stats, rep, nsplit, keep, shuffled)
+        if src is not None:
+            t.bn_src[ykey] = src
 
         def zeros():
             return torch.zeros(z.C, dtype=torch.float32, device=z.buf.device)
@@ -536,7 +562,9 @@
                     sink = (wt, bt)
                 else:
                     sums = made or (zeros(), zeros())
-            backward(t.grad_of(y), y, zz, dres, acc, sink, sums, mask)
+            pre = t.bn_sums.pop(ykey, None) if src is not None and t.gtouch.get(ykey) == 1 else None
+            extra = {} if pre is None else dict(conv_sums=pre)
+            backward(t.grad_of(y), y, zz, dres, acc, sink, sums, mask, **extra)
             if keep is not None and keep < z.C:
                 rest = z.slice(keep, z.C - keep)
                 sfhip.axpy(rest, rest, alpha=0.0, accumulate=False)
@@ -557,13 +585,14 @@
         mean, invstd, scale, shift, nsplit, gamma_b, sync = _bn_train_stats(bn, z, conv_stats)
     sel = slice(None) if nsplit > 1 else slice(0, z.C if keep is None else keep)
 
-    def backward(dy, y, zz, dres, dres_accumulate, sink, sums, mask):
+    def backward(dy, y, zz, dres, dres_accumulate, sink, sums, mask, conv_sums=None):
         sfhip.bn_bwd(dy, y, zz, mean[sel], invstd[sel], gamma_b[sel], relu, rep=rep, dres=dres, dz_out=zz,
                      dgamma_out=sums, nsplit=nsplit, sync=sync, grad_sink=sink, mask=mask,
-                     dres_overwrite=not dres_accumulate)
+                     dres_overwrite=not dres_accumulate, conv_sums=conv_sums)
 
     return _bn_epilogue(bn, z, scale, shift, lambda: backward, res, relu, rep, out, out_reserve, keep, out_cmul,
-                        nsplit=nsplit, eager_sums=not _GRAD_SINK, always_sums=True)
+                        nsplit=nsplit, eager_sums=not _GRAD_SINK, always_sums=True,
+                        dgrad_stats=(mean, invstd) if (nsplit == 1 and sync is None) else None)
 
 
 def bn_affine(bn, conv_bias=None):
diff --git a/include/sfhip.h b/include/sfhip.h
--- a/include/sfhip.h
+++ b/include/sfhip.h
@@ -176,6 +176,12 @@
                          const float* z, int z_cs, int z_coff, int N, int T, int H, int W, int C, int rep, int relu,
                          const float* mean, const float* invstd, float* dbeta, float* dgamma, float* ws,
                          float* dbeta_acc, float* dgamma_acc, void* stream);
+long sf_conv_dgrad_bn_sums_floats(const sf_conv_desc* d, int any_shape);
+int sf_conv_dgrad_bn_sums(const sf_conv_desc* d, const float* dz, const unsigned short* w_planes, float* out,
+                          const float* z, int z_cs, int z_coff, const unsigned char* mask, const float* mean,
+                          const float* invstd, float* sums, int any_shape, int* parts, void* stream);
+int sf_bn_bwd_sums_final(const float* sums, int parts, int C, float* dbeta, float* dgamma, float* dbeta_acc,
+                         float* dgamma_acc, void* stream);
 int sf_bn_bwd_apply(const float* dy, int dy_cs, int dy_coff, const float* y, int y_cs, int y_coff,
                     const float* z, int z_cs, int z_coff, int N, int T, int H, int W, int C, int rep, int relu,
                     const float* mean, const float* invstd, const float* gamma, const float* dbeta,
```

Result: no change. 152.4 (-0.2%).
